# jianzhnie/RLZero

Hardware: AMD Instinct MI355X
Metric: mcts_sims_per_sec (higher is better)
Workload: dtype f32 net (hi + lo f16 operand pairs on the f16 MFMA pipe, f32 accumulation) / f64 tree

## Files before the change

include/rlzero_hip.h:

```cpp
#ifndef RLZERO_HIP_H
#define RLZERO_HIP_H

#include <stdint.h>

#ifdef __cplusplus
extern "C" {
#endif

#define RZ_ABI_VERSION 27
#define RZ_MAX_BOARD_SIZE 16
#define RZ_BOARD_WORDS 4
#define RZ_MAX_IN_FLIGHT 16

enum {
    RZ_OK = 0,
    RZ_ERR_ARG = -1,
    RZ_ERR_HIP = -2,
    RZ_ERR_OOM = -3,
    RZ_ERR_OVERFLOW = -4,
    RZ_ERR_ILLEGAL = -5,
    RZ_ERR_INTERNAL = -6
};

enum {
    RZ_GAME_GOMOKU = 0,
    RZ_GAME_CONNECT4 = 1
};

enum {
    RZ_SCORE_UCT_REF = 0,
    RZ_SCORE_PUCT = 1
};

enum { RZ_EVAL_V0 = 0, RZ_EVAL_VLIN = 1 };

enum {
    RZ_FLAG_ARENA_FULL = 1,
    RZ_FLAG_BLOCKS_FULL = 2,
    RZ_FLAG_ILLEGAL_MOVE = 4,
    RZ_FLAG_LOGTAB = 8,
    RZ_FLAG_INTERNAL = 16,
    RZ_FLAG_REUSE_DROPPED = 32
};

typedef struct rz_engine rz_engine;

typedef struct rz_config {
    int32_t abi_version;
    int32_t game_kind;
    int32_t board_size;
    int32_t n_in_row;
    int32_t n_games;
    int32_t n_playout;
    int32_t score_mode;
    int32_t add_noise;
    double c_puct;
    double pool_factor;
    int32_t device;
    int32_t noise_seed;
    int32_t board_height;
    int32_t board_width;
    int32_t sims_in_flight;
    int32_t in_flight_impl;
} rz_config;

typedef struct rz_stats {
    int32_t error_flags;
    int32_t first_bad_game;
    int64_t arena_slots;
    int64_t prior_floats;
    int64_t max_slots_used;
    int64_t max_blocks_used;
    int64_t device_bytes;
    int64_t n_select_calls;
    int64_t reuse_dropped;
} rz_stats;

int rz_abi_version(void);
const char *rz_source_hash(void);
const char *rz_last_error(void);

int rz_create(const rz_config *cfg, rz_engine **out);
int rz_destroy(rz_engine *e);
int rz_geometry(rz_engine *e, int32_t *height, int32_t *width, int32_t *n_actions);

int rz_upload_log_table(rz_engine *e, const double *h_table, int64_t count);
int rz_log_table_size(rz_engine *e, int64_t *count);

int rz_set_roots(rz_engine *e, const uint64_t *d_stones, const int32_t *d_to_move,
                 const int32_t *d_last_move, const uint8_t *d_mask, int reset_trees,
                 void *stream);
int rz_get_roots(rz_engine *e, uint64_t *d_stones, int32_t *d_to_move, int32_t *d_last_move,
                 void *stream);
int rz_set_active(rz_engine *e, const uint8_t *d_active, void *stream);
int rz_set_noise_keys(rz_engine *e, const uint64_t *d_keys, const uint8_t *d_mask, void *stream);

int rz_select_step(rz_engine *e, float *d_obs, void *stream);
int rz_set_in_flight(rz_engine *e, int32_t k_backup, int32_t k_select);

int rz_leaf_buffers(rz_engine *e, const uint64_t **d_stones, const int32_t **d_to_move, const int32_t **d_last_cell);

int rz_encode_leaf_obs(rz_engine *e, float *d_obs, void *stream);
int rz_encode_root_obs(rz_engine *e, float *d_obs, void *stream);

int rz_get_leaves(rz_engine *e, uint64_t *d_stones, int32_t *d_to_move, int32_t *d_last_move,
                  int32_t *d_terminal, void *stream);

int rz_eval_synthetic(rz_engine *e, int kind, float *d_logp, float *d_value, void *stream);

int rz_eval_rollout(rz_engine *e, uint64_t seed, uint32_t sim_index, int32_t n_limit, float *d_value,
                    void *stream);

int rz_expand_backup(rz_engine *e, const float *d_logp, const float *d_value, void *stream);
int rz_expand_backup_f64(rz_engine *e, const float *d_logp, const double *d_value, void *stream);
int rz_expand_backup_probs(rz_engine *e, const float *d_probs, const double *d_value, void *stream);

int rz_tree_step(rz_engine *e, const float *d_logp, const float *d_value, float *d_obs, void *stream);

typedef struct rz_raw_heads {
    const float *raw;
    const float *hid;
    const float *w2;
    const float *b2;
    const float *act_scale;
    const float *act_bias;
    const float *val_scale;
    const float *val_bias;
    int64_t raw_part_stride;
    int64_t hid_part_stride;
    int32_t ld;
    int32_t n_parts;
} rz_raw_heads;

int rz_expand_backup_raw(rz_engine *e, const rz_raw_heads *heads, void *stream);
int rz_tree_step_raw(rz_engine *e, const rz_raw_heads *heads, float *d_obs, void *stream);

typedef struct rz_value_head {
    const float *valfeat;
    const float *w1t;
    const float *b1;
    const float *w2;
    const float *b2;
    int32_t ld;
    int32_t groups;
} rz_value_head;
typedef struct rz_deferred_logits {
    const float *raw;
    int32_t ld;
    int32_t rows_per_slot;
} rz_deferred_logits;
int rz_deferred_reserve(rz_engine *e, int32_t slots);
int rz_trace_attach(rz_engine *e, void *d_trace);
int rz_device_view(rz_engine *e, void *out, int64_t out_bytes);
int rz_deferred_slots(rz_engine *e, const int32_t **d_slot_of_game);
int rz_expand_backup_deferred(rz_engine *e, const rz_value_head *head, void *stream);
int rz_tree_step_deferred(rz_engine *e, const rz_value_head *head, void *stream);
int rz_deferred_flush(rz_engine *e, const rz_deferred_logits *logits, int32_t n_slots, void *stream);

int rz_root_visits(rz_engine *e, int32_t *d_visits, void *stream);
int rz_root_wsum(rz_engine *e, double *d_w, void *stream);
int rz_root_priors(rz_engine *e, float *d_p, void *stream);
int rz_root_stats(rz_engine *e, int32_t *d_n, double *d_w, void *stream);
int rz_root_values(rz_engine *e, double *d_out, void *stream);

int rz_advance_roots(rz_engine *e, const int32_t *d_moves, void *stream);

int rz_step_games(rz_engine *e, const int32_t *d_moves, int32_t *d_winner, uint8_t *d_ended,
                  void *stream);

#define RZ_PLAY_RECORD_WORDS 8
enum {
    RZ_PLAY_RUNNING = 1,
    RZ_PLAY_STALLED = 2,
    RZ_PLAY_RESOLVED = 4,
    RZ_PLAY_ENDED = 8,
    RZ_PLAY_SEARCHED = 16,
    RZ_PLAY_RESIGNED = 32,
    RZ_PLAY_NO_RESIGN = 64,
    RZ_PLAY_WOULD_RESIGN = 128
};
typedef struct rz_play_config {
    uint64_t seed;
    double temperature;
    double stall_margin;
    const int64_t *d_queue_ids;
    int32_t *d_queue_ctl;
    int32_t *d_log;
    int32_t ring_steps;
    int32_t reserved;
} rz_play_config;
int rz_play_attach(rz_engine *e, const rz_play_config *cfg);
int rz_play_draw(rz_engine *e, void *stream);
int rz_play_apply(rz_engine *e, void *stream);
int rz_play_set_resign(rz_engine *e, double threshold, double disabled_frac, void *stream);
int rz_play_resolve(rz_engine *e, int32_t slot, int32_t move, void *stream);
int rz_play_stop(rz_engine *e, void *stream);
int rz_play_state(rz_engine *e, int64_t *h_game_id, int32_t *h_ply, int32_t *h_state, int64_t *h_steps);

int rz_get_stats(rz_engine *e, rz_stats *out);
int rz_clear_errors(rz_engine *e);
int rz_poll_errors(rz_engine *e, int32_t *h_flags, int32_t *h_reuse_dropped, void *stream);

int rz_copy_arena(rz_engine *e, int32_t game, int64_t max_slots, int32_t *h_n, double *h_w,
                  int32_t *h_first_child, int32_t *h_n_visited, int32_t *h_n_children,
                  int32_t *h_prior_block, float *h_root_prior, int32_t *h_top);
int rz_copy_priors(rz_engine *e, int32_t game, int64_t max_floats, float *h_priors, int32_t *h_count);

int rz_uct_scores(rz_engine *e, const double *d_w, const int32_t *d_n, const int32_t *d_np,
                  double c_puct, double *d_out, int64_t count, void *stream);

typedef struct rz_net rz_net;
enum {
    RZ_NET_DIRECT = 0,
    RZ_NET_WINOGRAD_F4 = 1,
    RZ_NET_SPLIT_F16 = 2
    ,
    RZ_NET_SPLIT_F16_TILES = 3
    ,
    RZ_NET_SPLIT_F16_FP8 = 4
};
int rz_net_range_info(rz_net *net, float *h_info8);
enum { RZ_NET_FLAG_F16_RANGE = 1 };
int rz_net_error_flags(rz_net *net, uint32_t *h_flags);
int rz_net_set_algo(rz_net *net, int32_t algo);
int rz_net_set_max_workgroups(rz_net *net, int32_t max_workgroups);
enum { RZ_NET_HEADS_AUTO = 0, RZ_NET_HEADS_F32 = 1, RZ_NET_HEADS_SPLIT_32 = 2, RZ_NET_HEADS_SPLIT_64 = 3, RZ_NET_HEADS_SPLIT_PARTS = 4,
       RZ_NET_HEADS_IN_TRUNK = 5    };
int rz_net_set_heads_algo(rz_net *net, int32_t heads_algo);
int rz_net_create(int32_t height, int32_t width, int32_t n_actions, int32_t device, rz_net **out);
int rz_net_destroy(rz_net *net);
int rz_net_load(rz_net *net, const float *const *h_params, int32_t n_params);
int rz_net_reserve(rz_net *net, int32_t max_boards);
int rz_net_trunk(rz_net *net, const float *d_obs, int32_t n_boards, float *d_feat, void *stream);
int rz_net_trunk_leaves(rz_net *net, const uint64_t *d_stones, const int32_t *d_to_move, const int32_t *d_last_cell,
                        int32_t n_boards, void *stream);
int rz_net_deferred_reserve(rz_net *net, int32_t max_boards, int32_t slots);
int rz_net_trunk_leaves_deferred(rz_net *net, const uint64_t *d_stones, const int32_t *d_to_move, const int32_t *d_last_cell,
                                 int32_t n_boards, const int32_t *d_slot_of_board, rz_value_head *out, void *stream);
int rz_net_deferred_gemm(rz_net *net, int32_t n_boards, int32_t n_slots, rz_deferred_logits *out, void *stream);
int rz_net_trace_attach(rz_net *net, void *d_trace);
int rz_net_delta_reserve(rz_net *net, int32_t n_games);
int rz_net_delta_invalidate(rz_net *net, void *stream);
int rz_net_delta_resident(rz_net *net, int32_t on);
int rz_net_delta_bases(rz_net *net, const uint64_t *d_root_stones, const int32_t *d_root_to_move, int32_t n_games, void *stream);
int rz_net_delta_leaves(rz_net *net, const uint64_t *d_stones, const int32_t *d_to_move, const int32_t *d_last_cell, int32_t n_boards,
                        const int32_t *d_slot_of_board, const uint8_t *d_active, float *d_feat32, int32_t without_base, rz_value_head *out,
                        void *stream);
int rz_net_delta_bases_engine(rz_net *net, rz_engine *engine, void *stream);
int rz_net_delta_step(rz_net *net, rz_engine *engine, rz_value_head *out, void *stream);
int rz_net_delta_trunk_engine(rz_net *net, rz_engine *engine, void *stream);
int rz_net_delta_stats(rz_net *net, uint32_t *h_out8, int32_t reset);
int rz_net_search_resident(rz_net *net, rz_engine *engine, int32_t n_sims, int32_t select_first, void *stream);
int rz_net_heads(rz_net *net, int32_t n_boards, float *d_logp, float *d_value, void *stream);
int rz_net_heads_gemm(rz_net *net, int32_t n_boards, rz_raw_heads *out, void *stream);
int rz_net_forward(rz_net *net, const float *d_obs, int32_t n_boards, float *d_logp,
                   float *d_value, void *stream);

typedef struct rz_muzero rz_muzero;
typedef struct rz_mz_config {
    int32_t abi_version;
    int32_t n_games;
    int32_t n_actions;
    int32_t n_sims;
    double discount;
    double pb_c_base;
    double pb_c_init;
    int32_t device;
    int32_t reserved;
} rz_mz_config;

int rz_mz_create(const rz_mz_config *cfg, rz_muzero **out);
int rz_mz_destroy(rz_muzero *e);
int rz_mz_upload_log_table(rz_muzero *e, const double *h_table, int64_t count);
int rz_mz_init_roots(rz_muzero *e, const float *d_probs, const double *d_noise, double noise_frac,
                     const uint8_t *d_mask, void *stream);
int rz_mz_select(rz_muzero *e, int32_t *d_parent, int32_t *d_action, int32_t *d_leaf, const uint8_t *d_mask,
                 void *stream);
int rz_mz_expand_backup(rz_muzero *e, const float *d_reward, const float *d_probs, const float *d_value,
                        const uint8_t *d_mask, void *stream);
int rz_mz_load_model(rz_muzero *e, const float *const *h_params, int32_t n_params, int32_t hidden);
int rz_mz_search(rz_muzero *e, float *d_hidden, int32_t n_sims, int32_t *d_trace_parent, int32_t *d_trace_action,
                 int32_t *d_trace_leaf, float *d_trace_reward, float *d_trace_probs, float *d_trace_value, void *stream);
int rz_mz_set_search_shape(rz_muzero *e, int32_t games_per_workgroup);
typedef struct rz_mz_cartpole_play {
    double *d_state;
    int64_t *d_steps, *d_episode, *d_episode_start;
    uint64_t env_seed, noise_seed;
    double noise_frac, dirichlet_alpha, temperature;
    double *d_ring;
    int32_t ring_steps, reserved;
    int64_t first_step;
    double *d_arena;
    int64_t arena_rows;
    int64_t *d_counters, *d_entries;
    int64_t max_entries;
} rz_mz_cartpole_play;
int rz_mz_load_representation(rz_muzero *e, const float *const *h_params, int32_t n_params, int32_t obs_dim, int32_t hidden);
int rz_mz_play_cartpole(rz_muzero *e, float *d_hidden, int32_t n_sims, int32_t n_moves, const rz_mz_cartpole_play *play, void *stream);
int rz_cartpole_step(double *d_state, int64_t *d_steps, int64_t *d_episode, const int64_t *d_actions, int32_t n_envs, uint64_t seed,
                     float *d_obs, float *d_reward, uint8_t *d_terminated, uint8_t *d_truncated, void *stream);
int rz_mz_root_children(rz_muzero *e, int32_t what, void *d_out, void *stream);
int rz_mz_root_stats(rz_muzero *e, int32_t *d_n, double *d_value_sum, double *d_vmin, double *d_vmax, void *stream);
int rz_mz_geometry(rz_muzero *e, int32_t *slots_per_game, int64_t *device_bytes);
int rz_mz_error_flags(rz_muzero *e, int32_t *flags);

#ifdef __cplusplus
}
#endif
#endif
```

profiles/microbench/delta_resident_phases.py:

```python
import ctypes, os, sys
sys.path.insert(0, os.environ.get('GRAFT_REPO_ROOT', '.'))
import rlzero_amd._hip as H
H.library_path = lambda: os.environ.get('RZ_NETPROF_LIB') or os.path.join(os.path.dirname(os.path.abspath(__file__)), 'librlzero_netprof.so')
import rlzero_amd._build as B
B.needs_build = lambda: False
import numpy as np, torch
from rlzero_amd.engine import HipNetEvaluator, MCTSEngine
from rlzero_amd.games.gomoku.policy_value_net import PolicyValueNet
lib = H.load()
NAMES = [(0, 'leaf + changed cells'), (1, 'distances, requests, ranks'), (3, 'maps, base records'), (4, 'bar'), (5, 'conv1'), (6, 'bar'), (7, 'conv2'),
         (9, 'bar + conv3 + heads'), (10, 'bar'), (11, 'features'), (12, 'bar'), (16, 'value layer'), (17, 'expand + backup'),
         (2, 'sel: root record'), (8, 'sel: root scan / answer'), (13, 'sel: level-0 cell'), (14, 'sel: deeper levels'), (15, 'sel: terminal test + leaf stores'),
         (18, 'selection (rest: hand-over)'), (19, 'wave 1: pre-scan'), (20, 'wave 1: wait behind it')]
sizes = [int(a) for a in sys.argv[1:]] or [1, 256, 512]
for games in sizes:
    torch.manual_seed(0)
    net = PolicyValueNet(15).to('cuda:0')
    ev = HipNetEvaluator(net, 15, 'cuda:0', max_boards=games)
    sims = 800
    eng = MCTSEngine(15, 5, n_games=games, n_playout=sims, device='cuda:0', add_noise=True)
    eng.reset_games()
    assert ev.resident_ok(eng) and ev.resident_delta_ok(eng)
    rng = np.random.default_rng(0)
    for ply in range(6):
        eng.sim_chunk(ev, 40)
        visits = eng.root_visits()
        moves = np.array([int(rng.choice(np.flatnonzero(v > 0))) for v in visits], dtype=np.int32)
        eng.advance(moves)
        eng.step(moves)
    a, b = torch.cuda.Event(enable_timing=True), torch.cuda.Event(enable_timing=True)
    ev.hip.delta_stats(reset=True)
    a.record(); eng.sim_chunk(ev, sims); b.record(); torch.cuda.synchronize()
    st = ev.hip.delta_stats()
    out = (ctypes.c_longlong * 24)()
    assert lib.rz_net_debug_profile(out) == 0
    us = 1e3 * a.elapsed_time(b) / sims
    total = out[23] / sims
    print('%d games, %d simulations: %.2f us per simulation of a game (events, bases included), %d cycles (%.2f GHz); %.2f conv3 / %.2f conv2 tiles, %.2f changed cells per leaf, %d leaves without a base' % (
        games, sims, us, total, total / us / 1e3, st['tiles3'] / max(1, st['delta'] + st['no_base']), st['tiles2'] / max(1, st['delta'] + st['no_base']),
        st['cells'] / max(1, st['delta'] + st['no_base']), st['no_base']))
    print('   ' + '  '.join('%s=%d' % (nm, out[k] / sims) for k, nm in NAMES) + '  prescans=%d' % st['prescans'], flush=True)
    eng.close(); ev.hip.close()
```

rlzero_amd/_hip.py:

```python
import ctypes
import os
from ctypes import (POINTER, Structure, c_char_p, c_double, c_int, c_int32, c_int64, c_uint32, c_uint64,
                    c_void_p)

ABI_VERSION = 27
BOARD_WORDS = 4
MAX_BOARD_SIZE = 16
MAX_IN_FLIGHT = 16

OK = 0
SCORE_UCT_REF, SCORE_PUCT = 0, 1
GAME_GOMOKU, GAME_CONNECT4 = 0, 1
NET_DIRECT, NET_WINOGRAD_F4, NET_SPLIT_F16, NET_SPLIT_F16_TILES, NET_SPLIT_F16_FP8 = 0, 1, 2, 3, 4
NET_FLAG_F16_RANGE = 1
NET_HEADS_AUTO, NET_HEADS_F32, NET_HEADS_SPLIT_32, NET_HEADS_SPLIT_64, NET_HEADS_SPLIT_PARTS, NET_HEADS_IN_TRUNK = 0, 1, 2, 3, 4, 5
EVAL_V0, EVAL_VLIN = 0, 1
FLAG_NAMES = {1: 'arena full', 2: 'block queue full', 4: 'illegal move', 8: 'ln table too short',
              16: 'internal'}
FLAG_REUSE_DROPPED = 32


class RzConfig(Structure):
    _fields_ = [('abi_version', c_int32), ('game_kind', c_int32), ('board_size', c_int32),
                ('n_in_row', c_int32), ('n_games', c_int32), ('n_playout', c_int32),
                ('score_mode', c_int32), ('add_noise', c_int32), ('c_puct', c_double),
                ('pool_factor', c_double), ('device', c_int32), ('noise_seed', c_int32),
                ('board_height', c_int32), ('board_width', c_int32),
                ('sims_in_flight', c_int32), ('in_flight_impl', c_int32)]


class RzStats(Structure):
    _fields_ = [('error_flags', c_int32), ('first_bad_game', c_int32), ('arena_slots', c_int64),
                ('prior_floats', c_int64), ('max_slots_used', c_int64), ('max_blocks_used', c_int64),
                ('device_bytes', c_int64), ('n_select_calls', c_int64), ('reuse_dropped', c_int64)]


class RzMzConfig(Structure):
    _fields_ = [('abi_version', c_int32), ('n_games', c_int32), ('n_actions', c_int32), ('n_sims', c_int32),
                ('discount', c_double), ('pb_c_base', c_double), ('pb_c_init', c_double),
                ('device', c_int32), ('reserved', c_int32)]


class RzMzCartPolePlay(Structure):
    _fields_ = [('d_state', c_void_p), ('d_steps', c_void_p), ('d_episode', c_void_p), ('d_episode_start', c_void_p),
                ('env_seed', c_uint64), ('noise_seed', c_uint64), ('noise_frac', c_double), ('dirichlet_alpha', c_double),
                ('temperature', c_double), ('d_ring', c_void_p), ('ring_steps', c_int32), ('reserved', c_int32),
                ('first_step', c_int64), ('d_arena', c_void_p), ('arena_rows', c_int64), ('d_counters', c_void_p),
                ('d_entries', c_void_p), ('max_entries', c_int64)]


class RzRawHeads(Structure):
    _fields_ = [('raw', c_void_p), ('hid', c_void_p), ('w2', c_void_p), ('b2', c_void_p), ('act_scale', c_void_p),
                ('act_bias', c_void_p), ('val_scale', c_void_p), ('val_bias', c_void_p), ('raw_part_stride', c_int64),
                ('hid_part_stride', c_int64), ('ld', c_int32), ('n_parts', c_int32)]


class RzValueHead(Structure):
    _fields_ = [('valfeat', c_void_p), ('w1t', c_void_p), ('b1', c_void_p), ('w2', c_void_p), ('b2', c_void_p),
                ('ld', c_int32), ('groups', c_int32)]


class RzDeferredLogits(Structure):
    _fields_ = [('raw', c_void_p), ('ld', c_int32), ('rows_per_slot', c_int32)]


class RzPlayConfig(Structure):
    _fields_ = [('seed', c_uint64), ('temperature', c_double), ('stall_margin', c_double), ('d_queue_ids', c_void_p),
                ('d_queue_ctl', c_void_p), ('d_log', c_void_p), ('ring_steps', c_int32), ('reserved', c_int32)]


PLAY_RECORD_WORDS = 8
PLAY_RUNNING, PLAY_STALLED, PLAY_RESOLVED, PLAY_ENDED, PLAY_SEARCHED = 1, 2, 4, 8, 16
PLAY_RESIGNED, PLAY_NO_RESIGN, PLAY_WOULD_RESIGN = 32, 64, 128


class HipError(RuntimeError):
    pass


P = c_void_p

_SIGNATURES = {
    'rz_abi_version': (c_int, []),
    'rz_last_error': (c_char_p, []),
    'rz_source_hash': (c_char_p, []),
    'rz_create': (c_int, [POINTER(RzConfig), POINTER(c_void_p)]),
    'rz_destroy': (c_int, [P]),
    'rz_geometry': (c_int, [P, POINTER(c_int32), POINTER(c_int32), POINTER(c_int32)]),
    'rz_upload_log_table': (c_int, [P, P, c_int64]),
    'rz_log_table_size': (c_int, [P, POINTER(c_int64)]),
    'rz_set_roots': (c_int, [P, P, P, P, P, c_int, P]),
    'rz_get_roots': (c_int, [P, P, P, P, P]),
    'rz_set_active': (c_int, [P, P, P]),
    'rz_set_noise_keys': (c_int, [P, P, P, P]),
    'rz_select_step': (c_int, [P, P, P]),
    'rz_set_in_flight': (c_int, [P, c_int32, c_int32]),
    'rz_leaf_buffers': (c_int, [P, POINTER(c_void_p), POINTER(c_void_p), POINTER(c_void_p)]),
    'rz_encode_leaf_obs': (c_int, [P, P, P]),
    'rz_encode_root_obs': (c_int, [P, P, P]),
    'rz_get_leaves': (c_int, [P, P, P, P, P, P]),
    'rz_eval_synthetic': (c_int, [P, c_int, P, P, P]),
    'rz_eval_rollout': (c_int, [P, c_uint64, c_uint32, c_int32, P, P]),
    'rz_expand_backup': (c_int, [P, P, P, P]),
    'rz_expand_backup_f64': (c_int, [P, P, P, P]),
    'rz_expand_backup_probs': (c_int, [P, P, P, P]),
    'rz_tree_step': (c_int, [P, P, P, P, P]),
    'rz_expand_backup_raw': (c_int, [P, POINTER(RzRawHeads), P]),
    'rz_tree_step_raw': (c_int, [P, POINTER(RzRawHeads), P, P]),
    'rz_trace_attach': (c_int, [P, P]),
    'rz_net_trace_attach': (c_int, [P, P]),
    'rz_device_view': (c_int, [P, P, c_int64]),
    'rz_deferred_reserve': (c_int, [P, c_int32]),
    'rz_deferred_slots': (c_int, [P, POINTER(c_void_p)]),
    'rz_expand_backup_deferred': (c_int, [P, POINTER(RzValueHead), P]),
    'rz_tree_step_deferred': (c_int, [P, POINTER(RzValueHead), P]),
    'rz_deferred_flush': (c_int, [P, POINTER(RzDeferredLogits), c_int32, P]),
    'rz_root_visits': (c_int, [P, P, P]),
    'rz_root_wsum': (c_int, [P, P, P]),
    'rz_root_priors': (c_int, [P, P, P]),
    'rz_root_stats': (c_int, [P, P, P, P]),
    'rz_root_values': (c_int, [P, P, P]),
    'rz_advance_roots': (c_int, [P, P, P]),
    'rz_step_games': (c_int, [P, P, P, P, P]),
    'rz_play_attach': (c_int, [P, POINTER(RzPlayConfig)]),
    'rz_play_draw': (c_int, [P, P]),
    'rz_play_apply': (c_int, [P, P]),
    'rz_play_set_resign': (c_int, [P, c_double, c_double, P]),
    'rz_play_resolve': (c_int, [P, c_int32, c_int32, P]),
    'rz_play_stop': (c_int, [P, P]),
    'rz_play_state': (c_int, [P, P, P, P, POINTER(c_int64)]),
    'rz_get_stats': (c_int, [P, POINTER(RzStats)]),
    'rz_clear_errors': (c_int, [P]),
    'rz_poll_errors': (c_int, [P, POINTER(c_int32), POINTER(c_int32), P]),
    'rz_copy_arena': (c_int, [P, c_int32, c_int64, P, P, P, P, P, P, P, P]),
    'rz_copy_priors': (c_int, [P, c_int32, c_int64, P, P]),
    'rz_uct_scores': (c_int, [P, P, P, P, c_double, P, c_int64, P]),
    'rz_net_create': (c_int, [c_int32, c_int32, c_int32, c_int32, POINTER(c_void_p)]),
    'rz_net_destroy': (c_int, [P]),
    'rz_net_set_algo': (c_int, [P, c_int32]),
    'rz_net_set_max_workgroups': (c_int, [P, c_int32]),
    'rz_net_set_heads_algo': (c_int, [P, c_int32]),
    'rz_net_error_flags': (c_int, [P, POINTER(ctypes.c_uint32)]),
    'rz_net_range_info': (c_int, [P, POINTER(ctypes.c_float)]),
    'rz_net_load': (c_int, [P, POINTER(c_void_p), c_int32]),
    'rz_net_reserve': (c_int, [P, c_int32]),
    'rz_net_trunk': (c_int, [P, P, c_int32, P, P]),
    'rz_net_trunk_leaves': (c_int, [P, P, P, P, c_int32, P]),
    'rz_net_deferred_reserve': (c_int, [P, c_int32, c_int32]),
    'rz_net_trunk_leaves_deferred': (c_int, [P, P, P, P, c_int32, P, POINTER(RzValueHead), P]),
    'rz_net_deferred_gemm': (c_int, [P, c_int32, c_int32, POINTER(RzDeferredLogits), P]),
    'rz_net_search_resident': (c_int, [P, P, c_int32, c_int32, P]),
    'rz_net_delta_reserve': (c_int, [P, c_int32]),
    'rz_net_delta_invalidate': (c_int, [P, P]),
    'rz_net_delta_resident': (c_int, [P, c_int32]),
    'rz_net_delta_bases': (c_int, [P, P, P, c_int32, P]),
    'rz_net_delta_leaves': (c_int, [P, P, P, P, c_int32, P, P, P, c_int32, POINTER(RzValueHead), P]),
    'rz_net_delta_stats': (c_int, [P, POINTER(ctypes.c_uint32), c_int32]),
    'rz_net_delta_bases_engine': (c_int, [P, P, P]),
    'rz_net_delta_step': (c_int, [P, P, POINTER(RzValueHead), P]),
    'rz_net_delta_trunk_engine': (c_int, [P, P, P]),
    'rz_net_heads': (c_int, [P, c_int32, P, P, P]),
    'rz_net_heads_gemm': (c_int, [P, c_int32, POINTER(RzRawHeads), P]),
    'rz_net_forward': (c_int, [P, P, c_int32, P, P, P]),
    'rz_mz_create': (c_int, [POINTER(RzMzConfig), POINTER(c_void_p)]),
    'rz_mz_destroy': (c_int, [P]),
    'rz_mz_upload_log_table': (c_int, [P, P, c_int64]),
    'rz_mz_init_roots': (c_int, [P, P, P, c_double, P, P]),
    'rz_mz_select': (c_int, [P, P, P, P, P, P]),
    'rz_mz_expand_backup': (c_int, [P, P, P, P, P, P]),
    'rz_mz_load_model': (c_int, [P, POINTER(c_void_p), c_int32, c_int32]),
    'rz_mz_search': (c_int, [P, P, c_int32, P, P, P, P, P, P, P]),
    'rz_mz_set_search_shape': (c_int, [P, c_int32]),
    'rz_mz_load_representation': (c_int, [P, POINTER(c_void_p), c_int32, c_int32, c_int32]),
    'rz_mz_play_cartpole': (c_int, [P, P, c_int32, c_int32, POINTER(RzMzCartPolePlay), P]),
    'rz_cartpole_step': (c_int, [P, P, P, P, c_int32, c_uint64, P, P, P, P, P]),
    'rz_mz_root_children': (c_int, [P, c_int32, P, P]),
    'rz_mz_root_stats': (c_int, [P, P, P, P, P, P]),
    'rz_mz_geometry': (c_int, [P, POINTER(c_int32), POINTER(c_int64)]),
    'rz_mz_error_flags': (c_int, [P, POINTER(c_int32)]),
}

_lib = None


def library_path():
    return os.environ.get('RZ_HIP_LIBRARY') or os.path.join(os.path.dirname(os.path.abspath(__file__)), 'librlzero_hip.so')


def load():
    global _lib
    if _lib is not None:
        return _lib
    path = library_path()
    if not os.path.exists(path):
        raise HipError('%s is missing: the HIP extension is required (no CPU fallback). '
                       'Build it with `python -m rlzero_amd._build`.' % path)
    lib = ctypes.CDLL(path)
    for name, (restype, argtypes) in _SIGNATURES.items():
        fn = getattr(lib, name)
        fn.restype = restype
        fn.argtypes = argtypes
    got = lib.rz_abi_version()
    if got != ABI_VERSION:
        raise HipError('librlzero_hip.so has ABI %d, binding expects %d: rebuild' % (got, ABI_VERSION))
    if not os.environ.get('RZ_HIP_LIBRARY'):
        from . import _build
        built, tree = (lib.rz_source_hash() or b'').decode(), _build.source_hash()
        if built != tree:
            raise HipError('librlzero_hip.so was built from other sources (hash %s, this tree %s): python -m rlzero_amd._build' % (built, tree))
    _lib = lib
    return lib


def exported_symbols():
    return sorted(_SIGNATURES)


def check(rc, what=''):
    if rc != OK:
        msg = load().rz_last_error()
        raise HipError('%s failed (%d): %s' % (what or 'rz call', rc, (msg or b'').decode()))
```

rlzero_amd/csrc/rz_delta.h:

```cpp
#ifndef RZ_DELTA_TREE_PRIO
#define RZ_DELTA_TREE_PRIO 1
#endif
#ifndef RZ_DELTA_PRO_PRIO
#define RZ_DELTA_PRO_PRIO 0
#endif
#ifndef RZ_DELTA_PRESCAN
#define RZ_DELTA_PRESCAN 1
#endif

namespace dl {

using sp::f16x4;
using sp::f16x8;
typedef const __attribute__((address_space(3))) f16x8 *lds_frag;
typedef const __attribute__((address_space(3))) uint32_t *lds_u32;
typedef __attribute__((address_space(3))) f16x4 *lds_h4;
typedef __attribute__((address_space(3))) f32x4 *lds_v4;

constexpr int kC1Slots = 128, kC2Slots = 164;
constexpr int kT1 = 4, kT2 = 8, kT3 = 8;
constexpr int kMaxD = 4;
constexpr int P1 = rt::Geo<32>::pos_bytes, P2 = rt::Geo<64>::pos_bytes;
constexpr int kGrid = kRowW * kRowW;
constexpr int kShareFloats = kT3 * 4 * 96;
constexpr int kHeadW = 128 * 6 * 4 + 128 * 4 + 32;
constexpr int kOffC1 = sp::kInPieceBytes, kOffC2 = kOffC1 + kC1Slots * P1, kOffZero = kOffC2 + kC2Slots * P2, kOffHead = kOffZero + P2,
              kOffMap1 = kOffHead + kHeadW, kOffMap2 = kOffMap1 + kGrid * 4, kOffList = kOffMap2 + kGrid * 4,
              kLdsBytes = kOffList + 3 * 128 * 2;
static_assert(kShareFloats * 4 <= kC1Slots * P1, "the shares lie inside conv1's records (dead behind conv2)");
constexpr int kWinSets = rzw::kRadii * rzw::kWords, kWinLds = kWinSets * 8 + kWinSets * 4 + 16;
static_assert(2 * (kLdsBytes + 512 * 4 + 4 * 64 * 4 + 80 + kWinLds + (int)sizeof(rzt::RootPre) + 512) <= 160 * 1024,
              "two workgroups per CU, also of the resident search (value row, K-quarter sums, leaf, window sets, root pre-scan)");
static_assert(kOffC1 % 16 == 0 && kOffZero % 16 == 0 && kOffHead % 16 == 0 && kOffMap1 % 16 == 0, "alignment");

constexpr int kCells = RZ_MAX_BOARD_SIZE * RZ_MAX_BOARD_SIZE;
struct BaseHdr {
    uint64_t stones[2 * RZ_BOARD_WORDS];
    int32_t to_move, valid, pad[2];
};
constexpr size_t kBaseC2 = (size_t)kCells * 128, kBaseV = kBaseC2 + (size_t)kCells * 256, kBaseBytes = kBaseV + (size_t)6 * kCells * 4;

struct DeltaArgs {
    BaseHdr *hdr;
    char *recs;
    const uint8_t *active;
    float *feat32;
    unsigned *stats;
    int mode;
    int bw_rcp;
    const uint64_t *win;
};

__device__ __forceinline__ uint32_t lds_addr(const void *p) {
    return (uint32_t)(uintptr_t)((const __attribute__((address_space(3))) char *)p);
}

constexpr int unit_tiles(int nt) { return nt <= 3 ? nt : (nt + 1) / 2; }
constexpr int units_of(int nt) { return (nt + unit_tiles(nt) - 1) / unit_tiles(nt); }

template <int CIN, int NT, int UT>
__device__ __forceinline__ void read_unit(f16x8 (&b)[UT][2], const uint32_t (&rec)[NT][3], int h, int dy, int c) {
#pragma unroll
    for (int i = 0; i < UT; ++i) {
        const int t = h * UT + i;
        if (t < NT) {
            const uint32_t r = rec[t][dy] + (uint32_t)(c * 64);
            b[i][0] = *(lds_frag)(uintptr_t)r;
            b[i][1] = *(lds_frag)(uintptr_t)(r + CIN * 2);
        }
    }
}
template <int TM, int NT, int UT>
__device__ __forceinline__ void mfma_unit(f32x4 (&acc)[TM][NT], const f16x8 (&a)[TM][2], const f16x8 (&b)[UT][2], int h) {
#pragma unroll
    for (int combo = 0; combo < 3; ++combo)
#pragma unroll
        for (int i = 0; i < UT; ++i) {
            const int t = h * UT + i;
            if (t < NT) {
#pragma unroll
                for (int m = 0; m < TM; ++m)
                    acc[m][t] = __builtin_amdgcn_mfma_f32_16x16x32_f16(a[m][combo == 2], b[i][combo == 1], acc[m][t], 0, 0, 0);
            }
        }
}
template <int NT>
__device__ __forceinline__ void lookup(uint32_t (&rec)[NT][3], lds_u32 map, const int (&pos19)[NT], int dx, int g) {
#pragma unroll
    for (int t = 0; t < NT; ++t)
#pragma unroll
        for (int dy = 0; dy < 3; ++dy) rec[t][dy] = map[pos19[t] + dx + dy * kRowW] + (uint32_t)(g * 16);
}

template <int NT>
__device__ __forceinline__ void conv2_g(lds_u32 map, const int (&pos19)[NT], int lane, const f16x8 (&a2)[9][1][2], f32x4 (&acc)[1][NT]) {
    static_assert(NT <= 4, "one unit per step");
    const int g = lane >> 4;
#pragma unroll
    for (int t = 0; t < NT; ++t) acc[0][t] = f32x4{0.f, 0.f, 0.f, 0.f};
    constexpr int AHEAD = NT <= 2 ? 2 : 1;
    uint32_t rec[3][NT][3];
    f16x8 b[AHEAD + 1][NT][2];
#pragma unroll
    for (int dx = 0; dx < 3; ++dx) lookup<NT>(rec[dx], map, pos19, dx, g);
#pragma unroll
    for (int u = 0; u < AHEAD; ++u) read_unit<32, NT, NT>(b[u], rec[u / 3], 0, u % 3, 0);
#pragma unroll
    for (int u = 0; u < 9; ++u) {
        const int dx = u / 3, dy = u % 3;
        if (u + AHEAD < 9) read_unit<32, NT, NT>(b[(u + AHEAD) % (AHEAD + 1)], rec[(u + AHEAD) / 3], 0, (u + AHEAD) % 3, 0);
        mfma_unit<1, NT, NT>(acc, a2[dy * 3 + dx], b[u % (AHEAD + 1)], 0);
        __builtin_amdgcn_sched_barrier(0);
    }
}

#ifndef RZ_DELTA_RING6_UPTO
#define RZ_DELTA_RING6_UPTO 2
#endif
constexpr int ring3(int nt) { return nt <= RZ_DELTA_RING6_UPTO ? 6 : 3; }
__device__ __forceinline__ void load_a3(f16x8 (&a)[2][2], __amdgpu_buffer_rsrc_t w_rsrc, int lane, int dx, int j) {
    using G = rt::Geo<64>;
    const int c = j / 3, dy = j % 3;
#pragma unroll
    for (int m = 0; m < 2; ++m)
#pragma unroll
        for (int p = 0; p < 2; ++p)
            a[m][p] = sp::load_w(w_rsrc, lane * 16, dx * (G::chunks * 2048) + ((m * G::steps + dy * 3 * G::chunks + c) * 2 + p) * 1024);
}
template <int NT>
__device__ __forceinline__ void conv3_g(lds_u32 map, const uint16_t *list3, const void *wts, int lane, bool sync, f32x4 (&acc)[2][NT]) {
    static_assert(NT <= 6, "two units per step");
    constexpr int R = ring3(NT), H = units_of(NT);
    const int n = lane & 15, g = lane >> 4;
    const __amdgpu_buffer_rsrc_t w_rsrc = __builtin_amdgcn_make_buffer_rsrc(const_cast<void *>(wts), 0, 0x7fffffff, 0x00020000);
    f16x8 a3[R][2][2];
#pragma unroll
    for (int j = 0; j < R - 1; ++j) load_a3(a3[j], w_rsrc, lane, 0, j);
    if (sync) __syncthreads();
    int pos19[NT];
#pragma unroll
    for (int t = 0; t < NT; ++t) pos19[t] = (int)list3[16 * t + n] - 19;
#pragma unroll
    for (int m = 0; m < 2; ++m)
#pragma unroll
        for (int t = 0; t < NT; ++t) acc[m][t] = f32x4{0.f, 0.f, 0.f, 0.f};
    uint32_t rec[NT][3], recn[NT][3];
#ifndef RZ_DELTA_AHEAD3_SMALL
#define RZ_DELTA_AHEAD3_SMALL 1
#endif
    constexpr int UT = unit_tiles(NT), AH = UT <= 2 ? RZ_DELTA_AHEAD3_SMALL : 1, NB = AH + 1;
    static_assert((6 * H) % NB == 0 && AH <= H * 6, "a unit's registers are a constant of the unrolled body");
    f16x8 b[NB][UT][2];
    lookup<NT>(rec, map, pos19, 0, g);
#pragma unroll
    for (int u = 0; u < AH; ++u) read_unit<64, NT, UT>(b[u], rec, u % H, (u / H) % 3, u / H / 3);
#pragma unroll 1
    for (int dx = 0; dx < 3; ++dx) {
        lookup<NT>(recn, map, pos19, dx < 2 ? dx + 1 : 2, g);
#pragma unroll
        for (int u = 0; u < 6 * H; ++u) {
            const int j = u / H, h = u % H;
            if (h == 0) {
                const int jj = j + R - 1, dx2 = jj < 6 ? dx : (dx < 2 ? dx + 1 : 2);
                load_a3(a3[jj % R], w_rsrc, lane, dx2, jj % 6);
            }
            {
                const int v = u + AH;
                if (v < 6 * H) read_unit<64, NT, UT>(b[v % NB], rec, v % H, (v / H) % 3, v / H / 3);
                else read_unit<64, NT, UT>(b[v % NB], recn, (v - 6 * H) % H, ((v - 6 * H) / H) % 3, (v - 6 * H) / H / 3);
            }
            mfma_unit<2, NT, UT>(acc, a3[j % R], b[u % NB], h);
            __builtin_amdgcn_sched_barrier(0);
        }
#pragma unroll
        for (int t = 0; t < NT; ++t)
#pragma unroll
            for (int dy = 0; dy < 3; ++dy) rec[t][dy] = recn[t][dy];
    }
}

template <int T>
__device__ __forceinline__ void reduce_scatter(const float (&vals)[6 * T], float (&out)[6 * T / 4]) {
    float r1[3 * T];
#pragma unroll
    for (int i = 0; i < 3 * T; ++i) {
        const auto sw = __builtin_amdgcn_permlane16_swap(__float_as_uint(vals[i]), __float_as_uint(vals[3 * T + i]), false, false);
        r1[i] = __uint_as_float(sw[0]) + __uint_as_float(sw[1]);
    }
#pragma unroll
    for (int i = 0; i < 3 * T / 2; ++i) {
        const auto sw = __builtin_amdgcn_permlane32_swap(__float_as_uint(r1[i]), __float_as_uint(r1[3 * T / 2 + i]), false, false);
        out[i] = __uint_as_float(sw[0]) + __uint_as_float(sw[1]);
    }
}

template <int NT>
__device__ __forceinline__ void conv2_tiles(lds_u32 map1, lds_u32 map2, const uint16_t *list2, int n2, int lane, int wave, const f16x8 (&a2)[9][1][2],
                                            f32x4 bias2, float k2) {
    const int n = lane & 15, g = lane >> 4;
    int pos19[NT];
#pragma unroll
    for (int t = 0; t < NT; ++t) pos19[t] = (int)list2[16 * t + n] - 19;
    f32x4 acc[1][NT];
    conv2_g<NT>(map1, pos19, lane, a2, acc);
#pragma unroll
    for (int t = 0; t < NT; ++t) {
        if (16 * t + n < n2) {
            const uint32_t rec = map2[pos19[t] + kRowW + 1] + (uint32_t)((16 * wave + 4 * g) * 2);
            float z[4];
#pragma unroll
            for (int j = 0; j < 4; ++j) z[j] = fmaxf(fmaf(acc[0][t][j], k2, bias2[j]), 0.0f);
            f16x4 hi, lo;
            sp::split4(z, hi, lo);
            *(lds_h4)(uintptr_t)rec = hi;
            *(lds_h4)(uintptr_t)(rec + 128) = lo;
        }
    }
}

template <int NT>
__device__ __forceinline__ void conv3_tiles(lds_u32 map2, const uint16_t *list3, const void *wts, int lane, int wave, bool sync,
                                            const char *headw, float k3, float *shares) {
    constexpr int T = NT <= 4 ? 4 : 8;
    const int n = lane & 15, g = lane >> 4;
    float vals[6 * T];
    {
        f32x4 acc[2][NT];
        conv3_g<NT>(map2, list3, wts, lane, sync, acc);
        f32x4 hwr[2][6], b3r[2];
#pragma unroll
        for (int m = 0; m < 2; ++m) {
            const int c0 = 32 * wave + 16 * m + 4 * g;
#pragma unroll
            for (int i = 0; i < 6; ++i) hwr[m][i] = *reinterpret_cast<const f32x4 *>(headw + (c0 * 6 + 4 * i) * 4);
            b3r[m] = *reinterpret_cast<const f32x4 *>(headw + 128 * 6 * 4 + c0 * 4);
        }
#pragma unroll
        for (int t = 0; t < T; ++t) {
            f32x2 v2[3] = {f32x2{0.0f, 0.0f}, f32x2{0.0f, 0.0f}, f32x2{0.0f, 0.0f}};
            if (t < NT) {
#pragma unroll
                for (int m = 0; m < 2; ++m)
#pragma unroll
                    for (int j = 0; j < 4; ++j) {
                        const float hv = fmaxf(fmaf(acc[m][t < NT ? t : 0][j], k3, b3r[m][j]), 0.0f);
#pragma unroll
                        for (int o2 = 0; o2 < 3; ++o2) {
                            const int e = 6 * j + 2 * o2;
                            v2[o2] = __builtin_elementwise_fma(f32x2{hwr[m][e >> 2][e & 3], hwr[m][e >> 2][(e & 3) + 1]}, f32x2{hv, hv}, v2[o2]);
                        }
                    }
            }
#pragma unroll
            for (int o = 0; o < 6; ++o) vals[t * 6 + o] = v2[o >> 1][o & 1];
        }
    }
    float mine[6 * T / 4];
    reduce_scatter<T>(vals, mine);
    const int t0 = (T / 2) * (g & 1) + (T / 4) * (g >> 1);
#pragma unroll
    for (int i = 0; i < 6 * T / 4; ++i)
        if (t0 + i / 6 < NT) shares[((t0 + i / 6) * 4 + wave) * 96 + (i % 6) * 16 + n] = mine[i];
}

struct Leaf {
    f16x4 cell_planes;
    const char *base;
    int dys[kMaxD], dxs[kMaxD];
    _Float16 *dst16;
    float *vdst;
    float *dst32;
    const uint64_t *sets;
    bool deferred, store_head;
};
struct Layers {
    float k1, k2, k3, act1, act2, act3;
    const char *t2p, *t3p;
};
#ifdef RZ_NET_PROFILE
struct Prof { long long acc[24], t; };
#else
struct Prof {};
#endif

__device__ __forceinline__ void init_maps(char *lds, int tid) {
    uint32_t *map1 = reinterpret_cast<uint32_t *>(lds + kOffMap1);
    const uint32_t zaddr = lds_addr(lds + kOffZero);
    for (int i = tid; i < 2 * kGrid; i += 256) map1[i] = zaddr;
    if (tid < 3 * 128 / 2) reinterpret_cast<uint32_t *>(lds + kOffList)[tid] = 19u | (19u << 16);
}

__device__ __forceinline__ int cell_dist(int cy, int cx, int pass, const int (&dys)[kMaxD], const int (&dxs)[kMaxD], int BH, int BW) {
    int dist = 1000;
    if (pass < 0) {
#pragma unroll
        for (int i = 0; i < kMaxD; ++i) {
            const int ady = cy > dys[i] ? cy - dys[i] : dys[i] - cy, adx = cx > dxs[i] ? cx - dxs[i] : dxs[i] - cx;
            const int d = ady > adx ? ady : adx;
            dist = d < dist ? d : dist;
        }
    } else {
        const int y0 = 8 * (pass >> 1), x0 = 8 * (pass & 1);
        const int y1 = (y0 + 8 < BH ? y0 + 8 : BH) - 1, x1 = (x0 + 8 < BW ? x0 + 8 : BW) - 1;
        const int ddy = cy < y0 ? y0 - cy : (cy > y1 ? cy - y1 : 0), ddx = cx < x0 ? x0 - cx : (cx > x1 ? cx - x1 : 0);
        dist = ddy > ddx ? ddy : ddx;
    }
    return dist;
}

constexpr int kOutside = 1 << 30;
__device__ __forceinline__ f32x4 load_rec(__amdgpu_buffer_rsrc_t rsrc, int off) {
    return __builtin_bit_cast(f32x4, __builtin_amdgcn_raw_buffer_load_b128(rsrc, off, 0, 0));
}

__device__ __forceinline__ uint64_t uni64(uint64_t v) {
    return ((uint64_t)(unsigned)__builtin_amdgcn_readfirstlane((int)(v >> 32)) << 32) | (unsigned)__builtin_amdgcn_readfirstlane((int)v);
}

template <bool SETS>
__device__ __forceinline__ int delta_passes(const NetDev &nd, const DeltaArgs &da, char *lds, int tid0, int wave, const Leaf &leaf, const Layers &ly,
                                            f32x4 headv, bool &use_delta, Prof &prof) {
    char *in0 = lds, *c1 = lds + kOffC1, *c2 = lds + kOffC2, *zrec = lds + kOffZero, *headw = lds + kOffHead;
    uint32_t *map1 = reinterpret_cast<uint32_t *>(lds + kOffMap1), *map2 = reinterpret_cast<uint32_t *>(lds + kOffMap2);
    uint16_t *list1 = reinterpret_cast<uint16_t *>(lds + kOffList), *list2 = list1 + 128, *list3 = list2 + 128;
    float *shares = reinterpret_cast<float *>(c1);
    const int mode = da.mode, BH = nd.BH, BW = nd.BW, S = nd.S;
    const float k1 = ly.k1, k2 = ly.k2, k3 = ly.k3, act1 = ly.act1, act2 = ly.act2, act3 = ly.act3;
    const char *t2p = ly.t2p, *t3p = ly.t3p;
    const char *base = leaf.base;
    const f16x4 cell_planes = leaf.cell_planes;
    const int (&dys)[kMaxD] = leaf.dys, (&dxs)[kMaxD] = leaf.dxs;
    _Float16 *dst16 = leaf.dst16;
    float *vdst = leaf.vdst, *dst32 = leaf.dst32;
    const bool deferred = leaf.deferred, store_head = leaf.store_head;
    const uint32_t zaddr = lds_addr(zrec);
    int n_conv3_tiles = 0, n_conv2_tiles = 0;
#ifdef RZ_NET_PROFILE
    long long (&prof_acc)[24] = prof.acc, &prof_t = prof.t;
#endif
    for (int pass = use_delta ? -1 : 0; pass < 4; ++pass) {
        int tid = tid0;
        asm volatile("" : "+v"(tid));
        const int lane = tid & 63, g = lane >> 4;
        const int cy = (tid * da.bw_rcp) >> 16, cx = tid - cy * BW;
        const bool is_cell = tid < S;
        const int mypos = is_cell ? (cy + 1) * kRowW + cx + 1 : 0;
        if (RZ_DELTA_PRO_PRIO) __builtin_amdgcn_s_setprio(RZ_DELTA_PRO_PRIO);
        const int th[5] = {pass < 0 ? 1 : 2, pass < 0 ? 2 : 1, pass < 0 ? 3 : 0, pass < 0 ? 3 : 2, pass < 0 ? 4 : 1};
        bool f[5];
        uint64_t own[5];
        const bool handed = SETS && pass < 0;
        if (handed) {
#pragma unroll
            for (int k = 0; k < 5; ++k) {
                own[k] = uni64(leaf.sets[4 * (th[k] - 1) + wave]);
                f[k] = (own[k] >> lane) & 1ull;
            }
        } else {
            const int dist = cell_dist(cy, cx, pass, dys, dxs, BH, BW);
#pragma unroll
            for (int k = 0; k < 5; ++k) f[k] = is_cell && dist <= th[k];
        }
        const bool g1 = pass < 0 && f[3] && !f[0], g2 = pass < 0 && f[4] && !f[1];
        const __amdgpu_buffer_rsrc_t b_rsrc = __builtin_amdgcn_make_buffer_rsrc(const_cast<char *>(base), 0, kBaseBytes, 0x00020000);
        f32x4 r1[8], r2[16];
        {
            const int o1 = g1 ? tid * 128 : kOutside, o2 = g2 ? (int)kBaseC2 + tid * 256 : kOutside;
#pragma unroll
            for (int i = 0; i < 8; ++i) r1[i] = load_rec(b_rsrc, o1 + 16 * i);
#pragma unroll
            for (int i = 0; i < 16; ++i) r2[i] = load_rec(b_rsrc, o2 + 16 * i);
        }
        float bv[6];
        {
            const int ov = pass < 0 && is_cell && !f[2] ? (int)kBaseV + tid * 4 : kOutside;
#pragma unroll
            for (int o = 0; o < 6; ++o) bv[o] = __builtin_bit_cast(float, __builtin_amdgcn_raw_buffer_load_b32(b_rsrc, ov + o * kCells * 4, 0, 0));
        }
        sp::f16x8 a1[3][2];
        f32x4 bias1[4];
        if (32 * wave < 32 * kT1) {
#pragma unroll
            for (int ky = 0; ky < 3; ++ky)
#pragma unroll
                for (int p_ = 0; p_ < 2; ++p_) a1[ky][p_] = __builtin_bit_cast(sp::f16x8, nd.s1[(ky * 2 + p_) * 64 + lane]);
#pragma unroll
            for (int gg = 0; gg < 4; ++gg) bias1[gg] = *reinterpret_cast<const f32x4 *>(nd.b1 + 8 * gg + 4 * (lane >> 5));
        }
        f32x4 bias2 = *reinterpret_cast<const f32x4 *>(nd.b2 + 16 * wave + 4 * g);
        int rank[5], tot[5];
        if (handed) {
            const int *cnt = reinterpret_cast<const int *>(leaf.sets + kWinSets);
#pragma unroll
            for (int k = 0; k < 5; ++k) {
                int before = 0, all = 0;
#pragma unroll
                for (int w = 0; w < 4; ++w) {
                    const int c = __builtin_amdgcn_readfirstlane(cnt[4 * (th[k] - 1) + w]);
                    all += c;
                    before += w < wave ? c : 0;
                }
                rank[k] = before + (int)__builtin_amdgcn_mbcnt_hi((unsigned)(own[k] >> 32), __builtin_amdgcn_mbcnt_lo((unsigned)own[k], 0u));
                tot[k] = all;
            }
        } else {
            int before[5] = {0, 0, 0, 0, 0}, all[5] = {0, 0, 0, 0, 0};
            unsigned long long own[5] = {0ull, 0ull, 0ull, 0ull, 0ull};
#pragma unroll
            for (int b = 0; b < 4; ++b) {
                const int cell = 64 * b + lane, by = (cell * da.bw_rcp) >> 16, bx = cell - by * BW;
                const int d = cell_dist(by, bx, pass, dys, dxs, BH, BW);
#pragma unroll
                for (int k = 0; k < 5; ++k) {
                    const unsigned long long m = __ballot(cell < S && d <= th[k]);
                    const int c = __popcll(m);
                    all[k] += c;
                    before[k] += b < wave ? c : 0;
                    own[k] = b == wave ? m : own[k];
                }
            }
#pragma unroll
            for (int k = 0; k < 5; ++k) {
                rank[k] = before[k] + (int)__builtin_amdgcn_mbcnt_hi((unsigned)(own[k] >> 32), __builtin_amdgcn_mbcnt_lo((unsigned)own[k], 0u));
                tot[k] = all[k];
            }
        }
        NET_TICK(1);
        if (pass < 0 && (tot[0] > 32 * kT1 || tot[1] > 16 * kT2 || tot[2] > 16 * kT3 || tot[3] > kC1Slots || tot[4] > kC2Slots)) {
            use_delta = false;
            continue;
        }
        uint32_t rec1 = 0, rec2 = 0;
        if (f[3]) {
            rec1 = lds_addr(c1 + rank[3] * P1);
            map1[mypos] = rec1;
        }
        if (f[4]) {
            rec2 = lds_addr(c2 + rank[4] * P2);
            map2[mypos] = rec2;
        }
        if (f[0]) list1[rank[0]] = (uint16_t)mypos;
        if (f[1]) list2[rank[1]] = (uint16_t)mypos;
        if (f[2]) list3[rank[2]] = (uint16_t)mypos;
        if (pass <= 0 && is_cell) *reinterpret_cast<f16x4 *>(in0 + ((cy + 1) * sp::kInCols + (cx + 1)) * 8) = cell_planes;
        if (pass <= 0 && store_head && tid < 226) reinterpret_cast<f32x4 *>(headw)[tid] = headv;
        if (g1) {
#pragma unroll
            for (int i = 0; i < 8; ++i) *(lds_v4)(uintptr_t)(rec1 + 16 * i) = r1[i];
        }
        if (g2) {
#pragma unroll
            for (int i = 0; i < 16; ++i) *(lds_v4)(uintptr_t)(rec2 + 16 * i) = r2[i];
        }
        __builtin_amdgcn_sched_barrier(0);
        f16x8 a2[9][1][2];
        {
            const __amdgpu_buffer_rsrc_t w_rsrc = __builtin_amdgcn_make_buffer_rsrc(const_cast<char *>(t2p), 0, 0x7fffffff, 0x00020000);
#pragma unroll
            for (int tap = 0; tap < 9; ++tap)
#pragma unroll
                for (int p = 0; p < 2; ++p) a2[tap][0][p] = sp::load_w(w_rsrc, lane * 16, (tap * 2 + p) * 1024);
        }
        NET_TICK(3);
        __syncthreads();
        NET_TICK(4);

        if (32 * wave < tot[0]) {
            const int n32 = lane & 31, h = lane >> 5, idx = 32 * wave + n32;
            const int pos = list1[idx];
            const int py = (pos * 3641) >> 16, px = pos - py * kRowW;
            typedef const __attribute__((address_space(3))) f16x4 *lds_half;
            const lds_half q = (lds_half)(in0 + ((py - 1) * sp::kInCols + (px - 1) + 2 * h) * 8);
            sp::f16x8 b1[3];
#pragma unroll
            for (int ky = 0; ky < 3; ++ky) {
                const int o = ky * sp::kInCols;
                const f16x4 lo4 = q[o], hi4 = q[o + 1];
                b1[ky] = __builtin_shufflevector(lo4, hi4, 0, 1, 2, 3, 4, 5, 6, 7);
            }
            sp::f32x16 acc1;
#pragma unroll
            for (int r = 0; r < 16; ++r) acc1[r] = 0.0f;
#pragma unroll
            for (int ky = 0; ky < 3; ++ky)
#pragma unroll
                for (int combo = 0; combo < 3; combo += 2)
                    acc1 = __builtin_amdgcn_mfma_f32_32x32x16_f16(a1[ky][combo == 2], b1[ky], acc1, 0, 0, 0);
            if (idx < tot[0]) {
                const uint32_t rec = map1[pos] + (uint32_t)(4 * h * 2);
#pragma unroll
                for (int gg = 0; gg < 4; ++gg) {
// ... 18 lines not shown

        if (RZ_DELTA_PRO_PRIO) __builtin_amdgcn_s_setprio(0);
        const int nt3 = (tot[2] + 15) >> 4;
        {
            const lds_u32 m1 = (lds_u32)map1, m2 = (lds_u32)map2;
            const int nt2 = (tot[1] + 15) >> 4;
            n_conv2_tiles += nt2;
            for (int t0 = 0; t0 < nt2; t0 += 4) {
                const uint16_t *l2 = list2 + 16 * t0;
                const int left = tot[1] - 16 * t0;
                switch (nt2 - t0) {
                    case 1: conv2_tiles<1>(m1, m2, l2, left, lane, wave, a2, bias2 * act2, k2); break;
                    case 2: conv2_tiles<2>(m1, m2, l2, left, lane, wave, a2, bias2 * act2, k2); break;
                    case 3: conv2_tiles<3>(m1, m2, l2, left, lane, wave, a2, bias2 * act2, k2); break;
                    default: conv2_tiles<4>(m1, m2, l2, left, lane, wave, a2, bias2 * act2, k2); break;
                }
            }
        }
        NET_TICK(7);

        {
            const lds_u32 m2 = (lds_u32)map2;
            n_conv3_tiles += nt3;
            const int first = nt3 <= 6 ? nt3 : 4;
            switch (first) {
                case 0: __syncthreads(); break;
                case 1: conv3_tiles<1>(m2, list3, t3p, lane, wave, true, headw, k3, shares); break;
                case 2: conv3_tiles<2>(m2, list3, t3p, lane, wave, true, headw, k3, shares); break;
                case 3: conv3_tiles<3>(m2, list3, t3p, lane, wave, true, headw, k3, shares); break;
                case 4: conv3_tiles<4>(m2, list3, t3p, lane, wave, true, headw, k3, shares); break;
                case 5: conv3_tiles<5>(m2, list3, t3p, lane, wave, true, headw, k3, shares); break;
                default: conv3_tiles<6>(m2, list3, t3p, lane, wave, true, headw, k3, shares); break;
            }
            if (nt3 == 7) conv3_tiles<3>(m2, list3 + 64, t3p, lane, wave, false, headw, k3, shares + 4 * 4 * 96);
            else if (nt3 >= 8) conv3_tiles<4>(m2, list3 + 64, t3p, lane, wave, false, headw, k3, shares + 4 * 4 * 96);
        }
        NET_TICK(9);
        __syncthreads();
        NET_TICK(10);
        if (mode == 1 && f[1]) {
            f32x4 *dstp = reinterpret_cast<f32x4 *>(const_cast<char *>(base) + kBaseC2 + (size_t)tid * 256);
#pragma unroll
            for (int i = 0; i < 16; ++i) dstp[i] = *(lds_v4)(uintptr_t)(rec2 + 16 * i);
        }

        if (is_cell && (pass < 0 || f[2])) {
            const float *share = shares + (rank[2] >> 4) * 4 * 96 + (rank[2] & 15);
            float *basev = mode == 1 ? reinterpret_cast<float *>(const_cast<char *>(base) + kBaseV) : nullptr;
#pragma unroll
            for (int o = 0; o < 6; ++o) {
                float v;
                if (f[2]) {
                    float s = share[o * 16];
#pragma unroll
                    for (int w = 1; w < 4; ++w) s += share[w * 96 + o * 16];
                    v = fmaxf(s + reinterpret_cast<const float *>(headw + 128 * 7 * 4)[o], 0.0f);
                } else {
                    v = bv[o];
                }
                if (mode == 1) {
                    basev[o * kCells + tid] = v;
                    continue;
                }
                if (dst32) dst32[o * S + tid] = v;
                if (deferred && o >= 4) {
                    vdst[(o - 4) * S + tid] = v;
                } else if (dst16) {
                    const int k = (o < 4 ? o : o - 4) * S + tid;
                    const int step = (o < 4 ? 0 : nd.groups_act) + (k >> 4);
                    const float z = v * act3;
                    const _Float16 zh = (_Float16)z;
                    _Float16 *q = dst16 + (size_t)step * 1024 + (k & 15);
                    q[0] = zh;
                    q[512] = (_Float16)(z - (float)zh);
                }
            }
        }
        if (f[3]) map1[mypos] = zaddr;
        if (f[4]) map2[mypos] = zaddr;
        NET_TICK(11);
        if (pass < 0) break;
        __syncthreads();
    }
    return n_conv3_tiles | (n_conv2_tiles << 16);
}

__device__ __forceinline__ f16x4 planes_of(const uint64_t (&ls)[8], int tid, int tm_eff, bool has_last, int lc, int par_count) {
    f16x4 cell_planes;
    const int word = (tid >> 6) & 3, bit = tid & 63;
    uint64_t w0 = 0ull, w1 = 0ull;
#pragma unroll
    for (int w = 0; w < 4; ++w) {
        const uint64_t mk = word == w ? ~0ull : 0ull;
        w0 |= ls[w] & mk;
        w1 |= ls[4 + w] & mk;
    }
    const bool s0 = (w0 >> bit) & 1ull, s1 = (w1 >> bit) & 1ull;
    const bool mine = tm_eff == 0 ? s0 : s1, theirs = tm_eff == 0 ? s1 : s0;
    const _Float16 one = (_Float16)sp::kObsScale, zero = (_Float16)0.0f;
    cell_planes[0] = mine ? one : zero;
    cell_planes[1] = theirs ? one : zero;
    cell_planes[2] = (has_last && tid == lc) ? one : zero;
    cell_planes[3] = (par_count & 1) ? zero : one;
    return cell_planes;
}

__device__ __forceinline__ bool changed_cells(const uint64_t (&ls)[8], const uint64_t (&rs)[8], int nst, int tm, int lc, bool has_last, bool base_ok, int h_tm,
                                              int bw_rcp, int BW, int (&dys)[kMaxD], int (&dxs)[kMaxD], int &parity, int &nD) {
    bool use_delta = false;
    {
        bool sup = true;
        int nroot = 0;
        uint64_t D[4] = {0ull, 0ull, 0ull, 0ull};
#pragma unroll
        for (int q = 0; q < 8; ++q) {
            sup = sup && (rs[q] & ~ls[q]) == 0ull;
            nroot += __popcll(rs[q]);
            D[q & 3] |= rs[q] ^ ls[q];
        }
#pragma unroll
        for (int w = 0; w < 4; ++w) D[w] |= (has_last && lc >= 0 && (lc >> 6) == w) ? 1ull << (lc & 63) : 0ull;
        parity = (nst - nroot) & 1;
        nD = __popcll(D[0]) + __popcll(D[1]) + __popcll(D[2]) + __popcll(D[3]);
        use_delta = base_ok && sup && tm == (h_tm ^ parity) && nD <= kMaxD;
#pragma unroll
        for (int i = 0; i < kMaxD; ++i) {
            const bool z0 = D[0] == 0ull, z1 = D[1] == 0ull, z2 = D[2] == 0ull;
            const int w = !z0 ? 0 : !z1 ? 1 : !z2 ? 2 : 3;
            const uint64_t word = !z0 ? D[0] : !z1 ? D[1] : !z2 ? D[2] : D[3];
            const bool any = word != 0ull;
            const int cell = 64 * w + __builtin_ctzll(word | (1ull << 63));
            const uint64_t rest = word & (word - 1ull);
#pragma unroll
            for (int k = 0; k < 4; ++k) D[k] = k == w ? rest : D[k];
            const int y = (cell * bw_rcp) >> 16;
            dys[i] = any ? y : -100;
            dxs[i] = any ? cell - y * BW : -100;
        }
    }
    return use_delta;
}

template <bool TRACE>
__global__ __launch_bounds__(256, 2) void k_trunk_delta(NetDev nd, LeafBits leaves, _Float16 *__restrict__ feat16, int n_boards,
                                                        DeferredOut later, DeltaArgs da) {
    __shared__ __attribute__((aligned(16))) char lds[kLdsBytes];
    const int board = blockIdx.x;
    const int mode = da.mode;
    const int game = mode == 1 ? board >> 1 : board, par_b = mode == 1 ? board & 1 : 0;
    unsigned long long trace_t0 = 0;
    if (TRACE) trace_t0 = rz_trace_now();
    Prof prof;
#ifdef RZ_NET_PROFILE
    for (int i = 0; i < 24; ++i) prof.acc[i] = 0;
    prof.t = __builtin_readcyclecounter();
    const long long prof_k0 = prof.t;
    long long (&prof_acc)[24] = prof.acc, &prof_t = prof.t;
#endif
    const int tid0 = threadIdx.x, wave = __builtin_amdgcn_readfirstlane(tid0 >> 6);
    const int BW = nd.BW, S = nd.S;
    Layers ly;
    ly.t2p = reinterpret_cast<const char *>(nd.t2) + (size_t)wave * rt::Geo<32>::steps * 2 * 1024;
    ly.t3p = reinterpret_cast<const char *>(nd.t3) + (size_t)(2 * wave) * rt::Geo<64>::steps * 2 * 1024;
    f32x4 headv = tid0 < 192 ? reinterpret_cast<const f32x4 *>(nd.whp)[tid0] : reinterpret_cast<const f32x4 *>(nd.b3)[(tid0 - 192) & 31];
    {
        const float *bh = nd.bh + (tid0 == 225 ? 4 : 0);
        const f32x4 hbv = {bh[0], bh[1], tid0 == 225 ? 0.0f : bh[2], tid0 == 225 ? 0.0f : bh[3]};
        headv = (tid0 == 224 || tid0 == 225) ? hbv : headv;
    }
    ly.k1 = nd.s_inv[2], ly.k2 = nd.s_inv[0], ly.k3 = nd.s_inv[1];
    ly.act1 = nd.s_inv[5], ly.act2 = nd.s_inv[6], ly.act3 = nd.s_inv[7];

    const uint64_t *sb = leaves.stones + (size_t)game * 8;
    const BaseHdr *hd = da.hdr + game;
    uint64_t ls[8], rs[8];
    int nst = 0;
#pragma unroll
    for (int q = 0; q < 8; ++q) {
        ls[q] = sb[q];
        rs[q] = hd->stones[q];
        nst += __popcll(ls[q]);
    }
    const int tm = leaves.to_move[game];
    const int lc_raw = (mode == 1 ? leaves.to_move : leaves.last)[game];
    const int lc = mode == 1 ? -1 : lc_raw;
    const int h_tm = hd->to_move, h_valid = hd->valid;
    const int is_active = da.active[game];
    const bool deferred = later.slot_of != nullptr;
    const int slot_ = (deferred ? later.slot_of : leaves.to_move)[deferred ? board : game];
    const int tm_eff = tm ^ par_b;
    const int par_count = nst + par_b;
    const bool has_last = mode != 1 && nst > 0;

    Leaf leaf;
    int parity = 0, nD = 0;
    bool use_delta = changed_cells(ls, rs, nst, tm, lc, has_last, mode == 0 && h_valid != 0, h_tm, da.bw_rcp, BW, leaf.dys, leaf.dxs, parity, nD);
    leaf.base = da.recs + ((size_t)game * 2 + (mode == 1 ? par_b : parity)) * kBaseBytes;
    leaf.cell_planes = planes_of(ls, tid0, tm_eff, has_last, lc, par_count);

    leaf.dst16 = nullptr;
    leaf.vdst = nullptr;
    if (mode != 1 && deferred) {
        leaf.dst16 = (feat16 != nullptr && slot_ < later.n_slots) ? feat16 + (size_t)slot_ * later.slot_halfs + (size_t)(board >> 5) * nd.groups_act * 1024 + (board & 31) * 16 : nullptr;
        leaf.vdst = later.valfeat + (size_t)board * later.vf_ld;
    }
    if (mode != 1 && !deferred && feat16 != nullptr)
        leaf.dst16 = feat16 + ((size_t)(board >> 5) * (nd.groups_act + nd.groups_val) * 1024 + (board & 31) * 16);
    leaf.dst32 = (mode != 1 && da.feat32 != nullptr) ? da.feat32 + (size_t)board * 6 * S : nullptr;
    leaf.sets = nullptr;
    leaf.deferred = deferred;
    leaf.store_head = true;

    {
        const f32x4 zero = {0.f, 0.f, 0.f, 0.f};
        f32x4 *z = reinterpret_cast<f32x4 *>(lds);
        for (int i = tid0; i < sp::kInPieceBytes / 16; i += 256) z[i] = zero;
        if (tid0 < P2 / 16) reinterpret_cast<f32x4 *>(lds + kOffZero)[tid0] = zero;
        init_maps(lds, tid0);
    }
    if (mode == 0 && is_active == 0) return;
    __syncthreads();
    NET_TICK(0);
    const int n_tiles = delta_passes<false>(nd, da, lds, tid0, wave, leaf, ly, headv, use_delta, prof);
    const int n_conv3_tiles = n_tiles & 0xffff;

    if (mode == 1 && par_b == 0 && tid0 == 0) {
        BaseHdr *h = da.hdr + game;
#pragma unroll
        for (int q = 0; q < 8; ++q) h->stones[q] = sb[q];
        h->to_move = tm;
        h->valid = 1;
    }
    if (da.stats != nullptr && tid0 == 0 && mode != 1) {
        atomicAdd(da.stats + (use_delta ? 0 : 1), 1u);
        atomicAdd(da.stats + 2, (unsigned)n_conv3_tiles);
        atomicAdd(da.stats + 3, (unsigned)nD);
        atomicAdd(da.stats + 4, (unsigned)(n_tiles >> 16));
    }
#ifdef RZ_NET_PROFILE
    if (blockIdx.x == 0 && tid0 == 0) {
        for (int i = 0; i < 24; ++i) net_prof[i] = prof_acc[i];
        net_prof[23] = __builtin_readcyclecounter() - prof_k0;
        net_prof[22] = n_conv3_tiles;
    }
#endif
    if (TRACE && tid0 == 0) rz_trace_write(later.trace, RZ_TRACE_TRUNK, deferred ? slot_ : 0, board, trace_t0);
}

__device__ __forceinline__ void windows_store(uint64_t row, bool use_delta, int parity, int nD, int lane, uint64_t *ws) {
    unsigned lo = (unsigned)row, hi = (unsigned)(row >> 32);
    {
        const auto a = __builtin_amdgcn_permlane16_swap(lo, lo, false, false), b = __builtin_amdgcn_permlane16_swap(hi, hi, false, false);
        lo = a[0] | a[1];
        hi = b[0] | b[1];
    }
    {
        const auto a = __builtin_amdgcn_permlane32_swap(lo, lo, false, false), b = __builtin_amdgcn_permlane32_swap(hi, hi, false, false);
        lo = a[0] | a[1];
        hi = b[0] | b[1];
    }
    const uint64_t v = ((uint64_t)hi << 32) | lo;
    int *cnt = reinterpret_cast<int *>(ws + kWinSets);
    if (lane < kWinSets) {
        ws[lane] = v;
        cnt[lane] = __popcll(v);
    }
    if (lane == 0) cnt[kWinSets] = (use_delta ? 1 : 0) | (parity << 1) | (nD << 8);
}
__device__ __forceinline__ void leaf_windows(const uint64_t *leaf_lds, const uint64_t (&rs)[8], bool base_ok, int h_tm, const DeltaArgs &da, int BW,
                                             int lane, uint64_t *ws) {
    uint64_t ls[8];
    int nst = 0;
#pragma unroll
    for (int q = 0; q < 8; ++q) {
        ls[q] = uni64(leaf_lds[q]);
        nst += __popcll(ls[q]);
    }
    const int tm = __builtin_amdgcn_readfirstlane(reinterpret_cast<const int *>(leaf_lds + 2 * RZ_BOARD_WORDS)[0]);
    const int lc = __builtin_amdgcn_readfirstlane(reinterpret_cast<const int *>(leaf_lds + 2 * RZ_BOARD_WORDS)[1]);
    int dys[kMaxD], dxs[kMaxD], parity = 0, nD = 0;
    const bool use_delta = changed_cells(ls, rs, nst, tm, lc, nst > 0, base_ok, h_tm, da.bw_rcp, BW, dys, dxs, parity, nD);
    const int i = lane >> 4;
    int dy = dys[0], dx = dxs[0];
#pragma unroll
    for (int j = 1; j < kMaxD; ++j) {
        dy = i == j ? dys[j] : dy;
        dx = i == j ? dxs[j] : dx;
    }
    const bool any = dy >= 0;
    const uint64_t row = da.win[(any ? dy * BW + dx : 0) * kWinSets + (lane & (kWinSets - 1))];
    windows_store(any ? row : 0ull, use_delta, parity, nD, lane, ws);
}

#if defined(RZ_NET_PROFILE) && !defined(RZ_SEL_TICKS)
#define RZ_SEL_TICKS 0
#endif
struct ResHook {
    static constexpr bool kOn = true;
    rzt::RootPre *pre;
    const uint64_t *win;
    int depth;
    bool any0;
    uint64_t row;
    __device__ __forceinline__ void root_cell(int last, int stones, int lane) {
        any0 = stones > 0 && last >= 0 && last < kCells;
        row = win[(any0 ? last : 0) * kWinSets + (lane & (kWinSets - 1))];
    }
    __device__ __forceinline__ void cell(int level, int c, int lane) {
        const uint64_t v = win[c * kWinSets + (lane & (kWinSets - 1))];
        row = (lane >> 4) == level ? v : row;
    }
#ifdef RZ_NET_PROFILE
    Prof *prof;
    __device__ __forceinline__ void tick(int i, int arrived) {
        if ((RZ_SEL_TICKS >> i) & 1) {
            asm volatile("" ::"v"(arrived));
            const int slot = i == 0 ? 2 : i == 1 ? 8 : 12 + i;
            __builtin_amdgcn_sched_barrier(0);
            const long long now = __builtin_readcyclecounter();
            prof->acc[slot] += now - prof->t;
            prof->t = now;
            __builtin_amdgcn_sched_barrier(0);
        }
    }
#else
    __device__ __forceinline__ void tick(int, int) {}
#endif
};

__device__ __forceinline__ void path_windows(const ResHook &hook, bool base_ok, int lane, uint64_t *ws) {
    const int depth = hook.depth;
    const bool mine = depth == 0 ? (lane < 16 && hook.any0) : (lane >> 4) < depth;
    const int nD = depth == 0 ? (hook.any0 ? 1 : 0) : depth;
    windows_store(mine ? hook.row : 0ull, base_ok && nD <= kMaxD, depth & 1, nD, lane, ws);
}

constexpr int kResVrow = 512;
__global__ __launch_bounds__(256, 2) void k_delta_res(NetDev nd, _Float16 *__restrict__ store16, DeferredOut later, DeltaArgs da, ResArgs<true> res) {
    __shared__ __attribute__((aligned(16))) char lds[kLdsBytes];
    __shared__ float res_vrow[kResVrow];
    __shared__ float res_part[rzt::kDefWaves][rzt::kWave];
    __shared__ __attribute__((aligned(16))) uint64_t res_leaf[2 * RZ_BOARD_WORDS + 2];
    __shared__ __attribute__((aligned(16))) uint64_t res_win[kWinLds / 8];
    __shared__ __attribute__((aligned(16))) rzt::RootPre res_pre;
    const int game = blockIdx.x;
    if (game >= res.E.n_games || res.E.active[game] == 0) return;
    const unsigned long long clk0 = __builtin_readcyclecounter(), rt0 = __builtin_amdgcn_s_memrealtime();
    const int tid0 = threadIdx.x, wave = __builtin_amdgcn_readfirstlane(tid0 >> 6);
    const int BW = nd.BW;
    Prof prof;
#ifdef RZ_NET_PROFILE
    for (int i = 0; i < 24; ++i) prof.acc[i] = 0;
    prof.t = __builtin_readcyclecounter();
    const long long prof_k0 = prof.t;
    long long (&prof_acc)[24] = prof.acc, &prof_t = prof.t;
#endif
    Layers ly;
    ly.t2p = reinterpret_cast<const char *>(nd.t2) + (size_t)wave * rt::Geo<32>::steps * 2 * 1024;
    ly.t3p = reinterpret_cast<const char *>(nd.t3) + (size_t)(2 * wave) * rt::Geo<64>::steps * 2 * 1024;
    f32x4 headv = tid0 < 192 ? reinterpret_cast<const f32x4 *>(nd.whp)[tid0] : reinterpret_cast<const f32x4 *>(nd.b3)[(tid0 - 192) & 31];
    {
        const float *bh = nd.bh + (tid0 == 225 ? 4 : 0);
        const f32x4 hbv = {bh[0], bh[1], tid0 == 225 ? 0.0f : bh[2], tid0 == 225 ? 0.0f : bh[3]};
        headv = (tid0 == 224 || tid0 == 225) ? hbv : headv;
    }
    ly.k1 = nd.s_inv[2], ly.k2 = nd.s_inv[0], ly.k3 = nd.s_inv[1];
    ly.act1 = nd.s_inv[5], ly.act2 = nd.s_inv[6], ly.act3 = nd.s_inv[7];
    const int slot0 = res.E.pend[game];
    uint64_t rs[8];
    bool base_ok = da.hdr[game].valid != 0;
#pragma unroll
    for (int q = 0; q < 8; ++q) {
        rs[q] = res.E.root_stones[(size_t)game * 8 + q];
        base_ok = base_ok && da.hdr[game].stones[q] == rs[q];
    }
    const int h_tm = res.E.root_to_move[game];
    base_ok = base_ok && da.hdr[game].to_move == h_tm;
    {
        const f32x4 zero = {0.f, 0.f, 0.f, 0.f};
        f32x4 *z = reinterpret_cast<f32x4 *>(lds);
        for (int i = tid0; i < sp::kInPieceBytes / 16; i += 256) z[i] = zero;
        if (tid0 < P2 / 16) reinterpret_cast<f32x4 *>(lds + kOffZero)[tid0] = zero;
        init_maps(lds, tid0);
        for (int i = tid0; i < kResVrow; i += 256) res_vrow[i] = 0.0f;
    }
    if (tid0 == 0) res_pre.scan = res_pre.valid = res_pre.answered = 0;
    ResHook hook;
    hook.pre = &res_pre;
    hook.win = da.win;
    hook.depth = 0;
    hook.any0 = false;
    hook.row = 0ull;
#ifdef RZ_NET_PROFILE
    hook.prof = &prof;
    long long pre_cycles = 0, pre_wait = 0;
#endif
    if (res.select_first == 0 && tid0 == 0) {
#pragma unroll
        for (int q = 0; q < 8; ++q) res_leaf[q] = res.E.leaf_stones[(size_t)game * 8 + q];
        reinterpret_cast<int *>(res_leaf + 2 * RZ_BOARD_WORDS)[0] = res.E.leaf_to_move[game];
        reinterpret_cast<int *>(res_leaf + 2 * RZ_BOARD_WORDS)[1] = res.E.leaf_last[game];
    }
    __syncthreads();
    if (wave == 0) {
        const int lane0 = tid0 & 63;
        if (res.select_first != 0) {
            rzt::select_body<false, rzt::kWords, ResHook>(res.E, nullptr, game, lane0, 0, res_leaf, &hook);
            path_windows(hook, base_ok, lane0, res_win);
        } else {
            leaf_windows(res_leaf, rs, base_ok, h_tm, da, BW, lane0, res_win);
        }
    }
    __syncthreads();
    int tiles_total = 0, tiles2_total = 0, deltas = 0, cells_total = 0;
    for (int sim = 0; sim < res.n_sims; ++sim) {
        int tid_s = tid0;
        asm volatile("" : "+v"(tid_s));
        uint64_t ls[8];
        int nst = 0;
#pragma unroll
        for (int q = 0; q < 8; ++q) {
            const uint64_t v = res_leaf[q];
            ls[q] = ((uint64_t)(unsigned)__builtin_amdgcn_readfirstlane((int)(v >> 32)) << 32) | (unsigned)__builtin_amdgcn_readfirstlane((int)v);
            nst += __popcll(ls[q]);
        }
        const int tm = __builtin_amdgcn_readfirstlane(reinterpret_cast<const int *>(res_leaf + 2 * RZ_BOARD_WORDS)[0]);
        const int lc = __builtin_amdgcn_readfirstlane(reinterpret_cast<const int *>(res_leaf + 2 * RZ_BOARD_WORDS)[1]);
        const bool has_last = nst > 0;
        const int verdict = __builtin_amdgcn_readfirstlane(reinterpret_cast<const int *>(res_win + kWinSets)[kWinSets]);
        bool use_delta = (verdict & 1) != 0;
        const int parity = (verdict >> 1) & 1, nD = verdict >> 8;
        Leaf leaf;
        leaf.sets = res_win;
#pragma unroll
        for (int i = 0; i < kMaxD; ++i) leaf.dys[i] = leaf.dxs[i] = -100;
        leaf.base = da.recs + ((size_t)game * 2 + parity) * kBaseBytes;
        leaf.cell_planes = planes_of(ls, tid_s, tm, has_last, lc, nst);
        leaf.dst16 = slot0 + sim < later.n_slots ? store16 + (size_t)(slot0 + sim) * later.slot_halfs + (size_t)(game >> 5) * nd.groups_act * 1024 + (game & 31) * 16 : nullptr;
        leaf.vdst = res_vrow;
        leaf.dst32 = nullptr;
        leaf.deferred = true;
        leaf.store_head = sim == 0;
        NET_TICK(0);
        const int n_tiles = delta_passes<true>(nd, da, lds, tid_s, wave, leaf, ly, headv, use_delta, prof);
        tiles_total += n_tiles & 0xffff;
        tiles2_total += n_tiles >> 16;
        deltas += use_delta ? 1 : 0;
        cells_total += nD;
        __syncthreads();
        NET_TICK(12);
        const int lane = tid_s & 63;
        if (RZ_DELTA_TREE_PRIO) __builtin_amdgcn_s_setprio(RZ_DELTA_TREE_PRIO);
        if (res.vh.groups == 128) rzt::value_quarter_lds<16>(res.vh, res_vrow, lane, wave, res_part);
        else rzt::value_quarter_lds<8>(res.vh, res_vrow, lane, wave, res_part);
        NET_TICK(16);
        const bool more = sim + 1 < res.n_sims;
        if (wave == 0) {
            rzt::expand_backup_body<float, false, false, false, true>(res.E, nullptr, nullptr, game, lane, rz_raw_heads(), 0, res.vh, res_part);
        } else {
            __syncthreads();
            if (RZ_DELTA_PRESCAN && wave == 1 && more) {
#ifdef RZ_NET_PROFILE
                const long long t0 = __builtin_readcyclecounter();
#endif
                rzt::root_prescan<rzt::kWords>(res.E, game, lane, &res_pre);
#ifdef RZ_NET_PROFILE
                __builtin_amdgcn_s_waitcnt(0);
                const long long t1 = __builtin_readcyclecounter();
                pre_cycles += t1 - t0;
                pre_wait -= t1;
#endif
            }
        }
        __syncthreads();
#ifdef RZ_NET_PROFILE
        if (RZ_DELTA_PRESCAN && wave == 1 && more) pre_wait += __builtin_readcyclecounter();
#endif
        NET_TICK(17);
        if (wave == 0 && more) {
            hook.depth = 0, hook.any0 = false, hook.row = 0ull;
            int lane_t = lane;
            asm volatile("" : "+v"(lane_t));
            rzt::select_body<false, rzt::kWords, ResHook>(res.E, nullptr, game, lane_t, 0, res_leaf, &hook);
            path_windows(hook, base_ok, lane_t, res_win);
        }
        if (RZ_DELTA_TREE_PRIO) __builtin_amdgcn_s_setprio(0);
        __syncthreads();
        NET_TICK(18);
    }
    if (da.stats != nullptr && tid0 == 0) {
        atomicAdd(da.stats + 0, (unsigned)deltas);
        atomicAdd(da.stats + 1, (unsigned)(res.n_sims - deltas));
        atomicAdd(da.stats + 2, (unsigned)tiles_total);
        atomicAdd(da.stats + 3, (unsigned)cells_total);
        atomicAdd(da.stats + 4, (unsigned)tiles2_total);
        atomicAdd(da.stats + 5, (unsigned)res_pre.answered);
        if (game == 0) {
            da.stats[6] = (unsigned)((__builtin_readcyclecounter() - clk0) >> 8);
            da.stats[7] = (unsigned)(__builtin_amdgcn_s_memrealtime() - rt0);
        }
    }
#ifdef RZ_NET_PROFILE
    if (blockIdx.x == 0 && tid0 == 0) {
        for (int i = 0; i < 24; ++i)
            if (i != 19 && i != 20) net_prof[i] = prof_acc[i];
        net_prof[23] = __builtin_readcyclecounter() - prof_k0;
        net_prof[22] = tiles_total;
    }
    if (blockIdx.x == 0 && tid0 == 64) {
        net_prof[19] = pre_cycles;
        net_prof[20] = pre_wait;
    }
#endif
}

}
```

rlzero_amd/csrc/rz_net.hip:

```cpp

#include <hip/hip_runtime.h>

#include <cmath>
#include <cstdio>
#include <cstring>
#include <new>
#include <type_traits>
#include <utility>
#include <vector>

#include "rlzero_hip.h"
#include "rz_trace.h"
#include "rz_tree.h"
#include "rz_window.h"

void rz_set_error(const char *msg);

namespace {

typedef float f32x4 __attribute__((ext_vector_type(4)));
typedef float f32x2 __attribute__((ext_vector_type(2)));

constexpr int kRowW = 18;
constexpr int kPlaneDirect = 336, kPlaneWino = 337;
// ... 511 lines not shown
    __syncthreads();
    {
        float *dst = feat + (size_t)board * nd.feat_ld;
#pragma unroll
        for (int k = 0; k < kFeatPer; ++k) {
            if (feat_dst[k] < 0) continue;
            float v = feat_bias[k];
#pragma unroll
            for (int g = 0; g < 4; ++g) v += partial[g * 6 * 256 + feat_src[k]];
            dst[feat_dst[k]] = fmaxf(v, 0.0f);
        }
    }
    }
}

namespace sp {

typedef _Float16 f16x8 __attribute__((ext_vector_type(8)));
typedef _Float16 f16x4 __attribute__((ext_vector_type(4)));
typedef float f32x16 __attribute__((ext_vector_type(16)));
typedef const __attribute__((address_space(3))) f16x8 *lds_frag;

constexpr float kObsScale = 16.0f;
constexpr float kMaxActScale = 16.0f, kF16Room = 60000.0f;
constexpr int kGridPos = 18 * 18;
template <int CIN, int POS = kGridPos> struct Geo {
    static constexpr int pos_bytes = (CIN + 8) * 2;
    static constexpr int piece_bytes = POS * pos_bytes;
    static constexpr int chunks = CIN / 16, steps = 9 * chunks;
};
constexpr int kC1Bytes = 2 * Geo<32>::piece_bytes, kC2Bytes = 2 * Geo<64>::piece_bytes;
constexpr int kInCols = 20, kInPieceBytes = 18 * kInCols * 8, kInBytes = 2 * kInPieceBytes;
constexpr int kHeadFloats = 128 * 7 + 8;
constexpr int kLdsBytes = kInBytes + kC1Bytes + kC2Bytes + kHeadFloats * 4;
static_assert(kLdsBytes <= 160 * 1024, "LDS budget");
static_assert(kInBytes % 16 == 0, "piece alignment");

__device__ __forceinline__ f16x8 load_w(__amdgpu_buffer_rsrc_t rsrc, int lane_off, int uniform_off) {
    return __builtin_bit_cast(f16x8, __builtin_amdgcn_raw_buffer_load_b128(rsrc, lane_off, uniform_off, 0));
}

__device__ __forceinline__ float resid_lo(float z, unsigned pair) {
    float r;
    asm("v_fma_mix_f32 %0, %1, -1.0, %2 op_sel_hi:[1,0,0]" : "=v"(r) : "v"(pair), "v"(z));
    return r;
}
__device__ __forceinline__ float resid_hi(float z, unsigned pair) {
    float r;
    asm("v_fma_mix_f32 %0, %1, -1.0, %2 op_sel:[1,0,0] op_sel_hi:[1,0,0]" : "=v"(r) : "v"(pair), "v"(z));
    return r;
}
__device__ __forceinline__ void split4(const float (&z)[4], f16x4 &hi, f16x4 &lo) {
    typedef float f32x4v __attribute__((ext_vector_type(4)));
    typedef unsigned u32x2 __attribute__((ext_vector_type(2)));
    const f32x4v zv = {z[0], z[1], z[2], z[3]};
    hi = __builtin_convertvector(zv, f16x4);
    const u32x2 pairs = __builtin_bit_cast(u32x2, hi);
    const f32x4v r = {resid_lo(z[0], pairs[0]), resid_hi(z[1], pairs[0]), resid_lo(z[2], pairs[1]), resid_hi(z[3], pairs[1])};
    lo = __builtin_convertvector(r, f16x4);
}

constexpr int ring_depth(int tm, int tn) { return tm * tn >= 3 ? 3 : 5; }
constexpr int act_depth(int, int) { return 2; }
template <int CIN, int TM, int TN, int RPT, int RW, int S, int I>
__device__ __forceinline__ void slot(f32x16 (&acc)[TM][TN], f16x8 (&a)[ring_depth(TM, TN)][TM][2], f16x8 (&b)[act_depth(TM, TN)][TN][2], lds_frag q0,
                                     lds_frag q1, __amdgpu_buffer_rsrc_t w_rsrc, int w_base, int w_lane) {
    using G = Geo<CIN>;
    constexpr int D = ring_depth(TM, TN);
    constexpr int combo = I / (TM * TN), m = (I / TN) % TM, n = I % TN;
    constexpr int pa = combo == 2 ? 1 : 0, pb = combo == 1 ? 1 : 0;
    constexpr int DB = act_depth(TM, TN);
    if constexpr (S == 0 && combo == 0) {
        const f32x16 zero = {0.f, 0.f, 0.f, 0.f, 0.f, 0.f, 0.f, 0.f, 0.f, 0.f, 0.f, 0.f, 0.f, 0.f, 0.f, 0.f};
        acc[m][n] = __builtin_amdgcn_mfma_f32_32x32x16_f16(a[S % D][m][pa], b[S % DB][n][pb], zero, 0, 0, 0);
    } else {
        acc[m][n] = __builtin_amdgcn_mfma_f32_32x32x16_f16(a[S % D][m][pa], b[S % DB][n][pb], acc[m][n], 0, 0, 0);
    }
    if constexpr (I < 2 * TN) {
        if constexpr (S + DB - 1 < G::steps) {
            constexpr int s1 = S + DB - 1, tap = s1 / G::chunks, c = s1 % G::chunks, nn = I / 2, piece = I % 2;
            constexpr int off = ((RPT * nn + tap / 3) * RW + tap % 3) * G::pos_bytes + c * 32;
            static_assert(off % 16 == 0 && off < 65536, "ds_read_b128 immediate");
            b[s1 % DB][nn][piece] = (piece ? q1 : q0)[off / 16];
        }
    } else if constexpr (I < 2 * TN + 2 * TM) {
        if constexpr (S + D - 1 < G::steps) {
            constexpr int s2 = S + D - 1, j = I - 2 * TN, mm = j / 2, piece = j % 2;
            a[s2 % D][mm][piece] = load_w(w_rsrc, w_lane, w_base + ((mm * G::steps + s2) * 2 + piece) * 1024);
            if constexpr (TM == 1 && TN == 1 && I == 2)
                a[s2 % D][0][1] = load_w(w_rsrc, w_lane, w_base + (s2 * 2 + 1) * 1024);
        }
    }
    __builtin_amdgcn_sched_barrier(0);
}

template <int CIN, int TM, int TN, int RPT, int RW, int S, int... Is>
__device__ __forceinline__ void step(std::integer_sequence<int, Is...>, f32x16 (&acc)[TM][TN], f16x8 (&a)[ring_depth(TM, TN)][TM][2],
                                     f16x8 (&b)[act_depth(TM, TN)][TN][2], lds_frag q0, lds_frag q1, __amdgpu_buffer_rsrc_t w_rsrc,
                                     int w_base, int w_lane) {
    (slot<CIN, TM, TN, RPT, RW, S, Is>(acc, a, b, q0, q1, w_rsrc, w_base, w_lane), ...);
}

template <int CIN, int TM, int TN, int RPT, int RW, int... Ss>
__device__ __forceinline__ void steps(std::integer_sequence<int, Ss...>, f32x16 (&acc)[TM][TN], f16x8 (&a)[ring_depth(TM, TN)][TM][2],
                                      f16x8 (&b)[act_depth(TM, TN)][TN][2], lds_frag q0, lds_frag q1, __amdgpu_buffer_rsrc_t w_rsrc,
                                      int w_base, int w_lane) {
    (step<CIN, TM, TN, RPT, RW, Ss>(std::make_integer_sequence<int, 3 * TM * TN>{}, acc, a, b, q0, q1, w_rsrc, w_base, w_lane), ...);
}

template <int CIN, int TM, int TN>
__device__ __forceinline__ void preload_w(f16x8 (&a)[ring_depth(TM, TN)][TM][2], const void *wts, int lane) {
    using G = Geo<CIN>;
    const __amdgpu_buffer_rsrc_t w_rsrc = __builtin_amdgcn_make_buffer_rsrc(const_cast<void *>(wts), 0, 0x7fffffff, 0x00020000);
#pragma unroll
    for (int s = 0; s < ring_depth(TM, TN) - 1; ++s)
#pragma unroll
        for (int m = 0; m < TM; ++m)
#pragma unroll
            for (int p = 0; p < 2; ++p) a[s][m][p] = load_w(w_rsrc, lane * 16, ((m * G::steps + s) * 2 + p) * 1024);
}

template <int CIN, int TM, int TN, int RPT = 2, int RW = kRowW, int POS = kGridPos>
__device__ __forceinline__ void conv(const char *in, const void *wts, int row0, int ry, int x, int lane,
                                     f16x8 (&a)[ring_depth(TM, TN)][TM][2], f32x16 (&acc)[TM][TN]) {
    using G = Geo<CIN, POS>;
    const int h = lane >> 5;
    const int lane_byte = ((row0 + ry) * RW + x) * G::pos_bytes + h * 16;
    const lds_frag q0 = (lds_frag)(in + lane_byte), q1 = (lds_frag)(in + lane_byte + G::piece_bytes);
    const __amdgpu_buffer_rsrc_t w_rsrc = __builtin_amdgcn_make_buffer_rsrc(const_cast<void *>(wts), 0, 0x7fffffff, 0x00020000);
    f16x8 b[act_depth(TM, TN)][TN][2];
#pragma unroll
    for (int s0 = 0; s0 < act_depth(TM, TN) - 1; ++s0) {
        const int tap = s0 / G::chunks, c = s0 % G::chunks;
#pragma unroll
        for (int nn = 0; nn < TN; ++nn) {
            const int off = ((RPT * nn + tap / 3) * RW + tap % 3) * G::pos_bytes + c * 32;
            b[s0][nn][0] = q0[off / 16];
            b[s0][nn][1] = q1[off / 16];
        }
    }
    __builtin_amdgcn_sched_barrier(0);
    steps<CIN, TM, TN, RPT, RW>(std::make_integer_sequence<int, G::steps>{}, acc, a, b, q0, q1, w_rsrc, 0, lane * 16);
}

}

struct LeafBits {
    const uint64_t *stones;
    const int32_t *to_move;
    const int32_t *last;
};

#ifdef RZ_NET_PROFILE
__device__ long long net_prof[24];
#define NET_TICK(i) do { __builtin_amdgcn_sched_barrier(0); const long long now_ = __builtin_readcyclecounter(); prof_acc[i] += now_ - prof_t; prof_t = now_; __builtin_amdgcn_sched_barrier(0); } while (0)
#else
#define NET_TICK(i)
#endif

__device__ __forceinline__ float other_half(float x, int h) {
    const auto r = __builtin_amdgcn_permlane32_swap(__float_as_uint(x), __float_as_uint(x), false, false);
    return __uint_as_float(h ? r[0] : r[1]);
}

#ifndef RZ_SPLIT_TREE_PRIO
#define RZ_SPLIT_TREE_PRIO 1
#endif
template <bool RES> struct ResArgs {};
template <> struct ResArgs<true> {
    rzt::Dev E;
    rz_value_head vh;
    int n_sims;
    int select_first;
};
__device__ __forceinline__ int res_sims(const ResArgs<false> &) { return 0; }
__device__ __forceinline__ int res_sims(const ResArgs<true> &r) { return r.n_sims; }

struct DeferredOut {
    const int32_t *slot_of;
    long long slot_halfs;
    float *valfeat;
    int vf_ld;
    unsigned long long *trace;
    int n_slots;
};

template <int TN, int MS = 1, bool RES = false, int RW = kRowW, int RH = 18>
__global__ __launch_bounds__(256, (RW == kRowW ? 1 : 2)) void k_trunk_split(NetDev nd, const float *__restrict__ obs, LeafBits leaves,
                                                     float *__restrict__ feat, _Float16 *__restrict__ feat16,
                                                     int n_boards, unsigned *__restrict__ flags,
                                                     float *__restrict__ raw = nullptr, float *__restrict__ hid = nullptr,
                                                     DeferredOut later = DeferredOut{nullptr, 0, nullptr, 0, nullptr},
                                                     ResArgs<RES> res = ResArgs<RES>{}) {
#ifdef RZ_NET_PROFILE
    const long long prof_k0 = __builtin_readcyclecounter();
    long long prof_acc[24] = {0, 0, 0, 0, 0, 0, 0, 0, 0, 0, 0, 0, 0, 0, 0, 0, 0, 0, 0, 0, 0, 0, 0, 0}, prof_t = prof_k0;
#endif
    constexpr int kThreads = 256;
    constexpr int kResWords = (MS == 4 || MS == 2) ? 1 : 2;
    __shared__ float res_vrow[RES ? 256 : 1];
    __shared__ float res_part[RES ? rzt::kDefWaves : 1][RES ? rzt::kWave : 1];
    __shared__ __attribute__((aligned(16))) uint64_t res_leaf[RES ? 2 * RZ_BOARD_WORDS + 1 : 1];
    int res_slot0 = 0;
    if constexpr (RES) {
        if ((int)blockIdx.x >= n_boards || res.E.active[blockIdx.x] == 0) return;
        res_slot0 = res.E.pend[blockIdx.x];
        res_vrow[threadIdx.x] = 0.0f;
    }
    constexpr int POS = RW * RH, IC = RW + 2;
    constexpr int kInPiece = RH * IC * 8, kInB = 2 * kInPiece, kC1B = 2 * sp::Geo<32, POS>::piece_bytes, kC2B = 2 * sp::Geo<64, POS>::piece_bytes;
    static_assert(kInB % 16 == 0 && POS >= 128, "the grid: 16-byte pieces, 128 positions for the channel-split variants' partial sums");
    __shared__ __attribute__((aligned(16))) char lds_raw[kInB + kC1B + kC2B + sp::kHeadFloats * 4];
    char *in0 = lds_raw;
    char *c1 = lds_raw + kInB;
    char *c2 = c1 + kC1B;
    float *hw = reinterpret_cast<float *>(c2 + kC2B);
    const int tid0 = threadIdx.x;
    const int BH = nd.BH, BW = nd.BW, S = nd.S;
    float zmax = 0.0f;
    constexpr int kObsPer = (4 * RZ_MAX_BOARD_SIZE * RZ_MAX_BOARD_SIZE + kThreads - 1) / kThreads;
    float ob[kObsPer];
    auto load_obs = [&](int board, int tid) {
        const float *src = obs + (size_t)board * 4 * S;
#pragma unroll
        for (int k = 0; k < kObsPer; ++k) {
            const int i = tid + k * kThreads;
            ob[k] = i < 4 * S ? src[i] : 0.0f;
        }
    };
    const bool from_bits = leaves.stones != nullptr;
    int obs_off[kObsPer];
#pragma unroll
    for (int k = 0; k < kObsPer; ++k) obs_off[k] = -1;
    if (!from_bits) {
#pragma unroll
        for (int k = 0; k < kObsPer; ++k) {
            const int i = tid0 + k * kThreads;
            const int c = i / S, r = i - c * S, y = r / BW, x = r - y * BW;
            obs_off[k] = i < 4 * S ? ((y + 1) * IC + (x + 1)) * 8 + c * 2 : -1;
        }
    }
    const int cell_y = tid0 / BW, cell_x = tid0 - cell_y * BW;
    const int cell_off = tid0 < S ? ((cell_y + 1) * IC + (cell_x + 1)) * 8 : -1;
    sp::f16x4 cell_planes = {(_Float16)0.0f, (_Float16)0.0f, (_Float16)0.0f, (_Float16)0.0f};
    auto load_bits = [&](int board, int tid) {
        const uint64_t *sb = leaves.stones + (size_t)board * 8;
        const int tm = leaves.to_move[board], lc = leaves.last[board];
        int nst = 0;
#pragma unroll
        for (int q = 0; q < 8; ++q) nst += __popcll(sb[q]);
        const int word = (tid >> 6) & 3, bit = tid & 63;
        const uint64_t w0 = sb[word], w1 = sb[4 + word];
        const bool s0 = (w0 >> bit) & 1ull, s1 = (w1 >> bit) & 1ull;
        const bool mine = tm == 0 ? s0 : s1, theirs = tm == 0 ? s1 : s0;
        const _Float16 one = (_Float16)sp::kObsScale, zero = (_Float16)0.0f;
        cell_planes[0] = mine ? one : zero;
        cell_planes[1] = theirs ? one : zero;
        cell_planes[2] = (nst > 0 && tid == lc) ? one : zero;
        cell_planes[3] = (nst & 1) ? zero : one;
    };
    auto store_obs = [&](int) {
        if (from_bits) {
            if (cell_off >= 0) {
                *reinterpret_cast<sp::f16x4 *>(in0 + cell_off) = cell_planes;
                *reinterpret_cast<sp::f16x4 *>(in0 + kInPiece + cell_off) =
                    sp::f16x4{(_Float16)0.0f, (_Float16)0.0f, (_Float16)0.0f, (_Float16)0.0f};
            }
            return;
        }
#pragma unroll
        for (int k = 0; k < kObsPer; ++k)
            if (obs_off[k] >= 0) {
                const float z = ob[k] * sp::kObsScale;
                const _Float16 hi = (_Float16)z;
                zmax = fmaxf(zmax, fabsf(z));
                *reinterpret_cast<_Float16 *>(in0 + obs_off[k]) = hi;
                *reinterpret_cast<_Float16 *>(in0 + kInPiece + obs_off[k]) = (_Float16)(z - (float)hi);
            }
    };
    constexpr int kHwPer = (128 * 7 + kThreads - 1) / kThreads;
    float hw_reg[kHwPer];
#pragma unroll
    for (int k = 0; k < kHwPer; ++k) {
        const int i = tid0 + k * kThreads;
        hw_reg[k] = i < 768 ? nd.whp[i] : (i < 128 * 7 ? nd.b3[i - 768] : 0.0f);
    }
    const float bh_reg = tid0 < 6 ? nd.bh[tid0] : 0.0f;
    const float k1 = nd.s_inv[2], k2 = nd.s_inv[0], k3 = nd.s_inv[1];
    const float act1 = nd.s_inv[5], act2 = nd.s_inv[6], act3 = nd.s_inv[7];
    sp::f16x8 a1[3][2];
    f32x4 bias1[4];
    {
        const int lane0 = tid0 & 63;
#pragma unroll
        for (int ky = 0; ky < 3; ++ky)
#pragma unroll
            for (int p_ = 0; p_ < 2; ++p_) a1[ky][p_] = __builtin_bit_cast(sp::f16x8, nd.s1[(ky * 2 + p_) * 64 + lane0]);
#pragma unroll
        for (int g = 0; g < 4; ++g) bias1[g] = *reinterpret_cast<const f32x4 *>(nd.b1 + 8 * g + 4 * (lane0 >> 5)) * act1;
    }
    const bool first = (int)blockIdx.x < n_boards;
    bool sel_first = false;
    if constexpr (RES) sel_first = res.select_first != 0;
    if (first && !sel_first) {
        if (from_bits) load_bits(blockIdx.x, tid0); else load_obs(blockIdx.x, tid0);
    }
    auto planes_from_lds = [&](int tid) {
// ... 2108 lines not shown
    if (n_boards == 0) return RZ_OK;
    if (!d_stones || !d_to_move || !d_last_cell) return net_fail(RZ_ERR_ARG, "NULL device pointer");
    if (n_boards > net->feat_boards) return net_fail(RZ_ERR_ARG, "batch larger than rz_net_reserve()d");
    if (!split_trunk_ok(net))
        return net_fail(RZ_ERR_ARG, "rz_net_trunk_leaves needs the RZ_NET_SPLIT_F16 trunk (the others read float planes: rz_net_trunk)");
    launch_trunk(net, nullptr, net->d_feat, n_boards, stream, LeafBits{d_stones, d_to_move, d_last_cell});
    if (hipGetLastError() != hipSuccess) return net_fail(RZ_ERR_HIP, "launch of k_trunk_split failed");
    return RZ_OK;
}

int rz_net_deferred_reserve(rz_net *net, int32_t max_boards, int32_t slots) {
    int rc = net_ready(net, max_boards);
    if (rc != RZ_OK) return rc;
    if (slots < 1 || max_boards < 1) return net_fail(RZ_ERR_ARG, "rz_net_deferred_reserve: slots and max_boards must be positive");
    if (max_boards <= net->store_boards && slots <= net->store_slots) return RZ_OK;
    if (max_boards < net->store_boards) max_boards = net->store_boards;
    if (slots < net->store_slots) slots = net->store_slots;
    (void)hipDeviceSynchronize();
    if (net->d_store16) (void)hipFree(net->d_store16);
    if (net->d_store_raw) (void)hipFree(net->d_store_raw);
    if (net->d_valfeat) (void)hipFree(net->d_valfeat);
    net->d_store16 = nullptr;
    net->d_store_raw = net->d_valfeat = nullptr;
    net->store_boards = 0;
    net->store_slots = 0;
    const int tiles = ((max_boards + 63) / 64) * 2;
    const size_t store_bytes = (size_t)slots * tiles * net->dev.groups_act * 2048;
    const size_t raw_bytes = (size_t)slots * tiles * 32 * net->dev.Npad * sizeof(float);
    const size_t val_bytes = (size_t)tiles * 32 * net->vf_groups * 4 * sizeof(float);
    if (hipMalloc((void **)&net->d_store16, store_bytes) != hipSuccess || hipMalloc((void **)&net->d_store_raw, raw_bytes) != hipSuccess ||
        hipMalloc((void **)&net->d_valfeat, val_bytes) != hipSuccess)
        return net_fail(RZ_ERR_OOM, "hipMalloc failed (deferred-priors store)");
    if (hipMemset(net->d_store16, 0, store_bytes) != hipSuccess || hipMemset(net->d_valfeat, 0, val_bytes) != hipSuccess)
        return net_fail(RZ_ERR_HIP, "hipMemset failed (deferred-priors store)");
    net->store_tiles = tiles;
    net->store_slots = slots;
    net->store_boards = max_boards;
    return RZ_OK;
}

int rz_net_trunk_leaves_deferred(rz_net *net, const uint64_t *d_stones, const int32_t *d_to_move, const int32_t *d_last_cell,
                                 int32_t n_boards, const int32_t *d_slot_of_board, rz_value_head *out, void *stream) {
    int rc = net_ready(net, n_boards);
    if (rc != RZ_OK) return rc;
    if (!out) return net_fail(RZ_ERR_ARG, "NULL output pointer");
    if (!split_trunk_ok(net))
        return net_fail(RZ_ERR_ARG, "the deferred-priors route needs the RZ_NET_SPLIT_F16 trunk (a net with finite activation bounds)");
    if (n_boards > net->store_boards) return net_fail(RZ_ERR_ARG, "batch larger than rz_net_deferred_reserve()d");
    if (n_boards > 0) {
        if (!d_stones || !d_to_move || !d_last_cell || !d_slot_of_board) return net_fail(RZ_ERR_ARG, "NULL device pointer");
        const DeferredOut later{d_slot_of_board, (long long)net->store_tiles * net->dev.groups_act * 1024, net->d_valfeat, net->vf_groups * 4, net->d_trace, net->store_slots};
        launch_trunk(net, nullptr, net->d_feat, n_boards, stream, LeafBits{d_stones, d_to_move, d_last_cell}, later);
        if (hipGetLastError() != hipSuccess) return net_fail(RZ_ERR_HIP, "launch of the split-f16 trunk failed");
    }
    memset(out, 0, sizeof(*out));
    out->valfeat = net->d_valfeat;
    out->w1t = net->d_w1t;
    out->b1 = net->dev.fc_val1_b;
    out->w2 = net->dev.fc_val2_w;
    out->b2 = net->dev.fc_val2_b;
    out->ld = net->vf_groups * 4;
    out->groups = net->vf_groups;
    return RZ_OK;
}

int rz_net_search_resident(rz_net *net, rz_engine *engine, int32_t n_sims, int32_t select_first, void *stream) {
    rzt::Dev dev;
    int rc = rz_device_view(engine, &dev, (int64_t)sizeof(dev));
    if (rc != RZ_OK) return rc;
    if ((rc = net_ready(net, dev.n_games)) != RZ_OK) return rc;
    if (n_sims < 1) return net_fail(RZ_ERR_ARG, "rz_net_search_resident: n_sims must be positive");
    if (n_sims > net->store_slots || n_sims > dev.pend_cap) {
        char detail[160];
        snprintf(detail, sizeof(detail), ": %d simulations, %d / %d slots (rz_net_deferred_reserve / rz_deferred_reserve)", n_sims, net->store_slots, dev.pend_cap);
        return net_fail(RZ_ERR_ARG, "rz_net_search_resident: more simulations than the store has slots", detail);
    }
    const bool rows = net->algo == RZ_NET_SPLIT_F16 && rows_kernel_covers(net->dev.BH, net->dev.BW);
    const TrunkClass tc = trunk_class(net);
    if (!split_trunk_ok(net) || (!rows && (tc.ms == 0 || net->dev.BH > 10 || net->dev.BW > 10)))
        return net_fail(RZ_ERR_ARG, "the resident search needs the RZ_NET_SPLIT_F16 trunk on a board of 11 .. 16 rows and columns (the row-tile "
                                    "kernel) or of up to 10 x 10 (k_trunk_split with one N-tile per wave)");
    if (dev.K != 1 || dev.score_mode != RZ_SCORE_UCT_REF || dev.pend_cap <= 0)
        return net_fail(RZ_ERR_ARG, "the resident search is the deferred-priors route: RZ_SCORE_UCT_REF, one simulation in flight, rz_deferred_reserve first");
    if (dev.BH != net->dev.BH || dev.BW != net->dev.BW || dev.A != net->dev.A) return net_fail(RZ_ERR_ARG, "engine and network disagree on the board");
    const bool delta_res = net->delta_resident && delta_covers(net) && net->base_games >= dev.n_games;
    const bool compact_res = !rows && tc.compact;
    if (dev.n_games > net->store_boards || (!delta_res && !compact_res && dev.n_games > net->n_cus))
        return net_fail(RZ_ERR_ARG, "the resident search runs one workgroup per game, at most one per CU (any number with rz_net_delta_reserve, or on a board of "
                                    "the compact grid) and rz_net_deferred_reserve()d");
    if (rows ? (net->vf_groups != 64 && net->vf_groups != 128) : net->vf_groups > 64) return net_fail(RZ_ERR_INTERNAL, "value head groups");
    ResArgs<true> res;
    res.E = dev;
    memset(&res.vh, 0, sizeof(res.vh));
    res.vh.w1t = net->d_w1t;
    res.vh.b1 = net->dev.fc_val1_b;
    res.vh.w2 = net->dev.fc_val2_w;
    res.vh.b2 = net->dev.fc_val2_b;
    res.vh.ld = net->vf_groups * 4;
    res.vh.groups = net->vf_groups;
    res.n_sims = n_sims;
    res.select_first = select_first ? 1 : 0;
    const DeferredOut later{dev.pend, (long long)net->store_tiles * net->dev.groups_act * 1024, nullptr, 0, nullptr, net->store_slots};
    const LeafBits leaves{dev.leaf_stones, dev.leaf_to_move, dev.leaf_last};
    const dim3 grid((unsigned)dev.n_games);
    const hipStream_t st = (hipStream_t)stream;
    net->feat16_valid = net->feat32_valid = false;
    if (delta_res) {
        if (select_first) {
            if ((rc = rz_net_delta_bases(net, dev.root_stones, dev.root_to_move, dev.n_games, stream)) != RZ_OK) return rc;
        }
        dl::DeltaArgs da{net->d_base_hdr, net->d_base_recs, net->d_base_ones, nullptr, net->d_delta_stats, 0, (65536 + net->dev.BW - 1) / net->dev.BW, net->d_win};
        dl::k_delta_res<<<grid, dim3(256), 0, st>>>(net->dev, net->d_store16, later, da, res);
        if (hipGetLastError() != hipSuccess) return net_fail(RZ_ERR_HIP, "launch of the resident search (k_delta_res) failed");
        return RZ_OK;
    }
    if (rows)
        with_board_rows(net->dev.BH, [&](auto nt) {
            launch_search_rows<decltype(nt)::value>(grid, st, net->dev, leaves, net->d_store16, dev.n_games, net->d_flags, later, res, net->fp8_cross);
        });
    else
        launch_trunk_split<true>(tc.ms, compact_res, grid, st, net->dev, nullptr, leaves, nullptr, net->d_store16, dev.n_games, net->d_flags,
                                 nullptr, nullptr, later, res);
    if (hipGetLastError() != hipSuccess) return net_fail(RZ_ERR_HIP, "launch of the resident search failed");
    return RZ_OK;
}

int rz_net_delta_reserve(rz_net *net, int32_t n_games) {
    int rc = net_ready(net, n_games);
    if (rc != RZ_OK) return rc;
    if (!delta_covers(net))
        return net_fail(RZ_ERR_ARG, "receptive-field evaluation exists for the RZ_NET_SPLIT_F16 trunk on boards of 11 .. 16 rows and columns");
    if (n_games < 1) return net_fail(RZ_ERR_ARG, "rz_net_delta_reserve: n_games must be positive");
    if (n_games <= net->base_games) return RZ_OK;
    (void)hipDeviceSynchronize();
    if (!net->d_win) {
        std::vector<uint64_t> win(rzw::kEntries);
        rzw::window_table(win.data(), net->dev.BH, net->dev.BW);
        if (hipMalloc((void **)&net->d_win, win.size() * sizeof(uint64_t)) != hipSuccess) return net_fail(RZ_ERR_OOM, "hipMalloc failed (window table)");
        if (hipMemcpy(net->d_win, win.data(), win.size() * sizeof(uint64_t), hipMemcpyHostToDevice) != hipSuccess)
            return net_fail(RZ_ERR_HIP, "hipMemcpy failed (window table)");
    }
    if (net->d_base_hdr) (void)hipFree(net->d_base_hdr);
    if (net->d_base_recs) (void)hipFree(net->d_base_recs);
    if (net->d_base_ones) (void)hipFree(net->d_base_ones);
    net->d_base_ones = nullptr;
    net->d_base_hdr = nullptr;
    net->d_base_recs = nullptr;
    net->base_games = 0;
    const size_t hdr_bytes = (size_t)n_games * sizeof(dl::BaseHdr), rec_bytes = (size_t)n_games * 2 * dl::kBaseBytes;
    if (hipMalloc((void **)&net->d_base_hdr, hdr_bytes) != hipSuccess || hipMalloc((void **)&net->d_base_recs, rec_bytes) != hipSuccess ||
        hipMalloc((void **)&net->d_base_ones, (size_t)n_games) != hipSuccess)
        return net_fail(RZ_ERR_OOM, "hipMalloc failed (base cache)");
    if (hipMemset(net->d_base_ones, 1, (size_t)n_games) != hipSuccess) return net_fail(RZ_ERR_HIP, "hipMemset failed (base cache)");
    if (!net->d_delta_stats && hipMalloc((void **)&net->d_delta_stats, 8 * sizeof(unsigned)) != hipSuccess)
        return net_fail(RZ_ERR_OOM, "hipMalloc failed (delta counters)");
    if (hipMemset(net->d_base_hdr, 0, hdr_bytes) != hipSuccess || hipMemset(net->d_delta_stats, 0, 8 * sizeof(unsigned)) != hipSuccess)
        return net_fail(RZ_ERR_HIP, "hipMemset failed (base cache)");
    net->base_games = n_games;
    return RZ_OK;
}

int rz_net_delta_resident(rz_net *net, int32_t on) {
    if (!net) return net_fail(RZ_ERR_ARG, "net handle is NULL");
    net->delta_resident = on != 0;
    return RZ_OK;
}

int rz_net_delta_invalidate(rz_net *net, void *stream) {
    if (!net) return net_fail(RZ_ERR_ARG, "net handle is NULL");
    if (net->base_games > 0 &&
        hipMemsetAsync(net->d_base_hdr, 0, (size_t)net->base_games * sizeof(dl::BaseHdr), (hipStream_t)stream) != hipSuccess)
        return net_fail(RZ_ERR_HIP, "hipMemsetAsync failed (base cache)");
    return RZ_OK;
}

int rz_net_delta_bases(rz_net *net, const uint64_t *d_root_stones, const int32_t *d_root_to_move, int32_t n_games, void *stream) {
    int rc = net_ready(net, n_games);
    if (rc != RZ_OK) return rc;
    if (n_games == 0) return RZ_OK;
    if (!delta_covers(net)) return net_fail(RZ_ERR_ARG, "receptive-field evaluation: RZ_NET_SPLIT_F16 on boards of 11 .. 16 rows and columns");
    if (n_games > net->base_games) return net_fail(RZ_ERR_ARG, "more games than rz_net_delta_reserve()d");
    if (!d_root_stones || !d_root_to_move) return net_fail(RZ_ERR_ARG, "NULL device pointer");
    dl::DeltaArgs da{net->d_base_hdr, net->d_base_recs, net->d_base_ones, nullptr, nullptr, 1, (65536 + net->dev.BW - 1) / net->dev.BW};
    const DeferredOut none{nullptr, 0, nullptr, 0, nullptr, 0};
    dl::k_trunk_delta<false><<<dim3((unsigned)(2 * n_games)), dim3(256), 0, (hipStream_t)stream>>>(
        net->dev, LeafBits{d_root_stones, d_root_to_move, nullptr}, nullptr, 2 * n_games, none, da);
    if (hipGetLastError() != hipSuccess) return net_fail(RZ_ERR_HIP, "launch of k_trunk_delta (bases) failed");
    return RZ_OK;
}

int rz_net_delta_leaves(rz_net *net, const uint64_t *d_stones, const int32_t *d_to_move, const int32_t *d_last_cell, int32_t n_boards,
                        const int32_t *d_slot_of_board, const uint8_t *d_active, float *d_feat32, int32_t without_base, rz_value_head *out,
                        void *stream) {
    int rc = net_ready(net, n_boards);
    if (rc != RZ_OK) return rc;
    if (!delta_covers(net)) return net_fail(RZ_ERR_ARG, "receptive-field evaluation: RZ_NET_SPLIT_F16 on boards of 11 .. 16 rows and columns");
    if (without_base && n_boards > net->base_games && (rc = rz_net_delta_reserve(net, n_boards)) != RZ_OK) return rc;
    if (n_boards > net->base_games) return net_fail(RZ_ERR_ARG, "more boards than rz_net_delta_reserve()d games");
    if (d_slot_of_board && n_boards > net->store_boards) return net_fail(RZ_ERR_ARG, "batch larger than rz_net_deferred_reserve()d");
    if (n_boards > 0) {
        if (!d_stones || !d_to_move || !d_last_cell) return net_fail(RZ_ERR_ARG, "NULL device pointer");
        if (!d_slot_of_board && !d_feat32) return net_fail(RZ_ERR_ARG, "rz_net_delta_leaves: neither a store slot nor an f32 buffer to write to");
        const DeferredOut later{d_slot_of_board, (long long)net->store_tiles * net->dev.groups_act * 1024, net->d_valfeat, net->vf_groups * 4,
                                net->d_trace, net->store_slots};
        dl::DeltaArgs da{net->d_base_hdr, net->d_base_recs, d_active ? d_active : net->d_base_ones, d_feat32, net->d_delta_stats, without_base ? 2 : 0, (65536 + net->dev.BW - 1) / net->dev.BW};
        const dim3 grid((unsigned)n_boards);
        _Float16 *store = d_slot_of_board ? net->d_store16 : nullptr;
        if (d_slot_of_board) net->feat16_valid = net->feat32_valid = false;
        if (net->d_trace && d_slot_of_board)
            dl::k_trunk_delta<true><<<grid, dim3(256), 0, (hipStream_t)stream>>>(net->dev, LeafBits{d_stones, d_to_move, d_last_cell}, store, n_boards, later, da);
        else
            dl::k_trunk_delta<false><<<grid, dim3(256), 0, (hipStream_t)stream>>>(net->dev, LeafBits{d_stones, d_to_move, d_last_cell}, store, n_boards, later, da);
        if (hipGetLastError() != hipSuccess) return net_fail(RZ_ERR_HIP, "launch of k_trunk_delta failed");
    }
    if (out) {
        memset(out, 0, sizeof(*out));
        out->valfeat = net->d_valfeat;
        out->w1t = net->d_w1t;
        out->b1 = net->dev.fc_val1_b;
        out->w2 = net->dev.fc_val2_w;
        out->b2 = net->dev.fc_val2_b;
        out->ld = net->vf_groups * 4;
        out->groups = net->vf_groups;
    }
    return RZ_OK;
}

int rz_net_delta_bases_engine(rz_net *net, rz_engine *engine, void *stream) {
    rzt::Dev dev;
    int rc = rz_device_view(engine, &dev, (int64_t)sizeof(dev));
    if (rc != RZ_OK) return rc;
    if ((rc = net_ready(net, dev.n_games)) != RZ_OK) return rc;
    if (dev.BH != net->dev.BH || dev.BW != net->dev.BW) return net_fail(RZ_ERR_ARG, "engine and network disagree on the board");
    return rz_net_delta_bases(net, dev.root_stones, dev.root_to_move, dev.n_games, stream);
}

int rz_net_delta_step(rz_net *net, rz_engine *engine, rz_value_head *out, void *stream) {
    rzt::Dev dev;
    int rc = rz_device_view(engine, &dev, (int64_t)sizeof(dev));
    if (rc != RZ_OK) return rc;
    if ((rc = net_ready(net, dev.n_games)) != RZ_OK) return rc;
    if (!out) return net_fail(RZ_ERR_ARG, "NULL output pointer");
    if (dev.K != 1 || dev.pend_cap <= 0 || dev.pend == nullptr)
        return net_fail(RZ_ERR_ARG, "rz_net_delta_step is the deferred-priors route: one simulation in flight, rz_deferred_reserve first");
    if (dev.BH != net->dev.BH || dev.BW != net->dev.BW) return net_fail(RZ_ERR_ARG, "engine and network disagree on the board");
    return rz_net_delta_leaves(net, dev.leaf_stones, dev.leaf_to_move, dev.leaf_last, dev.n_games, dev.pend, dev.active, nullptr, 0, out, stream);
}

int rz_net_delta_trunk_engine(rz_net *net, rz_engine *engine, void *stream) {
    rzt::Dev dev;
    int rc = rz_device_view(engine, &dev, (int64_t)sizeof(dev));
    if (rc != RZ_OK) return rc;
    if ((rc = net_ready(net, dev.n_games)) != RZ_OK) return rc;
    if (!delta_covers(net)) return net_fail(RZ_ERR_ARG, "receptive-field evaluation: RZ_NET_SPLIT_F16 on boards of 11 .. 16 rows and columns");
    if (dev.K != 1) return net_fail(RZ_ERR_ARG, "rz_net_delta_trunk_engine: one simulation in flight per tree (a base per game)");
    if (dev.BH != net->dev.BH || dev.BW != net->dev.BW) return net_fail(RZ_ERR_ARG, "engine and network disagree on the board");
    if (dev.n_games > net->base_games) return net_fail(RZ_ERR_ARG, "more games than rz_net_delta_reserve()d");
    if (dev.n_games > net->feat_boards) return net_fail(RZ_ERR_ARG, "batch larger than rz_net_reserve()d");
    if (net->heads_algo == RZ_NET_HEADS_F32) return net_fail(RZ_ERR_ARG, "rz_net_delta_trunk_engine writes the f16 tiles only (RZ_NET_HEADS_F32 reads f32 features: rz_net_trunk_leaves)");
    net->feat16_valid = true;
    net->feat32_valid = false;
    net->raw_from_trunk = false;
    net->dev.feat_ld = 16 * (net->dev.groups_act + net->dev.groups_val);
    net->dev.feat_val_off = 16 * net->dev.groups_act;
    const DeferredOut later{nullptr, 0, nullptr, 0, nullptr, 0};
    dl::DeltaArgs da{net->d_base_hdr, net->d_base_recs, dev.active ? dev.active : net->d_base_ones, nullptr, net->d_delta_stats, 0,
                     (65536 + net->dev.BW - 1) / net->dev.BW};
    dl::k_trunk_delta<false><<<dim3((unsigned)dev.n_games), dim3(256), 0, (hipStream_t)stream>>>(
        net->dev, LeafBits{dev.leaf_stones, dev.leaf_to_move, dev.leaf_last}, net->d_feat16, dev.n_games, later, da);
    if (hipGetLastError() != hipSuccess) return net_fail(RZ_ERR_HIP, "launch of k_trunk_delta failed");
    return RZ_OK;
}

int rz_net_delta_stats(rz_net *net, uint32_t *h_out8, int32_t reset) {
    if (!net || !h_out8) return net_fail(RZ_ERR_ARG, "NULL argument");
    memset(h_out8, 0, 8 * sizeof(uint32_t));
    if (!net->d_delta_stats) return RZ_OK;
    if (hipDeviceSynchronize() != hipSuccess || hipMemcpy(h_out8, net->d_delta_stats, 8 * sizeof(uint32_t), hipMemcpyDeviceToHost) != hipSuccess)
        return net_fail(RZ_ERR_HIP, "hipMemcpy failed (delta counters)");
    if (reset && hipMemset(net->d_delta_stats, 0, 8 * sizeof(uint32_t)) != hipSuccess) return net_fail(RZ_ERR_HIP, "hipMemset failed (delta counters)");
    return RZ_OK;
}

int rz_net_trace_attach(rz_net *net, void *d_trace) {
    if (!net) return net_fail(RZ_ERR_ARG, "net handle is NULL");
    net->d_trace = (unsigned long long *)d_trace;
    return RZ_OK;
}

int rz_net_deferred_gemm(rz_net *net, int32_t n_boards, int32_t n_slots, rz_deferred_logits *out, void *stream) {
    int rc = net_ready(net, n_boards);
    if (rc != RZ_OK) return rc;
    if (!out) return net_fail(RZ_ERR_ARG, "NULL output pointer");
    if (n_slots < 0 || n_slots > net->store_slots || n_boards > net->store_boards)
        return net_fail(RZ_ERR_ARG, "more slots / boards than rz_net_deferred_reserve()d");
    if (n_slots > 0 && n_boards > 0) {
        NetDev nd = net->dev;
        nd.groups_val = 0;
        const int n_act_tiles = nd.Npad / 32, n_groups = (n_act_tiles + 3) / 4;
        if (n_groups > 2) return net_fail(RZ_ERR_INTERNAL, "more than 256 policy outputs");
        const size_t pairs = (size_t)n_slots * net->store_tiles / 2;
        const dim3 grid((unsigned)(n_groups == 2 ? 2 * ((pairs + 7) / 8 * 8) : pairs));
        k_heads_split<2, 4, 3, false, true><<<grid, dim3(256), 0, (hipStream_t)stream>>>(
            nd, reinterpret_cast<const f32x4 *>(net->d_store16), net->d_store_raw, nullptr, n_slots * net->store_tiles * 32);
        if (hipGetLastError() != hipSuccess) return net_fail(RZ_ERR_HIP, "launch of k_heads_split failed");
    }
    out->raw = net->d_store_raw;
    out->ld = net->dev.Npad;
    out->rows_per_slot = net->store_tiles * 32;
    return RZ_OK;
}

int rz_net_set_algo(rz_net *net, int32_t algo) {
    if (!net) return net_fail(RZ_ERR_ARG, "net handle is NULL");
    if (algo != RZ_NET_DIRECT && algo != RZ_NET_WINOGRAD_F4 && algo != RZ_NET_SPLIT_F16 && algo != RZ_NET_SPLIT_F16_TILES &&
        algo != RZ_NET_SPLIT_F16_FP8)
        return net_fail(RZ_ERR_ARG, "unknown algorithm");
    if (algo == RZ_NET_SPLIT_F16_FP8 && !rows_kernel_covers(net->dev.BH, net->dev.BW))
        return net_fail(RZ_ERR_ARG, "RZ_NET_SPLIT_F16_FP8 exists for boards of 11 .. 16 rows and columns (k_trunk_rows)");
    net->fp8_cross = algo == RZ_NET_SPLIT_F16_FP8;
    net->algo = net->fp8_cross ? RZ_NET_SPLIT_F16 : algo;
    return RZ_OK;
}

int rz_net_range_info(rz_net *net, float *h_info8) {
    if (!net || !h_info8) return net_fail(RZ_ERR_ARG, "NULL argument");
    if (!net->loaded) return net_fail(RZ_ERR_ARG, "rz_net_load has not been called");
    memcpy(h_info8, net->range_info, sizeof(net->range_info));
    return RZ_OK;
}

#ifdef RZ_NET_PROFILE
int rz_net_debug_profile(long long *h_out16) {
    return hipDeviceSynchronize() == hipSuccess && hipMemcpyFromSymbol(h_out16, HIP_SYMBOL(net_prof), 24 * sizeof(long long)) == hipSuccess ? RZ_OK : RZ_ERR_HIP;
}
#endif

int rz_net_set_heads_algo(rz_net *net, int32_t heads_algo) {
    if (!net) return net_fail(RZ_ERR_ARG, "net handle is NULL");
    if (heads_algo < RZ_NET_HEADS_AUTO || heads_algo > RZ_NET_HEADS_IN_TRUNK) return net_fail(RZ_ERR_ARG, "unknown heads algorithm");
    net->heads_algo = heads_algo;
    return RZ_OK;
}

int rz_net_set_max_workgroups(rz_net *net, int32_t max_workgroups) {
    if (!net) return net_fail(RZ_ERR_ARG, "net handle is NULL");
    if (max_workgroups < 0) return net_fail(RZ_ERR_ARG, "max_workgroups must be >= 0");
    net->max_wgs = max_workgroups;
    return RZ_OK;
}

int rz_net_heads_gemm(rz_net *net, int32_t n_boards, rz_raw_heads *out, void *stream) {
    int rc = net_ready(net, n_boards);
    if (rc != RZ_OK) return rc;
    if (!out) return net_fail(RZ_ERR_ARG, "NULL output pointer");
    if (n_boards > net->feat_boards) return net_fail(RZ_ERR_ARG, "batch larger than rz_net_reserve()d");
    if (n_boards > 0) {
        launch_heads_gemm(net, net->d_feat, n_boards, stream);
        if (hipGetLastError() != hipSuccess) return net_fail(RZ_ERR_HIP, "launch of k_heads_gemm failed");
    }
    memset(out, 0, sizeof(*out));
    out->raw = net->d_raw;
    out->hid = net->d_hid;
    out->w2 = net->dev.fc_val2_w;
    out->b2 = net->dev.fc_val2_b;
    out->act_scale = net->dev.s_inv + 3;
    out->act_bias = net->dev.fc_act_b;
    out->val_scale = net->dev.s_inv + 4;
    out->val_bias = net->dev.fc_val1_b;
    out->raw_part_stride = (int64_t)net->raw_part_floats;
    out->hid_part_stride = (int64_t)net->hid_part_floats;
    out->ld = net->dev.Npad;
    out->n_parts = n_boards > 0 ? net->raw_parts : 1;
    return RZ_OK;
}

int rz_net_heads(rz_net *net, int32_t n_boards, float *d_logp, float *d_value, void *stream) {
    int rc = net_ready(net, n_boards);
    if (rc != RZ_OK) return rc;
    if (n_boards == 0) return RZ_OK;
    if (!d_logp || !d_value) return net_fail(RZ_ERR_ARG, "NULL device pointer");
    if (n_boards > net->feat_boards) return net_fail(RZ_ERR_ARG, "batch larger than rz_net_reserve()d");
    return launch_heads(net, net->d_feat, n_boards, d_logp, d_value, stream);
}

int rz_net_forward(rz_net *net, const float *d_obs, int32_t n_boards, float *d_logp, float *d_value, void *stream) {
    int rc = net_ready(net, n_boards);
    if (rc != RZ_OK) return rc;
    if (n_boards == 0) return RZ_OK;
    if (!d_obs || !d_logp || !d_value) return net_fail(RZ_ERR_ARG, "NULL device pointer");
    if (net->fp8_cross)
        return net_fail(RZ_ERR_ARG, "RZ_NET_SPLIT_F16_FP8 evaluates positions (rz_net_trunk_leaves*, rz_net_search_resident): float planes are refused, "
                                    "not computed in another arithmetic");
    if (n_boards > net->feat_boards)
        return net_fail(RZ_ERR_ARG, "batch larger than rz_net_reserve()d (no allocation on the launch path)");
    launch_trunk(net, d_obs, net->d_feat, n_boards, stream);
    if (hipGetLastError() != hipSuccess) return net_fail(RZ_ERR_HIP, "launch of k_trunk failed");
    return launch_heads(net, net->d_feat, n_boards, d_logp, d_value, stream);
}

}
```

rlzero_amd/csrc/rz_tree.h:

```cpp
#pragma once
#include <hip/hip_runtime.h>

#include <cmath>
#include <stdint.h>

#include "rlzero_hip.h"
#include "rz_trace.h"

#pragma clang fp contract(off)

namespace rzt {
namespace {

constexpr int kWave = 64;
constexpr int kWords = RZ_BOARD_WORDS;

struct Dev {
    int kind, BH, BW, S, A, n_row, n_games, score_mode, n_playout;
    int K;
    int path_stride, qcap;
    long long cap, pcap, logtab_n;
    double c_puct;
    int4 *R;
    float *P;
// ... 317 lines not shown
    const float ub = (float)((hash32(key + 0x5bd1e995u) >> 8) + 1u) * k2m24;
    return g * __builtin_amdgcn_exp2f(__builtin_amdgcn_logf(ub) * (1.0f / 0.3f));
}

template <int CTRL>
__device__ __forceinline__ int dpp_move(int x) { return __builtin_amdgcn_update_dpp(0, x, CTRL, 0xF, 0xF, true); }
template <int STAGE>
__device__ __forceinline__ int partner_of(int x, int lane) {
    if (STAGE == 0) return dpp_move<0xB1>(x);
    if (STAGE == 1) return dpp_move<0x4E>(x);
    if (STAGE == 2) return dpp_move<0x141>(x);
    if (STAGE == 3) return dpp_move<0x140>(x);
    if (STAGE == 4) {
        const auto r = __builtin_amdgcn_permlane16_swap((unsigned)x, (unsigned)x, false, false);
        return (int)((lane & 16) ? r[0] : r[1]);
    }
    const auto r = __builtin_amdgcn_permlane32_swap((unsigned)x, (unsigned)x, false, false);
    return (int)((lane & 32) ? r[0] : r[1]);
}
template <int OFF>
__device__ __forceinline__ float xor_partner(float x, int lane) {
    const int v = __float_as_int(x);
    if (OFF == 32) return __int_as_float(partner_of<5>(v, lane));
    if (OFF == 16) return __int_as_float(partner_of<4>(v, lane));
    if (OFF == 8) return __int_as_float(dpp_move<0x128>(v));
    if (OFF == 4) {
        const int up = dpp_move<0x104>(v), down = dpp_move<0x114>(v);
        return __int_as_float((lane & 4) ? down : up);
    }
    if (OFF == 2) return __int_as_float(dpp_move<0x4E>(v));
    return __int_as_float(dpp_move<0xB1>(v));
}
__device__ __forceinline__ float wave_sum(float x, int lane) {
    x += xor_partner<32>(x, lane);
    x += xor_partner<16>(x, lane);
    x += xor_partner<8>(x, lane);
    x += xor_partner<4>(x, lane);
    x += xor_partner<2>(x, lane);
    x += xor_partner<1>(x, lane);
    return x;
}
__device__ __forceinline__ float wave_max(float x, int lane) {
    x = fmaxf(x, xor_partner<32>(x, lane));
    x = fmaxf(x, xor_partner<16>(x, lane));
    x = fmaxf(x, xor_partner<8>(x, lane));
    x = fmaxf(x, xor_partner<4>(x, lane));
    x = fmaxf(x, xor_partner<2>(x, lane));
    x = fmaxf(x, xor_partner<1>(x, lane));
    return x;
}

template <int STAGE>
__device__ __forceinline__ void max_stage(double &mx, int lane) {
    const long long b = __double_as_longlong(mx);
    const int olo = partner_of<STAGE>((int)b, lane), ohi = partner_of<STAGE>((int)(b >> 32), lane);
    const double ob = __longlong_as_double(((long long)ohi << 32) | (unsigned int)olo);
    mx = ob > mx ? ob : mx;
}
template <int W = kWords>
__device__ __forceinline__ int wave_first_max(double best, int besti, bool wide = true) {
    const int lane = (int)__builtin_amdgcn_mbcnt_hi(~0u, __builtin_amdgcn_mbcnt_lo(~0u, 0u));
    double mx = best;
    max_stage<0>(mx, lane);
    max_stage<1>(mx, lane);
    max_stage<2>(mx, lane);
    max_stage<3>(mx, lane);
    if (wide) {
        max_stage<4>(mx, lane);
        max_stage<5>(mx, lane);
    }
    const bool hit = besti != 0x7fffffff && best == mx;
    constexpr int kSlots = W == 1 ? 1 : (W == 2 ? 2 : 4);
#pragma unroll
    for (int s_ = 0; s_ < kSlots; ++s_) {
        const unsigned long long m = __ballot(hit && (besti >> 6) == s_);
        if (m != 0ull) return 64 * s_ + __ffsll((long long)m) - 1;
    }
    return 0x7fffffff;
}

template <bool SC1>
__device__ __forceinline__ int4 load_half(const int4 *R, int idx) {
    if constexpr (SC1) {
        const __amdgpu_buffer_rsrc_t rsrc = __builtin_amdgcn_make_buffer_rsrc(const_cast<int4 *>(R), 0, 0x7fffffff, 0x00020000);
        const auto v = __builtin_amdgcn_raw_buffer_load_b128(rsrc, idx * 16, 0, 16);
        return make_int4((int)v[0], (int)v[1], (int)v[2], (int)v[3]);
    } else {
        return R[idx];
    }
}
template <bool PUCT, int W = kWords, bool PRE = false>
__device__ __forceinline__ int scan_children(const Dev &E, const int4 *R, const float *P, const int4 &lo,
                                             const int4 &hi, double parent_term, int lane, int4 &clo, int4 &chi,
                                             int skip = -1, double *best_out = nullptr) {
    static_assert(!(PRE && PUCT), "the pre-scan is the reference rule's");
    const int k = rec_k(lo), fc = lo.y, pb = hi.z;
    int4 l0 = make_int4(0, -1, 0, 0), l1 = l0, l2 = l0, l3 = l0;
    int4 h0 = make_int4(0, 0, -1, 0), h1 = h0, h2 = h0, h3 = h0;
    float p0 = 0.f, p1 = 0.f, p2 = 0.f, p3 = 0.f;
    if (lane < k) { l0 = load_half<PRE>(R, 2 * (fc + lane)); h0 = load_half<PRE>(R, 2 * (fc + lane) + 1); if (PUCT) p0 = P[pb + lane]; }
    if constexpr (W >= 2) {
        if (lane + 64 < k) { l1 = load_half<PRE>(R, 2 * (fc + lane + 64)); h1 = load_half<PRE>(R, 2 * (fc + lane + 64) + 1); if (PUCT) p1 = P[pb + lane + 64]; }
    }
    if constexpr (W > 2) {
        if (lane + 128 < k) { l2 = load_half<PRE>(R, 2 * (fc + lane + 128)); h2 = load_half<PRE>(R, 2 * (fc + lane + 128) + 1); if (PUCT) p2 = P[pb + lane + 128]; }
        if (lane + 192 < k) { l3 = load_half<PRE>(R, 2 * (fc + lane + 192)); h3 = load_half<PRE>(R, 2 * (fc + lane + 192) + 1); if (PUCT) p3 = P[pb + lane + 192]; }
    }
    double best = -INFINITY;
    int besti = 0x7fffffff;
    int4 blo = l0, bhi = h0;
    auto consider = [&](const int4 &cl, const int4 &ch, float prior, int r0) {
        bool in = r0 < k;
        if constexpr (PRE) in = in && r0 != skip;
        if (in) {
            const double sc = PUCT ? puct(rec_w(ch), cl.x, prior, parent_term, E.c_puct)
                                   : uct_ref(rec_w(ch), cl.x, parent_term, E.c_puct);
            if (sc > best) {
                best = sc;
                besti = r0;
                blo = cl;
                bhi = ch;
            }
        }
    };
    consider(l0, h0, p0, lane);
    if constexpr (W >= 2) consider(l1, h1, p1, lane + 64);
    if constexpr (W > 2) {
        consider(l2, h2, p2, lane + 128);
        consider(l3, h3, p3, lane + 192);
    }
    const int r = __builtin_amdgcn_readfirstlane(wave_first_max<W>(best, besti, W > 2 || __builtin_amdgcn_readfirstlane(k) > 16));
    if constexpr (PRE) *best_out = -INFINITY;
    if (r >= k) return r;
    const int l = r & 63;
    if constexpr (PRE) {
        const long long b = __double_as_longlong(best);
        *best_out = __hiloint2double(__builtin_amdgcn_readlane((int)(b >> 32), l), __builtin_amdgcn_readlane((int)b, l));
    }
    clo = make_int4(__builtin_amdgcn_readlane(blo.x, l), __builtin_amdgcn_readlane(blo.y, l),
                    __builtin_amdgcn_readlane(blo.z, l), __builtin_amdgcn_readlane(blo.w, l));
    chi = make_int4(__builtin_amdgcn_readlane(bhi.x, l), __builtin_amdgcn_readlane(bhi.y, l),
                    __builtin_amdgcn_readlane(bhi.z, l), __builtin_amdgcn_readlane(bhi.w, l));
    return r;
}

struct RootPre {
    int4 lo;
    int r, scan, arena;
    int answered;
    int4 clo, chi;
    double best, term;
    int besti, valid, pad1[2];
};
struct NoHook { static constexpr bool kOn = false; };

template <int W = kWords>
__device__ __forceinline__ void root_prescan(const Dev &E, int g, int lane, RootPre *pre) {
    const int4 lo = make_int4(__builtin_amdgcn_readfirstlane(pre->lo.x), __builtin_amdgcn_readfirstlane(pre->lo.y),
                              __builtin_amdgcn_readfirstlane(pre->lo.z), __builtin_amdgcn_readfirstlane(pre->lo.w));
    const int r = __builtin_amdgcn_readfirstlane(pre->r), scan = __builtin_amdgcn_readfirstlane(pre->scan);
    const int arena = __builtin_amdgcn_readfirstlane(pre->arena);
    const int n1 = lo.x + 1, k = rec_k(lo);
    const bool ok = scan != 0 && n1 >= 1 && n1 < E.logtab_n && lo.y >= 0 && ((long long)lo.y + k) * 32 < 0x7fffffffll;
    if (ok) {
        const int4 *R = arena_records(E, g, arena);
        const double term = E.logtab[n1];
        int4 clo = make_int4(0, -1, 0, 0), chi = make_int4(0, 0, -1, 0);
        double best;
        const int4 nohi = make_int4(0, 0, -1, 0);
        const int bi = scan_children<false, W, true>(E, R, nullptr, lo, nohi, term, lane, clo, chi, r, &best);
        if (lane == 0) {
            pre->clo = clo;
            pre->chi = chi;
            pre->best = best;
            pre->term = term;
            pre->besti = bi;
        }
    }
    if (lane == 0) pre->valid = ok ? 1 : 0;
}

template <bool VL, int W = kWords, class Hook = NoHook>
__device__ __forceinline__ void select_body(const Dev &E, float *obs, int g, int lane, int j = 0, uint64_t *lds_leaf = nullptr,
                                            Hook *hook = nullptr) {
    static_assert(!(Hook::kOn && VL), "the root pre-scan is the sequential search's");
    const int gk = VL ? g * E.K + j : g;
    const int arena = E.cur_arena[g];
    const int top0 = E.top[g];
    int to_move = E.root_to_move[g];
    int last = E.root_last[g];
    const bool act = E.active[g] != 0;
    const int S = E.S;
    uint64_t st[2][kWords];
    load_board<W>(E.root_stones, g, st);
    uint64_t window = 0;
    window = E.line_tab[lane];
    uint64_t window_hi = 0;
    if constexpr (W == 2) window_hi = E.line_tab[kWave + lane];
    RootPre was = {};
    bool pre_ok = false;
    int4 st_lo = make_int4(0, -1, 0, 0);
    int st_r = 0, st_scan = 0;
    if constexpr (Hook::kOn) {
        was = *hook->pre;
        pre_ok = __builtin_amdgcn_readfirstlane(was.scan != 0 && was.valid != 0 ? 1 : 0) != 0;
    }
    if (!act) return;
    int4 *R = arena_records(E, g, arena);
    const float *P = arena_priors(E, g, arena);
    const bool use_puct = E.score_mode == RZ_SCORE_PUCT;
    int top = top0;
    int nst = count_bits<W>(st[0]) + count_bits<W>(st[1]);

    int32_t *path = E.path + (long long)gk * E.path_stride;
    int node = 0, depth = 0, fresh = 0;
    if (lane == 0) path[0] = 0;

    int4 lo = R[0], hi = R[1];
    int4 plo = lo, phi = hi;
    if constexpr (Hook::kOn) {
        const int s = pre_ok ? was.lo.y + was.r : 0;
        plo = R[2 * s];
        phi = R[2 * s + 1];
        hook->root_cell(last, nst, lane);
        hook->tick(0, lo.x);
    }
    for (int it = 0; it <= S; ++it) {
        const int k = rec_k(lo);
        if (k == 0) break;
        int fc = lo.y;
        int r;
        int4 clo = make_int4(0, -1, 0, 0), chi = make_int4(0, 0, -1, 0);
        if (use_puct) {
            r = scan_children<true, W>(E, R, P, lo, hi, sqrt((double)lo.x), lane, clo, chi);
        } else if (lo.z < k) {
            const int nv = lo.z;
            int cap = rec_cap(lo);
            if (nv == cap) {
                const int ncap = cap == 0 ? (k < kFirstCap ? k : kFirstCap) : (2 * cap < k ? 2 * cap : k);
                if ((long long)top + ncap > E.cap) {
                    flag(E, g, RZ_FLAG_ARENA_FULL, lane);
                    fresh = 2;
                    break;
                }
                for (int i = lane; i < nv; i += kWave) {
                    const int4 a = R[2 * (fc + i)], b = R[2 * (fc + i) + 1];
                    R[2 * (top + i)] = a;
                    R[2 * (top + i) + 1] = b;
                }
                if (VL) {
                    for (int jj = 0; jj < j; ++jj) {
                        const int gj = g * E.K + jj;
                        int32_t *pj = E.path + (long long)gj * E.path_stride;
                        const int dj = E.leaf_depth[gj];
                        for (int d = lane; d <= dj; d += kWave) {
                            const int q = pj[d];
                            if (q >= fc && q < fc + nv) pj[d] = q - fc + top;
                        }
                        if (lane == 0) {
                            const int q = E.leaf_node[gj];
                            if (q >= fc && q < fc + nv) E.leaf_node[gj] = q - fc + top;
                        }
                    }
                }
                fc = top;
                top += ncap;
                cap = ncap;
            }
            r = nv;
            fresh = 1;
            if constexpr (Hook::kOn) {
                if (it == 0) st_lo = make_int4(lo.x, fc, nv + 1, pack_kc(k, cap));
            }
            if (lane == 0) {
                R[2 * node] = make_int4(lo.x + (VL ? 1 : 0), fc, nv + 1, pack_kc(k, cap));
                if (VL) {
                    *rec_wsum(R, node) = rec_w(hi) - 1.0;
                    R[2 * (fc + r)] = make_int4(1, -1, 0, 0);
                    R[2 * (fc + r) + 1] = make_hi(-1.0, -1, 0.0f);
                }
            }
        } else {
            const int pn = lo.x;
            if (pn < 1 || pn >= E.logtab_n) {
                flag(E, g, RZ_FLAG_LOGTAB, lane);
                break;
            }
            bool answered = false;
            int r_pre = 0;
            if constexpr (Hook::kOn) {
                if (it == 0 && pre_ok && lo.x == was.lo.x + 1 && lo.y == was.lo.y && lo.z == was.lo.z && lo.w == was.lo.w) {
                    const double sr = uct_ref(rec_w(phi), plo.x, was.term, E.c_puct);
                    const bool cand = sr > -INFINITY, none = was.besti == 0x7fffffff;
                    const bool mine = cand && (none || sr > was.best || (sr == was.best && was.r < was.besti));
                    const bool take = __builtin_amdgcn_readfirstlane(mine ? 1 : 0) != 0;
                    r_pre = __builtin_amdgcn_readfirstlane(take ? was.r : was.besti);
                    const int4 wlo = take ? plo : was.clo, whi = take ? phi : was.chi;
                    clo = make_int4(__builtin_amdgcn_readfirstlane(wlo.x), __builtin_amdgcn_readfirstlane(wlo.y),
                                    __builtin_amdgcn_readfirstlane(wlo.z), __builtin_amdgcn_readfirstlane(wlo.w));
                    chi = make_int4(__builtin_amdgcn_readfirstlane(whi.x), __builtin_amdgcn_readfirstlane(whi.y),
                                    __builtin_amdgcn_readfirstlane(whi.z), __builtin_amdgcn_readfirstlane(whi.w));
                    if (lane == 0) hook->pre->answered += 1;
                    answered = true;
                }
            }
            r = answered ? r_pre : scan_children<false, W>(E, R, P, lo, hi, E.logtab[pn], lane, clo, chi);
            if constexpr (Hook::kOn) {
                if (it == 0) st_lo = lo;
            }
        }
        if constexpr (Hook::kOn) {
            if (it == 0) hook->tick(1, r);
        }
        if (r >= k) {
            flag(E, g, RZ_FLAG_INTERNAL, lane);
            break;
        }
        if (VL && !fresh && lane == 0) {
            *rec_n(R, node) = lo.x + 1;
            *rec_wsum(R, node) = rec_w(hi) - 1.0;
        }
        uint64_t occ[kWords];
#pragma unroll
        for (int j = 0; j < kWords; ++j) occ[j] = st[0][j] | st[1][j];
        const Legal L = legal_of<W>(E, occ, lane);
        int action, cell;
        if (!nth_legal<W>(E, occ, L, r, lane, action, cell)) {
            flag(E, g, RZ_FLAG_INTERNAL, lane);
            break;
        }
        if constexpr (Hook::kOn) {
            hook->cell(depth, cell, lane);
            if (it == 0) {
                st_r = r;
                st_scan = !use_puct && st_lo.z == k ? 1 : 0;
                hook->tick(2, cell);
            }
        }
        if (to_move == 0) set_bit<W>(st[0], cell); else set_bit<W>(st[1], cell);
        last = cell;
        to_move ^= 1;
        nst += 1;
        node = fc + r;
        depth += 1;
        if (lane == 0) path[depth] = node;
        if (fresh) break;
        lo = clo;
        hi = chi;
    }
    if constexpr (Hook::kOn) {
        hook->tick(3, node);
        hook->depth = depth;
        if (lane == 0) {
            RootPre *pre = hook->pre;
            pre->lo = st_lo;
            pre->r = st_r;
            pre->scan = st_scan;
            pre->arena = arena;
        }
    }
    if (lane == 0 && top != top0) E.top[g] = top;
    if (VL && fresh == 0 && lane == 0) {
        *rec_n(R, node) = lo.x + 1;
        *rec_wsum(R, node) = rec_w(hi) - 1.0;
    }

    int term = 0;
    double tval = 0.0;
    {
        int winner = -1;
        if (depth == 0) {
            if (line_anywhere<W>(st[0], S, E.BH, E.BW, E.n_row, lane, E.bw_rcp)) winner = 0;
            else if (line_anywhere<W>(st[1], S, E.BH, E.BW, E.n_row, lane, E.bw_rcp)) winner = 1;
        } else {
            const int mover = to_move ^ 1;
            if (line_through<W>(mover == 0 ? st[0] : st[1], last, E.BH, E.BW, E.n_row, lane, E.bw_rcp, E.n_rcp, window, window_hi, E.line_masks != 0)) winner = mover;
        }
        if (winner >= 0) {
            term = 2;
            tval = (winner == to_move) ? 1.0 : -1.0;
        } else if (nst == S) {
            term = 1;
            tval = 0.0;
        }
    }
    if (lane == 0) {
        E.leaf_node[gk] = node;
        E.leaf_depth[gk] = depth;
        E.leaf_fresh[gk] = fresh;
        E.leaf_term[gk] = term;
        E.leaf_tval[gk] = tval;
        E.leaf_to_move[gk] = to_move;
        E.leaf_last[gk] = last;
    }
    store_board<W>(E.leaf_stones, gk, st, lane);
    if (lds_leaf != nullptr) {
        store_board<W>(lds_leaf, 0, st, lane);
        if (lane == 0) {
            reinterpret_cast<int *>(lds_leaf + 2 * kWords)[0] = to_move;
            reinterpret_cast<int *>(lds_leaf + 2 * kWords)[1] = last;
        }
    }
    if constexpr (Hook::kOn) hook->tick(4, term);
    if (obs != nullptr)
        write_obs(obs + (long long)gk * 4 * S, to_move == 0 ? st[0] : st[1],
                  to_move == 0 ? st[1] : st[0], last, nst, S, lane);
}

typedef rz_raw_heads RawHeads;
typedef rz_value_head ValueHead;
constexpr int kDefWaves = 4;

template <typename VT, bool PROBS = false, bool RAW = false, bool VL = false, bool DEF = false, int W = kWords>
__device__ __forceinline__ void expand_backup_body(const Dev &E, const float *logp, const VT *value, int g,
                                                   int lane, RawHeads rh = RawHeads(), int j = 0, ValueHead vh = ValueHead(),
                                                   float (*part)[kWave] = nullptr) {
    const int gk = VL ? g * E.K + j : g;
    const int slot = DEF ? E.pend[g] : 0;
    const bool act = E.active[g] != 0;
    const int arena = E.cur_arena[g];
    const int depth = E.leaf_depth[gk];
    const int fresh = E.leaf_fresh[gk];
    const int term = E.leaf_term[gk];
    const double leaf_tval = E.leaf_tval[gk];
    const int ptop = E.ptop[g];
    const int nblk = E.nblk[g];
    const int top_now = E.top[g];
    const int noise_ctr = E.noise_ctr[g];
    const int32_t *path = E.path + (long long)gk * E.path_stride;
    const int path_lane = path[lane < E.path_stride ? lane : 0];
    uint64_t st[2][kWords];
    load_board<W>(E.leaf_stones, gk, st);
    float lse = 0.0f, raw_value = 0.0f;
    float x[kWords] = {0.f, 0.f, 0.f, 0.f};
    if (RAW) {
        const float *r = rh.raw + (size_t)gk * rh.ld;
        const float *hp = rh.hid + (size_t)gk * 64 + lane;
        const float w2 = rh.w2[lane], b2 = rh.b2[0];
        float hid = hp[0];
        float mx = -INFINITY;
        if (rh.n_parts == 4) {
            const long long rs = rh.raw_part_stride, hs = rh.hid_part_stride;
            const float act_scale = rh.act_scale[0], val_scale = rh.val_scale[0];
            float part[kWords][4], bias[kWords];
#pragma unroll
            for (int i = 0; i < kWords; ++i) {
                const int j = lane + 64 * i;
                const bool in = j < E.A;
#pragma unroll
                for (int q = 0; q < 4; ++q) part[i][q] = in ? r[j + q * rs] : 0.0f;
                bias[i] = in ? rh.act_bias[j] : 0.0f;
            }
            const float h1 = hp[hs], h2 = hp[2 * hs], h3 = hp[3 * hs], hb = rh.val_bias[lane];
#pragma unroll
            for (int i = 0; i < kWords; ++i) {
                const float sum4 = ((part[i][0] + part[i][1]) + part[i][2]) + part[i][3];
                x[i] = lane + 64 * i < E.A ? fmaf(sum4, act_scale, bias[i]) : -INFINITY;
                mx = fmaxf(mx, x[i]);
            }
            hid = fmaxf(fmaf(((hid + h1) + h2) + h3, val_scale, hb), 0.0f);
        } else {
#pragma unroll
            for (int i = 0; i < kWords; ++i) {
                const int j = lane + 64 * i;
                x[i] = j < E.A ? r[j] : -INFINITY;
                mx = fmaxf(mx, x[i]);
            }
        }
        mx = wave_max(mx, lane);
        float sum = 0.0f;
#pragma unroll
        for (int i = 0; i < kWords; ++i) sum += (lane + 64 * i < E.A) ? expf(x[i] - mx) : 0.0f;
        sum = wave_sum(sum, lane);
        lse = mx + logf(sum);
        float h = hid * w2;
        h = wave_sum(h, lane);
        raw_value = tanhf(h + b2);
    }
    float def_value = 0.0f;
    if (DEF) {
        const float b1 = vh.b1[lane], w2 = vh.w2[lane], b2 = vh.b2[0];
        __syncthreads();
        float hid = part[0][lane];
#pragma unroll
        for (int q = 1; q < kDefWaves; ++q) hid += part[q][lane];
        hid = fmaxf(hid + b1, 0.0f);
        def_value = tanhf(wave_sum(hid * w2, lane) + b2);
    }
    if (!act) return;
    int4 *R = arena_records(E, g, arena);
    float *P = arena_priors(E, g, arena);

    const double v = term ? leaf_tval : (DEF ? (double)def_value : RAW ? (double)raw_value : (double)value[gk]);
    if (DEF && slot >= E.pend_cap) {
        flag(E, g, RZ_FLAG_INTERNAL, lane);
        return;
    }
    const long long rec = DEF ? (long long)slot * E.n_games + g : 0;

    int new_fc = -1, new_nv = 0, new_k = 0, new_cap = 0, new_pb = -1;
    bool expand_now = !term && fresh != 2;
    if (VL && expand_now) {
        const int leaf = __shfl(path_lane, depth < kWave ? depth : 0);
        expand_now = rec_k(R[2 * (depth < kWave ? leaf : path[depth])]) == 0;
    }
    if (expand_now) {
        uint64_t occ[kWords];
#pragma unroll
        for (int j = 0; j < kWords; ++j) occ[j] = st[0][j] | st[1][j];
        const Legal L = legal_of<W>(E, occ, lane);
        const int k = L.k;
        const bool dense = !DEF && E.score_mode == RZ_SCORE_PUCT;
        const int top = dense ? top_now : 0;
        if ((long long)ptop + k > E.pcap || nblk >= E.qcap) {
            flag(E, g, RZ_FLAG_BLOCKS_FULL, lane);
        } else if (dense && (long long)top + k > E.cap) {
            flag(E, g, RZ_FLAG_ARENA_FULL, lane);
        } else {
            new_pb = ptop;
            new_k = k;
            if (dense) {
                new_fc = top;
                new_nv = k;
                new_cap = k;
            }
            if (lane == 0) {
                E.ptop[g] = ptop + k;
                E.nblk[g] = nblk + 1;
                if (dense) E.top[g] = top + k;
            }
            if (DEF) {
                if (lane == 0) {
                    E.pend_pb[rec] = ptop;
                    E.pend_ctr[rec] = noise_ctr;
                    if (E.add_noise) E.noise_ctr[g] = noise_ctr + 1;
                }
                store_board<W>(E.pend_stones, (int)rec, st, lane);
            }
            const float uniform = 1.0f / (float)k;
            if (!DEF) {
            int ranks[kWords];
            int before = 0;
#pragma unroll
            for (int j = 0; j < kWords; ++j) ranks[j] = lane_action_rank(E, occ, L, j, lane, before);
            float noise[kWords] = {0.f, 0.f, 0.f, 0.f};
            float noise_sum = 1.0f;
            if (E.add_noise) {
                const int ctr = noise_ctr;
                const uint64_t key = mix64(mix64(E.noise_key[g]) ^ (uint64_t)ctr);
                float local = 0.0f;
#pragma unroll
                for (int j = 0; j < kWords; ++j)
                    if (ranks[j] >= 0) {
                        noise[j] = gamma03(hash32((uint32_t)key ^ (uint32_t)(key >> 32)) + 0x9E3779B9u * (uint32_t)(64 * j + lane + 1));
                        local += noise[j];
                    }
                local = wave_sum(local, lane);
                noise_sum = local > 0.0f ? local : 1.0f;
                if (lane == 0) E.noise_ctr[g] = ctr + 1;
            }
#pragma unroll
            for (int j = 0; j < kWords; ++j) {
                const int r = ranks[j];
                if (r < 0) continue;
                const int a = 64 * j + lane;
                float prior = uniform;
                if (RAW) prior = expf(x[j] - lse);
                else if (logp) prior = PROBS ? logp[(long long)gk * E.A + a] : expf(logp[(long long)gk * E.A + a]);
                if (E.add_noise) prior = 0.75f * prior + 0.25f * (noise[j] / noise_sum);
                P[ptop + r] = prior;
                if (dense) {
                    R[2 * (top + r)] = make_int4(0, -1, 0, 0);
                    R[2 * (top + r) + 1] = make_hi(0.0, -1, prior);
                }
            }
            }
        }
    }
    if (DEF && lane == 0) {
        if (new_pb < 0) E.pend_pb[rec] = -1;
        E.pend[g] = slot + 1;
    }

    for (int d = lane; d <= depth; d += kWave) {
        const int node = d == lane ? path_lane : path[d];
        const double x = ((depth - d) & 1) ? v : -v;
        if (VL) {
            if (d == depth && new_k > 0) {
                const int4 m = R[2 * node];
                R[2 * node] = make_int4(m.x, new_fc, new_nv, pack_kc(new_k, new_cap));
                *rec_pb(R, node) = new_pb;
            }
            *rec_wsum(R, node) += x + 1.0;
        } else if (d == depth) {
            if (fresh == 1) {
                R[2 * node] = make_int4(1, new_fc, new_nv, pack_kc(new_k, new_cap));
                R[2 * node + 1] = make_hi(0.0 + x, new_pb, 0.0f);
            } else {
                const int4 m = R[2 * node];
                R[2 * node] = (new_k > 0) ? make_int4(m.x + 1, new_fc, new_nv, pack_kc(new_k, new_cap))
                                          : make_int4(m.x + 1, m.y, m.z, m.w);
                *rec_wsum(R, node) += x;
                if (new_k > 0) *rec_pb(R, node) = new_pb;
            }
        } else {
            *rec_n(R, node) += 1;
            *rec_wsum(R, node) += x;
        }
    }
}

template <int PER>
__device__ __forceinline__ void value_quarter_def(const ValueHead &vh, int gk, int lane, int q, float (*part)[kWave]) {
    typedef float vec4 __attribute__((ext_vector_type(4)));
    typedef const __attribute__((address_space(4))) vec4 *uniform_row;
    const vec4 *w = reinterpret_cast<const vec4 *>(vh.w1t) + (size_t)q * 2 * PER * kWave + lane;
    const uniform_row f = (uniform_row)(reinterpret_cast<const vec4 *>(vh.valfeat + (size_t)gk * vh.ld) + q * 2 * PER);
    float a0 = 0.0f, a1 = 0.0f;
#pragma unroll
    for (int half = 0; half < 2; ++half) {
        vec4 wv[PER], fv[PER];
#pragma unroll
        for (int i = 0; i < PER; ++i) {
            wv[i] = w[(size_t)(half * PER + i) * kWave];
            fv[i] = f[half * PER + i];
        }
#pragma unroll
        for (int i = 0; i < PER; ++i) {
            a0 = fmaf(fv[i].x, wv[i].x, a0);
            a1 = fmaf(fv[i].y, wv[i].y, a1);
            a0 = fmaf(fv[i].z, wv[i].z, a0);
            a1 = fmaf(fv[i].w, wv[i].w, a1);
        }
        __builtin_amdgcn_sched_barrier(0);
    }
    part[q][lane] = a0 + a1;
}

template <int PER>
__device__ __forceinline__ void value_quarter_lds(const ValueHead &vh, const float *row, int lane, int q, float (*part)[kWave]) {
    typedef float vec4 __attribute__((ext_vector_type(4)));
    const vec4 *w = reinterpret_cast<const vec4 *>(vh.w1t) + (size_t)q * 2 * PER * kWave + lane;
    const vec4 *f = reinterpret_cast<const vec4 *>(row) + q * 2 * PER;
    float a0 = 0.0f, a1 = 0.0f;
#pragma unroll
    for (int half = 0; half < 2; ++half) {
        vec4 wv[PER], fv[PER];
#pragma unroll
        for (int i = 0; i < PER; ++i) {
            wv[i] = w[(size_t)(half * PER + i) * kWave];
            fv[i] = f[half * PER + i];
        }
#pragma unroll
        for (int i = 0; i < PER; ++i) {
            a0 = fmaf(fv[i].x, wv[i].x, a0);
            a1 = fmaf(fv[i].y, wv[i].y, a1);
            a0 = fmaf(fv[i].z, wv[i].z, a0);
            a1 = fmaf(fv[i].w, wv[i].w, a1);
        }
        __builtin_amdgcn_sched_barrier(0);
    }
    part[q][lane] = a0 + a1;
}

}
}
```

rlzero_amd/engine.py:

```python
import ctypes
import functools
import os

import numpy as np

from . import _hip
from . import route as _route
from ._hip import HipError, check
from .route import compact_grid_board

WORDS = _hip.BOARD_WORDS


def _ptr(t):
    return None if t is None else ctypes.c_void_p(t.data_ptr())


_DEVICE_INDEX = {}


def _current_stream(torch, device):
    raw = getattr(torch._C, '_cuda_getCurrentRawStream', None)
    if raw is None:
        return ctypes.c_void_p(torch.cuda.current_stream(device).cuda_stream)
# ... 23 lines not shown
        self.seed = int(seed) & 0xFFFFFFFFFFFFFFFF
        self.n_limit = int(n_limit)
        self.sim_index = 0

    def __call__(self, eng):
        check(eng.lib.rz_eval_rollout(eng.handle, self.seed, self.sim_index & 0xFFFFFFFF, self.n_limit,
                                      _ptr(eng.value), eng.stream()), 'rz_eval_rollout')
        self.sim_index += 1
        return None, eng.value


class NetEvaluator(object):
    needs_obs = True

    def __init__(self, net):
        self.net = net

    def __call__(self, eng):
        import torch
        with torch.no_grad():
            logp, value = self.net(eng.obs)
        return logp.contiguous(), value.reshape(-1).contiguous()


PARAM_ORDER = ('conv1.weight', 'conv1.bias', 'conv2.weight', 'conv2.bias', 'conv3.weight', 'conv3.bias',
               'act_conv1.weight', 'act_conv1.bias', 'act_fc1.weight', 'act_fc1.bias',
               'val_conv1.weight', 'val_conv1.bias', 'val_fc1.weight', 'val_fc1.bias',
               'val_fc2.weight', 'val_fc2.bias')


def param_shapes(rows, cols, n_actions):
    S = rows * cols
    return ((32, 4, 3, 3), (32, ), (64, 32, 3, 3), (64, ), (128, 64, 3, 3), (128, ), (4, 128, 1, 1), (4, ),
            (n_actions, 4 * S), (n_actions, ), (2, 128, 1, 1), (2, ), (64, 2 * S), (64, ), (1, 64), (1, ))


def check_state_dict(state_dict, rows, cols, n_actions):
    for name, want in zip(PARAM_ORDER, param_shapes(rows, cols, n_actions)):
        if name not in state_dict:
            raise ValueError('the state dict has no %r (a PolicyValueNet state dict holds %s)' % (name, ', '.join(PARAM_ORDER)))
        got = tuple(int(v) for v in state_dict[name].shape)
        if got != want:
            raise ValueError('%r has shape %s, the net of a %d x %d board with %d actions needs %s'
                             % (name, got, rows, cols, n_actions, want))


class HipNet(object):

    def __init__(self, board_size, device='cuda:0', max_boards=512):
        import torch
        self.handle = None
        self.algo, self.heads_algo, self._split_ok, self._store, self._delta_games = 'split_f16', 'auto', True, (0, 0), 0
        self.lib = _hip.load()
        self.torch = torch
        dev = torch.device(device)
        if dev.type != 'cuda' or not torch.cuda.is_available():
            raise HipError('HipNet needs an MI355X (device=%r); there is no CPU fallback' % (device, ))
        self.device = torch.device('cuda', dev.index if dev.index is not None else torch.cuda.current_device())
        if isinstance(board_size, (tuple, list)):
            self.rows, self.cols, self.n_actions = (int(v) for v in board_size)
        else:
            self.rows = self.cols = int(board_size)
            self.n_actions = self.rows * self.cols
        self.board_size, self.n_cells = board_size, self.rows * self.cols
        self.n_cus = torch.cuda.get_device_properties(self.device).multi_processor_count
        handle = ctypes.c_void_p()
        check(self.lib.rz_net_create(self.rows, self.cols, self.n_actions, self.device.index,
                                     ctypes.byref(handle)), 'rz_net_create')
        self.handle = handle
        self.max_boards = 0
        self._want = int(max_boards)
        self.generation = 0

    def set_algo(self, algo):
        code = {'direct': _hip.NET_DIRECT, 'winograd_f4': _hip.NET_WINOGRAD_F4, 'split_f16': _hip.NET_SPLIT_F16,
                'split_f16_tiles': _hip.NET_SPLIT_F16_TILES, 'split_f16_fp8': _hip.NET_SPLIT_F16_FP8}[algo]
        check(self.lib.rz_net_set_algo(self.handle, code), 'rz_net_set_algo')
        self.algo = algo
        return self

    def route(self, **how):
        return _route.decide(self.rows, self.cols, self.algo, self._split_ok, self.heads_algo, **how)

    def reads_positions(self):
        return not self.route(environ={}).needs_planes

    def trunk_leaves(self, eng):
        n = eng.n_leaves
        if n > self.max_boards:
            self.reserve(n)
        stones, to_move, last = eng.leaf_buffers()
        check(self.lib.rz_net_trunk_leaves(self.handle, stones, to_move, last, n, self._stream()), 'rz_net_trunk_leaves')

    def supports_deferred(self):
        return self.route(environ={}).deferred

    def deferred_bytes_per_slot(self, n_boards):
        tiles = (n_boards + 63) // 64 * 2
        k_steps = (4 * self.n_cells + 15) // 16
        n_pad = (self.n_actions + 31) // 32 * 32
        return tiles * k_steps * 2048 + tiles * 32 * n_pad * 4

    def deferred_reserve(self, n_boards, slots):
        have = self._store
        check(self.lib.rz_net_deferred_reserve(self.handle, int(n_boards), int(slots)), 'rz_net_deferred_reserve')
        moved = int(n_boards) > have[0] or int(slots) > have[1]
        if moved:
            self._store = (max(have[0], int(n_boards)), max(have[1], int(slots)))
        return moved and have != (0, 0)

    def trunk_leaves_deferred(self, eng):
        stones, to_move, last = eng.leaf_buffers()
        out = _hip.RzValueHead()
        check(self.lib.rz_net_trunk_leaves_deferred(self.handle, stones, to_move, last, eng.n_leaves, eng.deferred_slot_ptr(),
                                                    ctypes.byref(out), self._stream()), 'rz_net_trunk_leaves_deferred')
        return out

    def supports_delta(self):
        return self.route(environ={}).delta

    def delta_reserve(self, n_games):
        check(self.lib.rz_net_delta_reserve(self.handle, int(n_games)), 'rz_net_delta_reserve')
        self._delta_games = max(self._delta_games, int(n_games))

    def delta_invalidate(self):
        check(self.lib.rz_net_delta_invalidate(self.handle, self._stream()), 'rz_net_delta_invalidate')

    def delta_bases(self, stones, to_move, n_games):
        check(self.lib.rz_net_delta_bases(self.handle, stones, to_move, int(n_games), self._stream()), 'rz_net_delta_bases')

    def delta_leaves(self, stones, to_move, last, n, slot_of=None, active=None, feat32=None, without_base=False, want_head=True):
        out = _hip.RzValueHead() if want_head else None
        check(self.lib.rz_net_delta_leaves(self.handle, stones, to_move, last, int(n), slot_of, active, feat32, 1 if without_base else 0,
                                           ctypes.byref(out) if out is not None else None, self._stream()), 'rz_net_delta_leaves')
        return out

    def delta_bases_engine(self, eng):
        check(self.lib.rz_net_delta_bases_engine(self.handle, eng.handle, self._stream()), 'rz_net_delta_bases_engine')

    def delta_step(self, eng):
        out = _hip.RzValueHead()
        check(self.lib.rz_net_delta_step(self.handle, eng.handle, ctypes.byref(out), self._stream()), 'rz_net_delta_step')
        return out

    def delta_trunk_engine(self, eng):
        check(self.lib.rz_net_delta_trunk_engine(self.handle, eng.handle, self._stream()), 'rz_net_delta_trunk_engine')

    def delta_stats(self, reset=False):
        out = (ctypes.c_uint32 * 8)()
        check(self.lib.rz_net_delta_stats(self.handle, out, 1 if reset else 0), 'rz_net_delta_stats')
        ghz = (256.0 * out[6]) / (10.0 * out[7]) if out[7] else None
        return {'delta': int(out[0]), 'no_base': int(out[1]), 'tiles3': int(out[2]), 'cells': int(out[3]), 'tiles2': int(out[4]),
                'prescans': int(out[5]), 'resident_sclk_ghz': ghz}

    def compact_resident(self):
        return self.route().compact_resident

    def supports_resident(self):
        return self.route(environ={}).resident

    def search_resident(self, eng, n_sims, select_first=False):
        check(self.lib.rz_net_search_resident(self.handle, eng.handle, int(n_sims), 1 if select_first else 0, self._stream()), 'rz_net_search_resident')

    def deferred_gemm(self, n_boards, n_slots):
        out = _hip.RzDeferredLogits()
        check(self.lib.rz_net_deferred_gemm(self.handle, int(n_boards), int(n_slots), ctypes.byref(out), self._stream()),
              'rz_net_deferred_gemm')
        return out

    def range_info(self):
        out = (ctypes.c_float * 8)()
        check(self.lib.rz_net_range_info(self.handle, out), 'rz_net_range_info')
        return {'bounds': (out[0], out[1], out[2]), 'scales': (out[3], out[4], out[5]), 'split_ok': bool(out[6])}

    def check_flags(self):
        flags = ctypes.c_uint32(0)
        check(self.lib.rz_net_error_flags(self.handle, ctypes.byref(flags)), 'rz_net_error_flags')
        if flags.value & _hip.NET_FLAG_F16_RANGE:
            raise HipError("an input outside [0, 1] drove an activation out of the range of the split-f16 trunk: "
                           "use set_algo('direct') for such inputs")
        return self

    def set_heads_algo(self, algo):
        code = {'auto': _hip.NET_HEADS_AUTO, 'f32': _hip.NET_HEADS_F32, 'split32': _hip.NET_HEADS_SPLIT_32,
                'split64': _hip.NET_HEADS_SPLIT_64, 'parts': _hip.NET_HEADS_SPLIT_PARTS, 'in_trunk': _hip.NET_HEADS_IN_TRUNK}[algo]
        check(self.lib.rz_net_set_heads_algo(self.handle, code), 'rz_net_set_heads_algo')
        self.heads_algo = algo
        return self

    def set_max_workgroups(self, n):
        check(self.lib.rz_net_set_max_workgroups(self.handle, int(n)), 'rz_net_set_max_workgroups')
        return self

    def load_state_dict(self, state_dict):
        check_state_dict(state_dict, self.rows, self.cols, self.n_actions)
        arrays = []
        for name in PARAM_ORDER:
            t = state_dict[name]
            a = t.detach().to('cpu', self.torch.float32).contiguous().numpy() if hasattr(t, 'detach') \
                else np.ascontiguousarray(t, dtype=np.float32)
            arrays.append(a)
        ptrs = (ctypes.c_void_p * 16)(*[a.ctypes.data for a in arrays])
        check(self.lib.rz_net_load(self.handle, ptrs, 16), 'rz_net_load')
        self.generation += 1
        self.reserve(max(self._want, self.max_boards))
        self._split_ok = self.range_info()['split_ok']
        return self

    def route_state(self):
        r = self.route(environ={})
        return not r.needs_planes, r.deferred, r.delta, r.resident

    def reserve(self, max_boards):
        check(self.lib.rz_net_reserve(self.handle, int(max_boards)), 'rz_net_reserve')
        self.max_boards = max(self.max_boards, int(max_boards))

    def forward(self, obs, logp=None, value=None):
        t = self.torch
        n = obs.shape[0]
        if n > self.max_boards:
            self.reserve(n)
        if logp is None:
            logp = t.empty((n, self.n_actions), dtype=t.float32, device=self.device)
        if value is None:
            value = t.empty(n, dtype=t.float32, device=self.device)
        st = ctypes.c_void_p(t.cuda.current_stream(self.device).cuda_stream)
        check(self.lib.rz_net_forward(self.handle, _ptr(obs), n, _ptr(logp), _ptr(value), st), 'rz_net_forward')
        return logp, value

    def _stream(self):
        return _current_stream(self.torch, self.device)

    def trunk_internal(self, obs):
        n = obs.shape[0]
        if n > self.max_boards:
            self.reserve(n)
        check(self.lib.rz_net_trunk(self.handle, _ptr(obs), n, None, self._stream()), 'rz_net_trunk')

    def heads_gemm(self, n):
        out = _hip.RzRawHeads()
        check(self.lib.rz_net_heads_gemm(self.handle, int(n), ctypes.byref(out), self._stream()), 'rz_net_heads_gemm')
        return out

    def heads(self, n, logp, value):
        check(self.lib.rz_net_heads(self.handle, int(n), _ptr(logp), _ptr(value), self._stream()), 'rz_net_heads')
        return logp, value

    def trunk(self, obs):
        t = self.torch
        n = obs.shape[0]
        feat = t.empty((n, 6, self.n_cells), dtype=t.float32, device=self.device)
        st = ctypes.c_void_p(t.cuda.current_stream(self.device).cuda_stream)
        check(self.lib.rz_net_trunk(self.handle, _ptr(obs), n, _ptr(feat), st), 'rz_net_trunk')
        return feat

    def close(self):
        if self.handle:
            self.lib.rz_net_destroy(self.handle)
            self.handle = None

    def __del__(self):
        try:
            self.close()
        except Exception:
            pass


class HipNetEvaluator(object):
    fused_heads = True
    deferred_priors = True
    delta_trunk = True
    resident_search = True

    def route(self, eng):
        hip = self.hip
        return _route.decide(hip.rows, hip.cols, hip.algo, hip._split_ok, hip.heads_algo, self.use_positions, self.deferred_priors, self.delta_trunk,
                             self.resident_search, eng.score_mode, eng.sims_in_flight, eng.n_games, hip.n_cus, eng.rows == hip.rows and eng.cols == hip.cols)

    @property
    def needs_obs(self):
        return self.hip.route(use_positions=self.use_positions).needs_planes

    def deferred_ok(self, eng):
        return self.route(eng).deferred

    def delta_ok(self, eng):
        return self.route(eng).delta

    def resident_delta_ok(self, eng):
        return self.route(eng).resident_delta

    def resident_ok(self, eng):
        return self.route(eng).resident

    def resident_per_cu(self, eng):
        return self.route(eng).resident_per_cu

    def delta_three_launch_ok(self, eng):
        return self.route(eng).delta_three_launch

    def reserve_bases(self, eng):
        if self.hip._delta_games < eng.n_games:
            self.hip.torch.cuda.synchronize(self.hip.device)
            self.hip.delta_reserve(eng.n_games)
            eng._drop_graphs('rz_net_delta_reserve moved the base cache')

# ... 804 lines not shown
```

Baseline: 21.38 million.

## Forward tree state between selection and backup in LDS for resident search

The resident search kernel now keeps per-game tree state in shared memory across simulations: root board, arena, top/ptop/nblk counters, leaf depth/fresh/term, the top path slots and records of the first levels. Selection and expand/backup read this forwarded state instead of reloading it from global memory, and backup writes whole records from the cached copies and refreshes the cache. The aim is to take global-memory round trips off the sequential select/backup critical path. In exchange it uses more LDS per workgroup, adds consistency bookkeeping, and ships an optional check mode plus counters and profiling slots.

Result: slower. 21.17 million (-1.0%).

```diff
diff --git a/include/rlzero_hip.h b/include/rlzero_hip.h
--- a/include/rlzero_hip.h
+++ b/include/rlzero_hip.h
@@ -7,7 +7,7 @@
 extern "C" {
 #endif
 
-#define RZ_ABI_VERSION 27
+#define RZ_ABI_VERSION 28
 #define RZ_MAX_BOARD_SIZE 16
 #define RZ_BOARD_WORDS 4
 #define RZ_MAX_IN_FLIGHT 16
@@ -250,6 +250,7 @@
 int rz_net_delta_step(rz_net *net, rz_engine *engine, rz_value_head *out, void *stream);
 int rz_net_delta_trunk_engine(rz_net *net, rz_engine *engine, void *stream);
 int rz_net_delta_stats(rz_net *net, uint32_t *h_out8, int32_t reset);
+int rz_net_resident_stats(rz_net *net, uint32_t *h_out4, int32_t reset);
 int rz_net_search_resident(rz_net *net, rz_engine *engine, int32_t n_sims, int32_t select_first, void *stream);
 int rz_net_heads(rz_net *net, int32_t n_boards, float *d_logp, float *d_value, void *stream);
 int rz_net_heads_gemm(rz_net *net, int32_t n_boards, rz_raw_heads *out, void *stream);
diff --git a/profiles/microbench/delta_resident_phases.py b/profiles/microbench/delta_resident_phases.py
--- a/profiles/microbench/delta_resident_phases.py
+++ b/profiles/microbench/delta_resident_phases.py
@@ -11,7 +11,9 @@
 NAMES = [(0, 'leaf + changed cells'), (1, 'distances, requests, ranks'), (3, 'maps, base records'), (4, 'bar'), (5, 'conv1'), (6, 'bar'), (7, 'conv2'),
          (9, 'bar + conv3 + heads'), (10, 'bar'), (11, 'features'), (12, 'bar'), (16, 'value layer'), (17, 'expand + backup'),
          (2, 'sel: root record'), (8, 'sel: root scan / answer'), (13, 'sel: level-0 cell'), (14, 'sel: deeper levels'), (15, 'sel: terminal test + leaf stores'),
-         (18, 'selection (rest: hand-over)'), (19, 'wave 1: pre-scan'), (20, 'wave 1: wait behind it')]
+         (18, 'selection (rest: hand-over)'), (19, 'wave 1: pre-scan'), (20, 'wave 1: wait behind it'),
+         (24, 'sel: search constants'), (25, 'backup: state arrived'), (26, 'backup: value finished'), (27, 'backup: expansion'),
+         (28, 'backup: path records + stores issued')]
 sizes = [int(a) for a in sys.argv[1:]] or [1, 256, 512]
 for games in sizes:
     torch.manual_seed(0)
@@ -29,15 +31,19 @@
         eng.advance(moves)
         eng.step(moves)
     a, b = torch.cuda.Event(enable_timing=True), torch.cuda.Event(enable_timing=True)
-    ev.hip.delta_stats(reset=True)
+    ev.hip.delta_stats(reset=True); ev.hip.resident_stats(reset=True)
     a.record(); eng.sim_chunk(ev, sims); b.record(); torch.cuda.synchronize()
     st = ev.hip.delta_stats()
-    out = (ctypes.c_longlong * 24)()
+    out = (ctypes.c_longlong * 32)()
     assert lib.rz_net_debug_profile(out) == 0
+    lib.rz_net_debug_profile2.argtypes = [ctypes.c_void_p]
+    assert lib.rz_net_debug_profile2(ctypes.byref(out, 24 * 8)) == 0
+    fwd = ev.hip.resident_stats()
     us = 1e3 * a.elapsed_time(b) / sims
     total = out[23] / sims
     print('%d games, %d simulations: %.2f us per simulation of a game (events, bases included), %d cycles (%.2f GHz); %.2f conv3 / %.2f conv2 tiles, %.2f changed cells per leaf, %d leaves without a base' % (
         games, sims, us, total, total / us / 1e3, st['tiles3'] / max(1, st['delta'] + st['no_base']), st['tiles2'] / max(1, st['delta'] + st['no_base']),
         st['cells'] / max(1, st['delta'] + st['no_base']), st['no_base']))
     print('   ' + '  '.join('%s=%d' % (nm, out[k] / sims) for k, nm in NAMES) + '  prescans=%d' % st['prescans'], flush=True)
+    print('   forwarded: %d selections, %d backups of %d, %d mismatches' % (fwd['forwarded_selections'], fwd['forwarded_backups'], games * sims, fwd['mismatches']), flush=True)
     eng.close(); ev.hip.close()
diff --git a/rlzero_amd/_hip.py b/rlzero_amd/_hip.py
--- a/rlzero_amd/_hip.py
+++ b/rlzero_amd/_hip.py
@@ -3,7 +3,7 @@
 from ctypes import (POINTER, Structure, c_char_p, c_double, c_int, c_int32, c_int64, c_uint32, c_uint64,
                     c_void_p)
 
-ABI_VERSION = 27
+ABI_VERSION = 28
 BOARD_WORDS = 4
 MAX_BOARD_SIZE = 16
 MAX_IN_FLIGHT = 16
@@ -156,6 +156,7 @@
     'rz_net_delta_bases': (c_int, [P, P, P, c_int32, P]),
     'rz_net_delta_leaves': (c_int, [P, P, P, P, c_int32, P, P, P, c_int32, POINTER(RzValueHead), P]),
     'rz_net_delta_stats': (c_int, [P, POINTER(ctypes.c_uint32), c_int32]),
+    'rz_net_resident_stats': (c_int, [P, POINTER(ctypes.c_uint32), c_int32]),
     'rz_net_delta_bases_engine': (c_int, [P, P, P]),
     'rz_net_delta_step': (c_int, [P, P, POINTER(RzValueHead), P]),
     'rz_net_delta_trunk_engine': (c_int, [P, P, P]),
diff --git a/rlzero_amd/csrc/rz_delta.h b/rlzero_amd/csrc/rz_delta.h
--- a/rlzero_amd/csrc/rz_delta.h
+++ b/rlzero_amd/csrc/rz_delta.h
@@ -6,6 +6,12 @@
 #endif
 #ifndef RZ_DELTA_PRESCAN
 #define RZ_DELTA_PRESCAN 1
+#endif
+#ifndef RZ_DELTA_FWD
+#define RZ_DELTA_FWD 1
+#endif
+#ifndef RZ_DELTA_FWD_CHECK
+#define RZ_DELTA_FWD_CHECK 0
 #endif
 
 namespace dl {
@@ -29,8 +35,8 @@
               kLdsBytes = kOffList + 3 * 128 * 2;
 static_assert(kShareFloats * 4 <= kC1Slots * P1, "the shares lie inside conv1's records (dead behind conv2)");
 constexpr int kWinSets = rzw::kRadii * rzw::kWords, kWinLds = kWinSets * 8 + kWinSets * 4 + 16;
-static_assert(2 * (kLdsBytes + 512 * 4 + 4 * 64 * 4 + 80 + kWinLds + (int)sizeof(rzt::RootPre) + 512) <= 160 * 1024,
-              "two workgroups per CU, also of the resident search (value row, K-quarter sums, leaf, window sets, root pre-scan)");
+static_assert(2 * (kLdsBytes + 512 * 4 + 4 * 64 * 4 + 80 + kWinLds + (int)sizeof(rzt::RootPre) + (int)sizeof(rzt::TreeFwd) + 128) <= 160 * 1024,
+              "two workgroups per CU, also of the resident search (value row, K-quarter sums, leaf, window sets, root pre-scan, forwarded tree state)");
 static_assert(kOffC1 % 16 == 0 && kOffZero % 16 == 0 && kOffHead % 16 == 0 && kOffMap1 % 16 == 0, "alignment");
 
 constexpr int kCells = RZ_MAX_BOARD_SIZE * RZ_MAX_BOARD_SIZE;
@@ -278,7 +284,7 @@
     const char *t2p, *t3p;
 };
 #ifdef RZ_NET_PROFILE
-struct Prof { long long acc[24], t; };
+struct Prof { long long acc[32], t; };
 #else
 struct Prof {};
 #endif
@@ -336,7 +342,7 @@
     const uint32_t zaddr = lds_addr(zrec);
     int n_conv3_tiles = 0, n_conv2_tiles = 0;
 #ifdef RZ_NET_PROFILE
-    long long (&prof_acc)[24] = prof.acc, &prof_t = prof.t;
+    long long (&prof_acc)[32] = prof.acc, &prof_t = prof.t;
 #endif
     for (int pass = use_delta ? -1 : 0; pass < 4; ++pass) {
         int tid = tid0;
@@ -661,10 +667,10 @@
     if (TRACE) trace_t0 = rz_trace_now();
     Prof prof;
 #ifdef RZ_NET_PROFILE
-    for (int i = 0; i < 24; ++i) prof.acc[i] = 0;
+    for (int i = 0; i < 32; ++i) prof.acc[i] = 0;
     prof.t = __builtin_readcyclecounter();
     const long long prof_k0 = prof.t;
-    long long (&prof_acc)[24] = prof.acc, &prof_t = prof.t;
+    long long (&prof_acc)[32] = prof.acc, &prof_t = prof.t;
 #endif
     const int tid0 = threadIdx.x, wave = __builtin_amdgcn_readfirstlane(tid0 >> 6);
     const int BW = nd.BW, S = nd.S;
@@ -805,8 +811,16 @@
 #define RZ_SEL_TICKS 0
 #endif
 struct ResHook {
-    static constexpr bool kOn = true;
+    static constexpr bool kOn = true, kFwd = RZ_DELTA_FWD != 0;
+#ifdef RZ_NET_PROFILE
+    static constexpr bool kFwdCheck = kFwd && RZ_DELTA_FWD_CHECK != 0;
+#else
+    static constexpr bool kFwdCheck = false;
+#endif
     rzt::RootPre *pre;
+    rzt::TreeFwd *fwd;
+    const uint64_t *leaf;
+    int pend;
     const uint64_t *win;
     int depth;
     bool any0;
@@ -824,7 +838,7 @@
     __device__ __forceinline__ void tick(int i, int arrived) {
         if ((RZ_SEL_TICKS >> i) & 1) {
             asm volatile("" ::"v"(arrived));
-            const int slot = i == 0 ? 2 : i == 1 ? 8 : 12 + i;
+            const int slot = i == 0 ? 2 : i == 1 ? 8 : i >= 5 ? 19 + i : 12 + i;
             __builtin_amdgcn_sched_barrier(0);
             const long long now = __builtin_readcyclecounter();
             prof->acc[slot] += now - prof->t;
@@ -852,6 +866,7 @@
     __shared__ __attribute__((aligned(16))) uint64_t res_leaf[2 * RZ_BOARD_WORDS + 2];
     __shared__ __attribute__((aligned(16))) uint64_t res_win[kWinLds / 8];
     __shared__ __attribute__((aligned(16))) rzt::RootPre res_pre;
+    __shared__ __attribute__((aligned(16))) rzt::TreeFwd res_fwd;
     const int game = blockIdx.x;
     if (game >= res.E.n_games || res.E.active[game] == 0) return;
     const unsigned long long clk0 = __builtin_readcyclecounter(), rt0 = __builtin_amdgcn_s_memrealtime();
@@ -859,10 +874,10 @@
     const int BW = nd.BW;
     Prof prof;
 #ifdef RZ_NET_PROFILE
-    for (int i = 0; i < 24; ++i) prof.acc[i] = 0;
+    for (int i = 0; i < 32; ++i) prof.acc[i] = 0;
     prof.t = __builtin_readcyclecounter();
     const long long prof_k0 = prof.t;
-    long long (&prof_acc)[24] = prof.acc, &prof_t = prof.t;
+    long long (&prof_acc)[32] = prof.acc, &prof_t = prof.t;
 #endif
     Layers ly;
     ly.t2p = reinterpret_cast<const char *>(nd.t2) + (size_t)wave * rt::Geo<32>::steps * 2 * 1024;
@@ -894,8 +909,32 @@
         for (int i = tid0; i < kResVrow; i += 256) res_vrow[i] = 0.0f;
     }
     if (tid0 == 0) res_pre.scan = res_pre.valid = res_pre.answered = 0;
+    if (tid0 == 0) {
+        rzt::TreeFwd *f = &res_fwd;
+#pragma unroll
+        for (int q = 0; q < 8; ++q) f->root[q] = rs[q];
+        f->arena = res.E.cur_arena[game];
+        f->root_to_move = h_tm;
+        f->root_last = res.E.root_last[game];
+        f->top = res.E.top[game];
+        f->ptop = res.E.ptop[game];
+        f->nblk = res.E.nblk[game];
+        f->noise_ctr = res.E.noise_ctr[game];
+        f->depth = res.E.leaf_depth[game];
+        f->fresh = res.E.leaf_fresh[game];
+        f->term = res.E.leaf_term[game];
+        f->tval = res.E.leaf_tval[game];
+        const int32_t *path = res.E.path + (long long)game * res.E.path_stride;
+#pragma unroll
+        for (int d = 0; d < rzt::kFwdLevels; ++d) f->slot[d] = path[d < res.E.path_stride ? d : 0];
+        f->nrec = f->root_ok = 0;
+        f->n_sel = f->n_bk = f->n_bad = 0;
+    }
     ResHook hook;
     hook.pre = &res_pre;
+    hook.fwd = &res_fwd;
+    hook.leaf = res_leaf;
+    hook.pend = slot0;
     hook.win = da.win;
     hook.depth = 0;
     hook.any0 = false;
@@ -965,7 +1004,8 @@
         NET_TICK(16);
         const bool more = sim + 1 < res.n_sims;
         if (wave == 0) {
-            rzt::expand_backup_body<float, false, false, false, true>(res.E, nullptr, nullptr, game, lane, rz_raw_heads(), 0, res.vh, res_part);
+            hook.pend = slot0 + sim;
+            rzt::expand_backup_body<float, false, false, false, true, rzt::kWords, ResHook>(res.E, nullptr, nullptr, game, lane, rz_raw_heads(), 0, res.vh, res_part, &hook);
         } else {
             __syncthreads();
             if (RZ_DELTA_PRESCAN && wave == 1 && more) {
@@ -1004,6 +1044,9 @@
         atomicAdd(da.stats + 3, (unsigned)cells_total);
         atomicAdd(da.stats + 4, (unsigned)tiles2_total);
         atomicAdd(da.stats + 5, (unsigned)res_pre.answered);
+        atomicAdd(da.stats + 8, (unsigned)res_fwd.n_sel);
+        atomicAdd(da.stats + 9, (unsigned)res_fwd.n_bk);
+        atomicAdd(da.stats + 10, (unsigned)res_fwd.n_bad);
         if (game == 0) {
             da.stats[6] = (unsigned)((__builtin_readcyclecounter() - clk0) >> 8);
             da.stats[7] = (unsigned)(__builtin_amdgcn_s_memrealtime() - rt0);
@@ -1011,7 +1054,7 @@
     }
 #ifdef RZ_NET_PROFILE
     if (blockIdx.x == 0 && tid0 == 0) {
-        for (int i = 0; i < 24; ++i)
+        for (int i = 0; i < 32; ++i)
             if (i != 19 && i != 20) net_prof[i] = prof_acc[i];
         net_prof[23] = __builtin_readcyclecounter() - prof_k0;
         net_prof[22] = tiles_total;
diff --git a/rlzero_amd/csrc/rz_net.hip b/rlzero_amd/csrc/rz_net.hip
--- a/rlzero_amd/csrc/rz_net.hip
+++ b/rlzero_amd/csrc/rz_net.hip
@@ -687,7 +687,7 @@
 };
 
 #ifdef RZ_NET_PROFILE
-__device__ long long net_prof[24];
+__device__ long long net_prof[32];
 #define NET_TICK(i) do { __builtin_amdgcn_sched_barrier(0); const long long now_ = __builtin_readcyclecounter(); prof_acc[i] += now_ - prof_t; prof_t = now_; __builtin_amdgcn_sched_barrier(0); } while (0)
 #else
 #define NET_TICK(i)
@@ -3102,9 +3102,9 @@
         hipMalloc((void **)&net->d_base_ones, (size_t)n_games) != hipSuccess)
         return net_fail(RZ_ERR_OOM, "hipMalloc failed (base cache)");
     if (hipMemset(net->d_base_ones, 1, (size_t)n_games) != hipSuccess) return net_fail(RZ_ERR_HIP, "hipMemset failed (base cache)");
-    if (!net->d_delta_stats && hipMalloc((void **)&net->d_delta_stats, 8 * sizeof(unsigned)) != hipSuccess)
+    if (!net->d_delta_stats && hipMalloc((void **)&net->d_delta_stats, 12 * sizeof(unsigned)) != hipSuccess)
         return net_fail(RZ_ERR_OOM, "hipMalloc failed (delta counters)");
-    if (hipMemset(net->d_base_hdr, 0, hdr_bytes) != hipSuccess || hipMemset(net->d_delta_stats, 0, 8 * sizeof(unsigned)) != hipSuccess)
+    if (hipMemset(net->d_base_hdr, 0, hdr_bytes) != hipSuccess || hipMemset(net->d_delta_stats, 0, 12 * sizeof(unsigned)) != hipSuccess)
         return net_fail(RZ_ERR_HIP, "hipMemset failed (base cache)");
     net->base_games = n_games;
     return RZ_OK;
@@ -3232,6 +3232,16 @@
     return RZ_OK;
 }
 
+int rz_net_resident_stats(rz_net *net, uint32_t *h_out4, int32_t reset) {
+    if (!net || !h_out4) return net_fail(RZ_ERR_ARG, "NULL argument");
+    memset(h_out4, 0, 4 * sizeof(uint32_t));
+    if (!net->d_delta_stats) return RZ_OK;
+    if (hipDeviceSynchronize() != hipSuccess || hipMemcpy(h_out4, net->d_delta_stats + 8, 4 * sizeof(uint32_t), hipMemcpyDeviceToHost) != hipSuccess)
+        return net_fail(RZ_ERR_HIP, "hipMemcpy failed (resident counters)");
+    if (reset && hipMemset(net->d_delta_stats + 8, 0, 4 * sizeof(uint32_t)) != hipSuccess) return net_fail(RZ_ERR_HIP, "hipMemset failed (resident counters)");
+    return RZ_OK;
+}
+
 int rz_net_trace_attach(rz_net *net, void *d_trace) {
     if (!net) return net_fail(RZ_ERR_ARG, "net handle is NULL");
     net->d_trace = (unsigned long long *)d_trace;
@@ -3284,6 +3294,9 @@
 int rz_net_debug_profile(long long *h_out16) {
     return hipDeviceSynchronize() == hipSuccess && hipMemcpyFromSymbol(h_out16, HIP_SYMBOL(net_prof), 24 * sizeof(long long)) == hipSuccess ? RZ_OK : RZ_ERR_HIP;
 }
+int rz_net_debug_profile2(long long *h_out8) {
+    return hipDeviceSynchronize() == hipSuccess && hipMemcpyFromSymbol(h_out8, HIP_SYMBOL(net_prof), 8 * sizeof(long long), 24 * sizeof(long long)) == hipSuccess ? RZ_OK : RZ_ERR_HIP;
+}
 #endif
 
 int rz_net_set_heads_algo(rz_net *net, int32_t heads_algo) {
diff --git a/rlzero_amd/csrc/rz_tree.h b/rlzero_amd/csrc/rz_tree.h
--- a/rlzero_amd/csrc/rz_tree.h
+++ b/rlzero_amd/csrc/rz_tree.h
@@ -493,7 +493,23 @@
     double best, term;
     int besti, valid, pad1[2];
 };
-struct NoHook { static constexpr bool kOn = false; };
+struct NoHook {
+    static constexpr bool kOn = false, kFwd = false, kFwdCheck = false;
+};
+
+constexpr int kFwdLevels = 4;
+struct TreeFwd {
+    int4 lo[kFwdLevels], hi[kFwdLevels];
+    int slot[kFwdLevels];
+    uint64_t root[2 * kWords];
+    int arena, root_to_move, root_last;
+    int top, ptop, nblk, noise_ctr;
+    int depth, fresh, term;
+    int nrec;
+    int root_ok;
+    double tval;
+    int n_sel, n_bk, n_bad, pad;
+};
 
 template <int W = kWords>
 __device__ __forceinline__ void root_prescan(const Dev &E, int g, int lane, RootPre *pre) {
@@ -526,14 +542,38 @@
                                             Hook *hook = nullptr) {
     static_assert(!(Hook::kOn && VL), "the root pre-scan is the sequential search's");
     const int gk = VL ? g * E.K + j : g;
-    const int arena = E.cur_arena[g];
-    const int top0 = E.top[g];
-    int to_move = E.root_to_move[g];
-    int last = E.root_last[g];
-    const bool act = E.active[g] != 0;
+    int arena, top0, to_move, last;
+    bool act;
     const int S = E.S;
     uint64_t st[2][kWords];
-    load_board<W>(E.root_stones, g, st);
+    if constexpr (Hook::kFwd) {
+        const TreeFwd *f = hook->fwd;
+        arena = f->arena;
+        top0 = f->top;
+        to_move = f->root_to_move;
+        last = f->root_last;
+        act = true;
+#pragma unroll
+        for (int j = 0; j < kWords; ++j) {
+            st[0][j] = j < W ? f->root[j] : 0ull;
+            st[1][j] = j < W ? f->root[kWords + j] : 0ull;
+        }
+        if constexpr (Hook::kFwdCheck) {
+            uint64_t ld[2][kWords];
+            load_board<W>(E.root_stones, g, ld);
+            bool same = arena == E.cur_arena[g] && top0 == E.top[g] && to_move == E.root_to_move[g] && last == E.root_last[g] && E.active[g] != 0;
+#pragma unroll
+            for (int j = 0; j < kWords; ++j) same = same && ld[0][j] == st[0][j] && ld[1][j] == st[1][j];
+            if (lane == 0 && !same) hook->fwd->n_bad += 1;
+        }
+    } else {
+        arena = E.cur_arena[g];
+        top0 = E.top[g];
+        to_move = E.root_to_move[g];
+        last = E.root_last[g];
+        act = E.active[g] != 0;
+        load_board<W>(E.root_stones, g, st);
+    }
     uint64_t window = 0;
     window = E.line_tab[lane];
     uint64_t window_hi = 0;
@@ -556,17 +596,50 @@
     int32_t *path = E.path + (long long)gk * E.path_stride;
     int node = 0, depth = 0, fresh = 0;
     if (lane == 0) path[0] = 0;
-
-    int4 lo = R[0], hi = R[1];
-    int4 plo = lo, phi = hi;
-    if constexpr (Hook::kOn) {
+    bool bad = false;
+    bool fw_sel = false;
+    if constexpr (Hook::kOn) hook->tick(5, top0);
+
+    int4 lo, hi;
+    int4 plo, phi;
+    if constexpr (Hook::kFwd) {
+        TreeFwd *f = hook->fwd;
         const int s = pre_ok ? was.lo.y + was.r : 0;
-        plo = R[2 * s];
-        phi = R[2 * s + 1];
+        fw_sel = __builtin_amdgcn_readfirstlane(f->root_ok != 0 && (!pre_ok || f->slot[1] == s) ? 1 : 0) != 0;
+        if (fw_sel) {
+            lo = f->lo[0], hi = f->hi[0];
+            plo = f->lo[1], phi = f->hi[1];
+            if constexpr (Hook::kFwdCheck) {
+                const int4 a = R[0], b = R[1], c = R[2 * s], d = R[2 * s + 1];
+                bool same = a.x == lo.x && a.y == lo.y && a.z == lo.z && a.w == lo.w && b.x == hi.x && b.y == hi.y && b.z == hi.z && b.w == hi.w;
+                if (pre_ok) same = same && c.x == plo.x && c.y == plo.y && c.z == plo.z && c.w == plo.w && d.x == phi.x && d.y == phi.y && d.z == phi.z && d.w == phi.w;
+                if (lane == 0 && !same) f->n_bad += 1;
+            }
+        } else {
+            lo = R[0], hi = R[1];
+            plo = R[2 * s], phi = R[2 * s + 1];
+        }
+        if (lane == 0) f->slot[0] = 0;
         hook->root_cell(last, nst, lane);
         hook->tick(0, lo.x);
+    } else {
+        lo = R[0], hi = R[1];
+        plo = lo, phi = hi;
+        if constexpr (Hook::kOn) {
+            const int s = pre_ok ? was.lo.y + was.r : 0;
+            plo = R[2 * s];
+            phi = R[2 * s + 1];
+            hook->root_cell(last, nst, lane);
+            hook->tick(0, lo.x);
+        }
     }
     for (int it = 0; it <= S; ++it) {
+        if constexpr (Hook::kFwd) {
+            if (depth < kFwdLevels && lane == 0) {
+                hook->fwd->lo[depth] = lo;
+                hook->fwd->hi[depth] = hi;
+            }
+        }
         const int k = rec_k(lo);
         if (k == 0) break;
         int fc = lo.y;
@@ -582,6 +655,7 @@
                 if ((long long)top + ncap > E.cap) {
                     flag(E, g, RZ_FLAG_ARENA_FULL, lane);
                     fresh = 2;
+                    bad = true;
                     break;
                 }
                 for (int i = lane; i < nv; i += kWave) {
@@ -613,6 +687,9 @@
             if constexpr (Hook::kOn) {
                 if (it == 0) st_lo = make_int4(lo.x, fc, nv + 1, pack_kc(k, cap));
             }
+            if constexpr (Hook::kFwd) {
+                if (depth < kFwdLevels && lane == 0) hook->fwd->lo[depth] = make_int4(lo.x, fc, nv + 1, pack_kc(k, cap));
+            }
             if (lane == 0) {
                 R[2 * node] = make_int4(lo.x + (VL ? 1 : 0), fc, nv + 1, pack_kc(k, cap));
                 if (VL) {
@@ -625,6 +702,7 @@
             const int pn = lo.x;
             if (pn < 1 || pn >= E.logtab_n) {
                 flag(E, g, RZ_FLAG_LOGTAB, lane);
+                bad = true;
                 break;
             }
             bool answered = false;
@@ -642,6 +720,9 @@
                     chi = make_int4(__builtin_amdgcn_readfirstlane(whi.x), __builtin_amdgcn_readfirstlane(whi.y),
                                     __builtin_amdgcn_readfirstlane(whi.z), __builtin_amdgcn_readfirstlane(whi.w));
                     if (lane == 0) hook->pre->answered += 1;
+                    if constexpr (Hook::kFwd) {
+                        if (lane == 0 && fw_sel) hook->fwd->n_sel += 1;
+                    }
                     answered = true;
                 }
             }
@@ -655,6 +736,7 @@
         }
         if (r >= k) {
             flag(E, g, RZ_FLAG_INTERNAL, lane);
+            bad = true;
             break;
         }
         if (VL && !fresh && lane == 0) {
@@ -668,6 +750,7 @@
         int action, cell;
         if (!nth_legal<W>(E, occ, L, r, lane, action, cell)) {
             flag(E, g, RZ_FLAG_INTERNAL, lane);
+            bad = true;
             break;
         }
         if constexpr (Hook::kOn) {
@@ -685,6 +768,9 @@
         node = fc + r;
         depth += 1;
         if (lane == 0) path[depth] = node;
+        if constexpr (Hook::kFwd) {
+            if (depth < kFwdLevels && lane == 0) hook->fwd->slot[depth] = node;
+        }
         if (fresh) break;
         lo = clo;
         hi = chi;
@@ -701,6 +787,9 @@
         }
     }
     if (lane == 0 && top != top0) E.top[g] = top;
+    if constexpr (Hook::kFwd) {
+        if (lane == 0 && top != top0) hook->fwd->top = top;
+    }
     if (VL && fresh == 0 && lane == 0) {
         *rec_n(R, node) = lo.x + 1;
         *rec_wsum(R, node) = rec_w(hi) - 1.0;
@@ -734,6 +823,17 @@
         E.leaf_to_move[gk] = to_move;
         E.leaf_last[gk] = last;
     }
+    if constexpr (Hook::kFwd) {
+        if (lane == 0) {
+            TreeFwd *f = hook->fwd;
+            const int have = fresh == 1 ? depth : depth + 1;
+            f->depth = depth;
+            f->fresh = fresh;
+            f->term = term;
+            f->tval = tval;
+            f->nrec = bad ? 0 : (have < kFwdLevels ? have : kFwdLevels);
+        }
+    }
     store_board<W>(E.leaf_stones, gk, st, lane);
     if (lds_leaf != nullptr) {
         store_board<W>(lds_leaf, 0, st, lane);
@@ -752,26 +852,68 @@
 typedef rz_value_head ValueHead;
 constexpr int kDefWaves = 4;
 
-template <typename VT, bool PROBS = false, bool RAW = false, bool VL = false, bool DEF = false, int W = kWords>
+template <class Hook>
+__device__ __forceinline__ const TreeFwd *fwd_of(Hook *hook) {
+    if constexpr (Hook::kFwd) return hook->fwd;
+    else return nullptr;
+}
+template <class Hook>
+__device__ __forceinline__ int pend_of(Hook *hook) {
+    if constexpr (Hook::kFwd) return hook->pend;
+    else return 0;
+}
+template <typename VT, bool PROBS = false, bool RAW = false, bool VL = false, bool DEF = false, int W = kWords, class Hook = NoHook>
 __device__ __forceinline__ void expand_backup_body(const Dev &E, const float *logp, const VT *value, int g,
                                                    int lane, RawHeads rh = RawHeads(), int j = 0, ValueHead vh = ValueHead(),
-                                                   float (*part)[kWave] = nullptr) {
+                                                   float (*part)[kWave] = nullptr, Hook *hook = nullptr) {
+    static_assert(!Hook::kFwd || (DEF && !VL), "the forwarded state is the resident search's");
     const int gk = VL ? g * E.K + j : g;
-    const int slot = DEF ? E.pend[g] : 0;
-    const bool act = E.active[g] != 0;
-    const int arena = E.cur_arena[g];
-    const int depth = E.leaf_depth[gk];
-    const int fresh = E.leaf_fresh[gk];
-    const int term = E.leaf_term[gk];
-    const double leaf_tval = E.leaf_tval[gk];
-    const int ptop = E.ptop[g];
-    const int nblk = E.nblk[g];
-    const int top_now = E.top[g];
-    const int noise_ctr = E.noise_ctr[g];
+    const TreeFwd *f = fwd_of<Hook>(hook);
+    const int slot = Hook::kFwd ? pend_of<Hook>(hook) : DEF ? E.pend[g] : 0;
+    const bool act = Hook::kFwd ? true : E.active[g] != 0;
+    const int arena = Hook::kFwd ? f->arena : E.cur_arena[g];
+    const int depth = Hook::kFwd ? f->depth : E.leaf_depth[gk];
+    const int fresh = Hook::kFwd ? f->fresh : E.leaf_fresh[gk];
+    const int term = Hook::kFwd ? f->term : E.leaf_term[gk];
+    const double leaf_tval = Hook::kFwd ? f->tval : E.leaf_tval[gk];
+    const int ptop = Hook::kFwd ? f->ptop : E.ptop[g];
+    const int nblk = Hook::kFwd ? f->nblk : E.nblk[g];
+    const int top_now = Hook::kFwd ? f->top : E.top[g];
+    const int noise_ctr = Hook::kFwd ? f->noise_ctr : E.noise_ctr[g];
     const int32_t *path = E.path + (long long)gk * E.path_stride;
-    const int path_lane = path[lane < E.path_stride ? lane : 0];
+    const int fs = Hook::kFwd ? f->slot[lane & (kFwdLevels - 1)] : 0;
+    const int path_lane = Hook::kFwd && depth < kFwdLevels ? fs : path[lane < E.path_stride ? lane : 0];
     uint64_t st[2][kWords];
-    load_board<W>(E.leaf_stones, gk, st);
+    if constexpr (!Hook::kFwd) load_board<W>(E.leaf_stones, gk, st);
+    int4 flo = make_int4(0, -1, 0, 0), fhi = make_int4(0, 0, -1, 0);
+    bool have = false;
+    if constexpr (Hook::kFwd) {
+        flo = f->lo[lane & (kFwdLevels - 1)];
+        fhi = f->hi[lane & (kFwdLevels - 1)];
+        have = lane < f->nrec && lane <= depth && fs == path_lane;
+#pragma unroll
+        for (int q = 0; q < kWords; ++q) {
+            st[0][q] = q < W ? hook->leaf[q] : 0ull;
+            st[1][q] = q < W ? hook->leaf[kWords + q] : 0ull;
+        }
+        if constexpr (Hook::kFwdCheck) {
+            uint64_t ld[2][kWords];
+            load_board<W>(E.leaf_stones, gk, ld);
+            bool same = slot == E.pend[g] && E.active[g] != 0 && arena == E.cur_arena[g] && depth == E.leaf_depth[gk] && fresh == E.leaf_fresh[gk] &&
+                        term == E.leaf_term[gk] && __double_as_longlong(leaf_tval) == __double_as_longlong(E.leaf_tval[gk]) && ptop == E.ptop[g] &&
+                        nblk == E.nblk[g] && top_now == E.top[g] && noise_ctr == E.noise_ctr[g];
+#pragma unroll
+            for (int q = 0; q < kWords; ++q) same = same && ld[0][q] == st[0][q] && ld[1][q] == st[1][q];
+            if (lane <= depth && lane < E.path_stride) same = same && path_lane == path[lane];
+            if (have) {
+                const int4 a = arena_records(E, g, arena)[2 * path_lane], b = arena_records(E, g, arena)[2 * path_lane + 1];
+                same = same && a.x == flo.x && a.y == flo.y && a.z == flo.z && a.w == flo.w && b.x == fhi.x && b.y == fhi.y && b.z == fhi.z && b.w == fhi.w;
+            }
+            const unsigned long long wrong = __ballot(!same);
+            if (lane == 0 && wrong != 0ull) hook->fwd->n_bad += 1;
+        }
+    }
+    if constexpr (Hook::kOn) hook->tick(6, path_lane + depth + ptop);
     float lse = 0.0f, raw_value = 0.0f;
     float x[kWords] = {0.f, 0.f, 0.f, 0.f};
     if (RAW) {
@@ -828,6 +970,7 @@
         hid = fmaxf(hid + b1, 0.0f);
         def_value = tanhf(wave_sum(hid * w2, lane) + b2);
     }
+    if constexpr (Hook::kOn) hook->tick(7, __float_as_int(def_value));
     if (!act) return;
     int4 *R = arena_records(E, g, arena);
     float *P = arena_priors(E, g, arena);
@@ -835,12 +978,16 @@
     const double v = term ? leaf_tval : (DEF ? (double)def_value : RAW ? (double)raw_value : (double)value[gk]);
     if (DEF && slot >= E.pend_cap) {
         flag(E, g, RZ_FLAG_INTERNAL, lane);
+        if constexpr (Hook::kFwd) {
+            if (lane == 0) hook->fwd->root_ok = 0;
+        }
         return;
     }
     const long long rec = DEF ? (long long)slot * E.n_games + g : 0;
 
     int new_fc = -1, new_nv = 0, new_k = 0, new_cap = 0, new_pb = -1;
     bool expand_now = !term && fresh != 2;
+    bool flagged = false;
     if (VL && expand_now) {
         const int leaf = __shfl(path_lane, depth < kWave ? depth : 0);
         expand_now = rec_k(R[2 * (depth < kWave ? leaf : path[depth])]) == 0;
@@ -855,8 +1002,10 @@
         const int top = dense ? top_now : 0;
         if ((long long)ptop + k > E.pcap || nblk >= E.qcap) {
             flag(E, g, RZ_FLAG_BLOCKS_FULL, lane);
+            flagged = true;
         } else if (dense && (long long)top + k > E.cap) {
             flag(E, g, RZ_FLAG_ARENA_FULL, lane);
+            flagged = true;
         } else {
             new_pb = ptop;
             new_k = k;
@@ -869,6 +1018,13 @@
                 E.ptop[g] = ptop + k;
                 E.nblk[g] = nblk + 1;
                 if (dense) E.top[g] = top + k;
+            }
+            if constexpr (Hook::kFwd) {
+                if (lane == 0) {
+                    hook->fwd->ptop = ptop + k;
+                    hook->fwd->nblk = nblk + 1;
+                    if (E.add_noise) hook->fwd->noise_ctr = noise_ctr + 1;
+                }
             }
             if (DEF) {
                 if (lane == 0) {
@@ -923,10 +1079,29 @@
         E.pend[g] = slot + 1;
     }
 
+    if constexpr (Hook::kOn) hook->tick(8, new_pb);
+    int4 nlo = flo, nhi = fhi;
+    bool whole = false;
     for (int d = lane; d <= depth; d += kWave) {
         const int node = d == lane ? path_lane : path[d];
         const double x = ((depth - d) & 1) ? v : -v;
-        if (VL) {
+        const bool fw = Hook::kFwd && have && d == lane;
+        if (fw) {
+            const double w = rec_w(fhi) + x;
+            if (d == depth) {
+                nlo = (new_k > 0) ? make_int4(flo.x + 1, new_fc, new_nv, pack_kc(new_k, new_cap)) : make_int4(flo.x + 1, flo.y, flo.z, flo.w);
+                nhi = make_int4(__double2loint(w), __double2hiint(w), new_k > 0 ? new_pb : fhi.z, fhi.w);
+                R[2 * node] = nlo;
+                *rec_wsum(R, node) = w;
+                if (new_k > 0) *rec_pb(R, node) = new_pb;
+            } else {
+                nlo = make_int4(flo.x + 1, flo.y, flo.z, flo.w);
+                nhi = make_int4(__double2loint(w), __double2hiint(w), fhi.z, fhi.w);
+                *rec_n(R, node) = flo.x + 1;
+                *rec_wsum(R, node) = w;
+            }
+            whole = true;
+        } else if (VL) {
             if (d == depth && new_k > 0) {
                 const int4 m = R[2 * node];
                 R[2 * node] = make_int4(m.x, new_fc, new_nv, pack_kc(new_k, new_cap));
@@ -937,6 +1112,11 @@
             if (fresh == 1) {
                 R[2 * node] = make_int4(1, new_fc, new_nv, pack_kc(new_k, new_cap));
                 R[2 * node + 1] = make_hi(0.0 + x, new_pb, 0.0f);
+                if constexpr (Hook::kFwd) {
+                    nlo = make_int4(1, new_fc, new_nv, pack_kc(new_k, new_cap));
+                    nhi = make_hi(0.0 + x, new_pb, 0.0f);
+                    whole = d == lane;
+                }
             } else {
                 const int4 m = R[2 * node];
                 R[2 * node] = (new_k > 0) ? make_int4(m.x + 1, new_fc, new_nv, pack_kc(new_k, new_cap))
@@ -947,6 +1127,21 @@
         } else {
             *rec_n(R, node) += 1;
             *rec_wsum(R, node) += x;
+        }
+    }
+    if constexpr (Hook::kOn) hook->tick(9, nlo.x);
+    if constexpr (Hook::kFwd) {
+        TreeFwd *f = hook->fwd;
+        const bool mine = lane <= depth && lane < kWave;
+        const unsigned long long loaded = __ballot(lane <= depth && !whole);
+        const bool none_loaded = depth < kWave && loaded == 0ull;
+        if (mine && lane < 2 && whole) {
+            f->lo[lane] = nlo;
+            f->hi[lane] = nhi;
+        }
+        if (lane == 0) {
+            f->root_ok = !flagged && (loaded & 3ull) == 0ull ? 1 : 0;
+            if (none_loaded) f->n_bk += 1;
         }
     }
 }
diff --git a/rlzero_amd/engine.py b/rlzero_amd/engine.py
--- a/rlzero_amd/engine.py
+++ b/rlzero_amd/engine.py
@@ -199,6 +199,11 @@
         ghz = (256.0 * out[6]) / (10.0 * out[7]) if out[7] else None
         return {'delta': int(out[0]), 'no_base': int(out[1]), 'tiles3': int(out[2]), 'cells': int(out[3]), 'tiles2': int(out[4]),
                 'prescans': int(out[5]), 'resident_sclk_ghz': ghz}
+
+    def resident_stats(self, reset=False):
+        out = (ctypes.c_uint32 * 4)()
+        check(self.lib.rz_net_resident_stats(self.handle, out, 1 if reset else 0), 'rz_net_resident_stats')
+        return {'forwarded_selections': int(out[0]), 'forwarded_backups': int(out[1]), 'mismatches': int(out[2])}
 
     def compact_resident(self):
         return self.route().compact_resident
```
